# meringlab/FlashWeave.jl

Measured on AMD Instinct MI355X. Metric: ci_tests_per_sec, higher is better.
Workload: dtype f64

## Files before the change

flashweave.jl_amd/csrc/fw_devhiton.hip:

```cpp
#include <algorithm>
#include <cassert>
#include <cstring>
#include <condition_variable>
#include <mutex>
#include <thread>
#include <vector>

#include "fw_internal.h"
#define MI_MAX_K FW_MAX_K_FAST
#include "fw_mi_core.h"
#include "fw_fz_core.h"
#include "fw_unrank.h"

namespace {

struct DhTgt {
    int32_t T, phase, pos, nc;
    int32_t na, ntpc, npc, wl_n;
    long long co;
    long long cand_off;
    long long wl_off, nb_off;
    int32_t nb_n, cap;
    int32_t jactive, nsp;
    int32_t cur, pad0;
    unsigned long long jN, jnext, jwidth, jwin, jevaluated;
    unsigned long long c_eval_short;
    int na_max, wl_used;
    double jbest_p, jbest_stat;
    unsigned long long c_ref, c_calls, c_eval;
    double c_alg;
    unsigned int r_first0, r_more0, r_first1, r_more1;
    int32_t spmode, wl_unsorted;
    unsigned long long jwin2, jN2;
    long long tm_off;
};

struct DhGlobal {
    unsigned long long launched_ranks, next_ranks;
    unsigned int n_live_prev, n_live_next;
    unsigned int ns, seglen, done, rounds, rounds_nonempty, max_a;
    unsigned long long cond_tests_ref, subsets_calls, evaluated;
    double alg_bytes;
    unsigned int n_act, act_sel;
    unsigned int pad_b, max_ab;
    unsigned int ns_ring[64];
    unsigned int pad_l0[32];
    unsigned int step_ticket;
    unsigned int pad_l1[31];
    unsigned int any_big;
    unsigned int pad_l2[31];
};

#define DH_ACC_OFF(x, b, d1) (2ll * (x).co * (long long)(d1) + 2ll * (long long)(b) * (long long)(x).cap)

struct DhArrays {
    const int32_t *cand0;
    int32_t *tpc_key, *pc_key, *acc;
    double *tpc_stat, *tpc_p, *pc_stat, *pc_p;
    const int32_t *wl;
    const unsigned int *wl_cnt;
    const long long *nb_off;
    const int32_t *nb_idx;
    const double *nb_stat, *nb_p;
    const float *tmat;
    fw_rejection *rej;
};

struct DhParams {
    double alpha;
    int max_k;
    long long max_tests;
    unsigned long long small_launch, w0_big, w0_small;
    unsigned int seg_q, seg_min;
    double disc_bytes_per_col;
    int elim_full;
    unsigned long long growth_small, growth, growth_busy;
    unsigned int busy_jobs;
    int spec_depth;
    unsigned long long spec_below;
    unsigned int mi_seq, mi_win0, mi_chunk_div, mi_chunk_min, mi_chunk_max, mi_help_jobs;
    unsigned int mi_elim_min;
    unsigned int mi_heavy;
    unsigned int mi_seq_heavy;
    unsigned int mi_seq_tail;
    unsigned int mi_chunk_tail, mi_win0_tail;
    unsigned int mi_ahead;
    unsigned int mi_team;
    unsigned int mi_team_tail;
    unsigned int mi_team_steps;
    unsigned int mi_trace;
    int spec0_depth;
    unsigned long long spec0_below;
    unsigned int spec0_jobs;
    int spec0_depth_light;
    unsigned long long spec0_light_below;
    int spec1_depth;
    int elim_mode;
};

__device__ __forceinline__ bool dh_in_wl(const DhTgt &x, const DhArrays &A, int32_t v)
{
    const int lane = (int)(threadIdx.x & 63u);
    const int32_t *w = A.wl + x.wl_off;
    for (int base = 0; base < x.wl_n; base += 64) {
        const int32_t e = base + lane < x.wl_n ? w[base + lane] : -1;
        if (__ballot(e == v) != 0ull) return true;
        if (!x.wl_unsorted && __shfl(e, 63) > v) return false;
    }
    return false;
}

__device__ __forceinline__ double dh_alg_bytes(int a, unsigned long long evaluated, int max_k, double disc_bytes_per_col)
{
    double bytes = 0.0, left = (double)evaluated;
    for (int s = max_k; s >= 1 && left > 0.0; --s) {
        double b = 1.0;
        for (int i = 1; i <= s; ++i) b = b * (double)(a - s + i) / (double)i;
        if (a < s) b = 0.0;
        const double cnt = left < b ? left : b;
        bytes += cnt * (disc_bytes_per_col > 0.0 ? (double)(s + 2) * disc_bytes_per_col + 32.0
                                                 : 4.0 * (double)((s + 2) * (s + 1) / 2) + 32.0);
        left -= cnt;
    }
    return bytes;
}

__device__ __forceinline__ unsigned long long dh_enum_size(int a, int max_k, long long max_tests)
{
    unsigned long long N = 0ull;
    if (max_k <= 3 && a <= FW_UNRANK32_A) {
        for (int s = max_k; s >= 1; --s) N += (unsigned long long)fw_binom32(a, s);
    } else {
        for (int s = max_k; s >= 1; --s) {
            N += fw_binom_u64(a, s);
            if (N > (1ull << 62)) N = 1ull << 62;
        }
    }
    if (max_tests > 0 && (unsigned long long)max_tests < N) N = (unsigned long long)max_tests;
    return N;
}

__device__ __noinline__ void dh_rej_write(const DhTgt &x, const DhArrays &A, int max_k, int32_t cand, const int32_t *acc, int a,
                                          unsigned long long nt, double stat, double p, int df, int pow)
{
    const int32_t *b = A.nb_idx + x.nb_off;
    int lo = 0, hi = x.nb_n;
    while (lo < hi) {
        const int mid = (lo + hi) >> 1;
        if (b[mid] < cand)
            lo = mid + 1;
        else
            hi = mid;
    }
    if (lo >= x.nb_n || b[lo] != cand) return;
    fw_rejection r;
    r.target = x.T;
    r.candidate = cand;
    r.n_zs = 0;
#pragma unroll
    for (int q = 0; q < FW_MAX_K; ++q) r.zs[q] = 0;
    if (nt > 0ull) {
        unsigned long long rem = nt - 1ull;
        int s = max_k;
        while (s > 1) {
            const unsigned long long cnt = fw_binom_u64(a, s);
            if (rem < cnt) break;
            rem -= cnt;
            --s;
        }
        int pos[FW_MAX_K_FAST];
        fw_unrank_comb(rem, a, s, pos);
        r.n_zs = s;
#pragma unroll
        for (int q = 0; q < FW_MAX_K_FAST; ++q)
            if (q < s) r.zs[q] = acc[pos[q]];
    }
    r.df = nt > 0ull ? df : 0;
    r.suff_power = pow;
    r.phase = x.phase;
    r.n_acc = a;
    r.num_tests = (long long)nt;
    r.frac = 0.0;
    r.stat = stat;
    r.pval = p;
    A.rej[x.nb_off + lo] = r;
}

__device__ __forceinline__ double dh_alg_bytes_disc32(int a, unsigned long long evaluated, int max_k, double disc_bytes_per_col)
{
    double bytes = 0.0;
    unsigned long long left = evaluated;
    for (int s = max_k; s >= 1 && left > 0ull; --s) {
        const unsigned long long b = (unsigned long long)fw_binom32(a, s), cnt = left < b ? left : b;
        bytes += (double)cnt * ((double)(s + 2) * disc_bytes_per_col + 32.0);
        left -= cnt;
    }
    return bytes;
}

__device__ bool dh_advance(DhTgt &x, const DhArrays &A, int lane, int d1, bool keep_elim_stats = false)
{
    for (;;) {
        int32_t *acc = A.acc + DH_ACC_OFF(x, x.cur, d1);
        if (x.phase == 2) return false;
        const int32_t *cands = x.phase == 0 ? A.cand0 + x.cand_off : A.tpc_key + x.co;
        int32_t *dkey = (x.phase == 0 ? A.tpc_key : A.pc_key) + x.co;
        double *dstat = (x.phase == 0 ? A.tpc_stat : A.pc_stat) + x.co;
        double *dp = (x.phase == 0 ? A.tpc_p : A.pc_p) + x.co;
        int32_t &dn = x.phase == 0 ? x.ntpc : x.npc;
        while (x.pos < x.nc) {
            const int32_t cand = cands[x.pos];
            if (x.wl_n > 0 && dh_in_wl(x, A, cand)) {
                if (lane == 0) {
                    acc[x.na] = cand;
                    dkey[dn] = cand;
                    dstat[dn] = NAN;
                    dp[dn] = NAN;
                }
                ++x.na;
                x.wl_used += x.phase == 0 ? 1 : 0;
                ++dn;
                ++x.pos;
                continue;
            }
            if (x.phase == 1) {
                __builtin_amdgcn_fence(__ATOMIC_SEQ_CST, "workgroup");
                int w = 0;
                for (int base = 0; base < x.na; base += 64) {
                    const int q = base + lane;
                    const int32_t v = q < x.na ? acc[q] : cand;
                    const bool keep = q < x.na && v != cand;
                    const unsigned long long m = __ballot(keep);
                    if (keep) acc[w + __popcll(m & ((1ull << lane) - 1ull))] = v;
                    w += __popcll(m);
                }
                x.na = w;
                __builtin_amdgcn_fence(__ATOMIC_SEQ_CST, "workgroup");
            }
            if (x.na == 0) {
                double s = NAN, p = NAN;
                if (x.phase == 0) {
                    const int32_t *b = A.nb_idx + x.nb_off;
                    int lo = 0, hi = x.nb_n;
                    while (lo < hi) {
                        const int mid = (lo + hi) >> 1;
                        if (b[mid] < cand)
                            lo = mid + 1;
                        else
                            hi = mid;
                    }
                    s = A.nb_stat[x.nb_off + lo];
                    p = A.nb_p[x.nb_off + lo];
                } else {
                    for (int q = 0; q < x.ntpc; ++q)
                        if (A.tpc_key[x.co + q] == cand) {
                            s = A.tpc_stat[x.co + q];
                            p = A.tpc_p[x.co + q];
                            break;
                        }
                }
                if (lane == 0) {
                    acc[x.na] = cand;
                    dkey[dn] = cand;
                    dstat[dn] = s;
                    dp[dn] = p;
                }
                ++x.na;
                ++dn;
                ++x.pos;
                continue;
            }
            return true;
        }
        __builtin_amdgcn_fence(__ATOMIC_SEQ_CST, "workgroup");
        if (x.phase == 0) {
            x.phase = 1;
            x.nc = x.ntpc;
            for (int q = lane; q < x.ntpc; q += 64) acc[q] = A.tpc_key[x.co + q];
            x.na = x.ntpc;
            x.pos = 0;
        } else {
            for (int i = keep_elim_stats ? x.npc : lane; i < x.npc; i += 64) {
                const int32_t k = A.pc_key[x.co + i];
                for (int q = 0; q < x.ntpc; ++q)
                    if (A.tpc_key[x.co + q] == k) {
                        const double tp = A.tpc_p[x.co + q], pp = A.pc_p[x.co + i];
                        if (tp > pp || isnan(pp)) {
                            A.pc_stat[x.co + i] = A.tpc_stat[x.co + q];
                            A.pc_p[x.co + i] = tp;
                        }
                        break;
                    }
            }
            x.phase = 2;
        }
        __builtin_amdgcn_fence(__ATOMIC_SEQ_CST, "workgroup");
    }
}

__device__ __forceinline__ unsigned int dh_ceil_div(unsigned long long w, unsigned long long seglen, double inv)
{
    if (w == 0ull) return 0u;
    unsigned long long q = (unsigned long long)((double)w * inv);
    while (q * seglen < w) ++q;
    while (q > 0ull && (q - 1ull) * seglen >= w) --q;
    return (unsigned int)q;
}


#define DH_MAX_SPEC 8
#define DH_SPEC_EXACT 4

struct DhMerge {
    bool stop;
    double stat, p;
    int pow;
    unsigned long long nt;
    unsigned long long ev;
    double g;
    int df;
};

template <bool TR = false>
__device__ __forceinline__ DhMerge dh_merge(const FwSegOut *__restrict__ so, long long base, int nseg, int lane)
{
    unsigned long long ev = 0ull;
    int my_stop = 0x7fffffff;
    double st_stat = 0.0, st_p = 0.0;
    int st_pow = 0, st_df = 0;
    unsigned long long st_rank = 0ull;
    double bp = -2.0, bs = 0.0;
    int bi = -1;
    for (int sg = lane; sg < nseg; sg += 64) {
        const FwSegOut o = so[base + sg];
        ev += o.evaluated;
        if (o.stop_rank != FW_RANK_NONE) {
            if (my_stop == 0x7fffffff) {
                my_stop = sg;
                st_stat = o.stop_stat;
                st_p = o.stop_pval;
                st_pow = o.stop_power;
                st_rank = o.stop_rank;
                st_df = o.stop_df;
            }
        } else if (o.best_pval >= bp) {
            bp = o.best_pval;
            bs = o.best_stat;
            bi = sg;
        }
    }
    int first = my_stop;
#pragma unroll
    for (int o = 32; o > 0; o >>= 1) {
        ev += __shfl_xor(ev, o);
        const int f2 = __shfl_xor(first, o);
        first = f2 < first ? f2 : first;
        const double p2 = __shfl_xor(bp, o), s2 = __shfl_xor(bs, o);
        const int i2 = __shfl_xor(bi, o);
        if (p2 > bp || (p2 == bp && i2 > bi)) {
            bp = p2;
            bs = s2;
            bi = i2;
        }
    }
    DhMerge M;
    M.ev = ev;
    if (first != 0x7fffffff) {
        const int owner = first & 63;
        M.stop = true;
        M.stat = __shfl(st_stat, owner);
        M.p = __shfl(st_p, owner);
        M.pow = __shfl(st_pow, owner);
        M.nt = __shfl(st_rank, owner) + 1ull;
        if (__shfl(st_df, owner) == -2) M.nt = 0ull;
        if constexpr (TR) M.df = __shfl(st_df, owner);
    } else {
        M.stop = false;
        M.stat = bs;
        M.p = bi >= 0 ? bp : -2.0;
        M.pow = 1;
        M.nt = 0ull;
    }
    M.g = 0.0;
    if constexpr (!TR) M.df = 0;
    else if (!M.stop) M.df = 0;
    return M;
}

template <bool TR = false>
__device__ __forceinline__ bool dh_commit(DhTgt &x, const DhArrays &A, int lane, int d1, double r_stat, double r_p, int r_pow,
                                          double alpha, bool exact = false, int max_k_rej = 0, unsigned long long r_nt = 0ull, int r_df = 0)
{
    const int32_t *cands = x.phase == 0 ? A.cand0 + x.cand_off : A.tpc_key + x.co;
    const int32_t cand = cands[x.pos];
    ++x.pos;
    if (!(r_p < alpha && r_pow)) {
        if constexpr (TR) {
            if (lane == 0) dh_rej_write(x, A, max_k_rej, cand, A.acc + DH_ACC_OFF(x, x.cur, d1), x.na, r_nt, r_stat, r_p, r_df, r_pow);
        }
        if (!(exact && x.phase == 1)) return false;
        if (lane == 0) A.acc[DH_ACC_OFF(x, x.cur, d1) + x.na] = cand;
        ++x.na;
        return true;
    }
    if (lane == 0) {
        A.acc[DH_ACC_OFF(x, x.cur, d1) + x.na] = cand;
        if (x.phase == 0) {
            A.tpc_key[x.co + x.ntpc] = cand;
            A.tpc_stat[x.co + x.ntpc] = r_stat;
            A.tpc_p[x.co + x.ntpc] = r_p;
        } else {
            A.pc_key[x.co + x.npc] = cand;
            A.pc_stat[x.co + x.npc] = r_stat;
            A.pc_p[x.co + x.npc] = r_p;
        }
    }
    ++x.na;
    if (x.phase == 0)
        ++x.ntpc;
    else
        ++x.npc;
    return true;
}

#define MI_BOARD_CAP (1u << 18)
#define MI_REC_CAP (1u << 20)

__shared__ unsigned short dh_mi_tab[4][2 * MI_TAB16];

__shared__ int32_t dh_mi_acc[4][1024];
__shared__ DhTgt dh_mi_x[4];
__shared__ MiBest dh_mi_seed[4];
struct DhMiCtx {
    DhArrays A;
    MiDev M;
    DhParams P;
};
__shared__ DhMiCtx dh_mi_ctx;
__shared__ FwSegOut dh_mi_out[4];
#ifdef FW_MI_TICKS
__shared__ unsigned long long dh_mi_ticks[4][12];
#endif

struct MiBoard {
    unsigned long long tc;
    unsigned long long ac;
    unsigned long long acc_off;
    unsigned long long start, end;
    unsigned long long nr;
    unsigned long long stop_min;
    unsigned int next_chunk, done;
    unsigned int ready, seed_df;
    double seed_p, seed_g;
};

struct alignas(16) MiQueue {
    unsigned int next_target, targets_done, n_boards, hint, res_top, bacc_top, pad[1], next_team;
    unsigned long long t_body, t_ctl, t_sleep, n_seg;
    unsigned long long t_total;
    unsigned long long tick[12];
    unsigned long long tm_run, tm_wait, tm_steps, tm_tests;
};

#define MI_BACC_CAP (1u << 22)
#define MI_ACC_LDS 1024

__device__ __forceinline__ unsigned int mi_ld_u32(const unsigned int *p) { return __hip_atomic_load(p, __ATOMIC_RELAXED, __HIP_MEMORY_SCOPE_AGENT); }
__device__ __forceinline__ unsigned long long mi_ld_u64(const unsigned long long *p) { return __hip_atomic_load(p, __ATOMIC_RELAXED, __HIP_MEMORY_SCOPE_AGENT); }
__device__ __forceinline__ void mi_st_u64(unsigned long long *p, unsigned long long v) { __hip_atomic_store(p, v, __ATOMIC_RELAXED, __HIP_MEMORY_SCOPE_AGENT); }
__device__ __forceinline__ void mi_st_u32(unsigned int *p, unsigned int v) { __hip_atomic_store(p, v, __ATOMIC_RELAXED, __HIP_MEMORY_SCOPE_AGENT); }
__device__ __forceinline__ void mi_drain() { asm volatile("s_waitcnt vmcnt(0)" ::: "memory"); }
typedef unsigned int mi_u32x4 __attribute__((ext_vector_type(4)));
__device__ __forceinline__ mi_u32x4 mi_ld_u128(const void *p)
{
    mi_u32x4 v;
    asm volatile("global_load_dwordx4 %0, %1, off sc1\n\ts_waitcnt vmcnt(0)" : "=v"(v) : "v"(p) : "memory");
    return v;
}
#ifndef MI_NAP_WAIT
#define MI_NAP_WAIT 2
#endif
#ifndef MI_NAP_TAIL
#define MI_NAP_TAIL 32
#endif
__device__ __forceinline__ void mi_nap_wait()
{
#pragma unroll
    for (int i = 0; i < MI_NAP_WAIT; ++i) __builtin_amdgcn_s_sleep(2);
}
__device__ __forceinline__ void mi_nap_tail()
{
#pragma unroll
    for (int i = 0; i < MI_NAP_TAIL; ++i) __builtin_amdgcn_s_sleep(8);
}
#ifndef MI_WD_TICKS
#define MI_WD_TICKS 200000000ull
#endif
struct MiWatch {
    unsigned long long t0;
    unsigned int last, n;
};
__device__ __forceinline__ void mi_watch_begin(MiWatch &w, unsigned int word)
{
    w.t0 = 0ull;
    w.last = word;
    w.n = 0u;
}
__device__ __forceinline__ bool mi_watch_expired(MiWatch &w, unsigned int word)
{
    if (word != w.last) {
        w.last = word;
        w.t0 = 0ull;
        w.n = 0u;
        return false;
    }
    if ((++w.n & 255u) != 0u) return false;
    const unsigned long long now = wall_clock64();
    if (w.t0 == 0ull) {
        w.t0 = now;
        return false;
    }
    return now - w.t0 > MI_WD_TICKS;
}
__device__ __forceinline__ unsigned int mi_wave_add(unsigned int *p, unsigned int v, int lane)
{
    unsigned int r = 0u;
    if (lane == 0) r = atomicAdd(p, v);
    return (unsigned int)__builtin_amdgcn_readfirstlane((int)r);
}

__device__ __forceinline__ unsigned long long mi_rfl_lane64(unsigned long long v, int src)
{
    const unsigned lo = (unsigned)__builtin_amdgcn_readlane((int)(unsigned)v, src), hi = (unsigned)__builtin_amdgcn_readlane((int)(unsigned)(v >> 32), src);
    return ((unsigned long long)hi << 32) | lo;
}

template <int L, int NXY, int PRE, bool STOP_P = false>
__device__ __noinline__ void mi_run_ranks(int T, int cand, const int32_t *__restrict__ acc_in, int a, int max_k,
                                          long long max_tests, unsigned long long r0, unsigned long long r1,
                                          const unsigned long long *stop_min_in, int remote_acc, const MiBest *seed_in)
{
    unsigned short *tab = dh_mi_tab[threadIdx.x >> 6];
    const MiDev M = mi_uniform(dh_mi_ctx.M);
    T = __builtin_amdgcn_readfirstlane(T);
    cand = __builtin_amdgcn_readfirstlane(cand);
    a = __builtin_amdgcn_readfirstlane(a);
    max_k = __builtin_amdgcn_readfirstlane(max_k);
    max_tests = (long long)mi_rfl64((unsigned long long)max_tests);
    r0 = mi_rfl64(r0);
    r1 = mi_rfl64(r1);
    const int32_t *acc = (const int32_t *)mi_rfl64((unsigned long long)acc_in);
    const unsigned long long *stop_min = (const unsigned long long *)mi_rfl64((unsigned long long)stop_min_in);
    remote_acc = __builtin_amdgcn_readfirstlane(remote_acc);
    FwSegOut o;
    o.stop_rank = FW_RANK_NONE;
    o.stop_stat = o.stop_pval = 0.0;
    o.best_rank = 0ull;
    o.best_stat = 0.0;
    o.best_pval = -3.0;
// ... 1010 lines not shown
                        o.evaluated += computed;
                    }
                }
            }
            if (!first_known)
                o = mi_run_ranks_sel<L, NXY, PRE, R4>(x.T, cand, A.acc + acc_off, a, P.max_k, P.max_tests, 0ull, next, nullptr, 0, nullptr);
            unsigned long long ev = o.evaluated, nt = 0ull;
            bool stopped = o.stop_rank != FW_RANK_NONE;
            double r_stat = stopped ? o.stop_stat : 0.0, r_p = stopped ? o.stop_pval : 0.0;
            int r_pow = stopped ? o.stop_power : 1;
            double best_p = o.best_pval, best_stat = o.best_stat, best_g = stopped ? 0.0 : o.stop_stat;
            int best_df = o.best_df;
            if (stopped) nt = o.stop_rank + 1ull;
            unsigned long long width = elim_full ? N : (unsigned long long)(tail ? P.mi_win0_tail : P.mi_win0);
            const unsigned long long chunk_min = tail ? P.mi_chunk_tail : P.mi_chunk_min;
            unsigned int bacc_off = MI_BACC_CAP;
            const unsigned long long tk2 = MI_CLK();
            tk_seq += tk2 - tk1;
            if (lane == 0) x.r_first1 += (unsigned int)(tk2 - tk1);
            while (!stopped && next < N) {
                const unsigned long long W = (N - next) < width ? (N - next) : width;
                unsigned long long chunk = W / (unsigned long long)P.mi_chunk_div;
                chunk = chunk < chunk_min ? chunk_min : (chunk > P.mi_chunk_max ? P.mi_chunk_max : chunk);
                const unsigned int nch = (unsigned int)((W + chunk - 1ull) / chunk);
                unsigned int bi, ro;
                const unsigned long long tkp0 = MI_CLK();
                const bool published = mi_publish(Q, boards, bacc, bacc_off, A.acc + acc_off, a, x.T, cand, next, W, chunk, nch, lane, bi, ro,
                                                  best_p, best_g, best_df);
                MI_TICK(9, tkp0);
                DhMerge mg;
                if (!published) {
                    const FwSegOut q = mi_run_ranks_sel<L, NXY, PRE, R4>(x.T, cand, A.acc + acc_off, a, P.max_k, P.max_tests, next, next + W, nullptr, 0, nullptr);
                    mg.stop = q.stop_rank != FW_RANK_NONE;
                    mg.stat = mg.stop ? q.stop_stat : q.best_stat;
                    mg.p = mg.stop ? q.stop_pval : (q.best_pval < 0.0 ? -2.0 : q.best_pval);
                    mg.pow = q.stop_power;
                    mg.nt = q.stop_rank + 1ull;
                    mg.ev = q.evaluated;
                    mg.g = q.stop_stat;
                    mg.df = q.best_df;
                } else {
                    MiBoard *b = boards + bi;
                    while (mi_board_work<L, NXY, PRE, R4>(b, res, bacc, A.acc + acc_off, lane)) {
                    }
                    MiWatch wd;
                    unsigned int dn = mi_ld_u32(&b->done);
                    mi_watch_begin(wd, dn);
                    while (dn < nch) {
                        if (heavy || !mi_help<L, NXY, PRE, R4>(Q, boards, res, bacc, lane)) {
                            const unsigned long long tkw0 = MI_CLK();
                            mi_nap_wait();
                            MI_TICK(10, tkw0);
                            if (mi_watch_expired(wd, mi_ld_u32(&b->done))) {
                                if (lane == 0) atomicExch(&Q->pad[0], 1u);
                                break;
                            }
                        } else {
                            mi_watch_begin(wd, dn);
                        }
                        dn = mi_ld_u32(&b->done);
                    }
                    const unsigned long long tkm0 = MI_CLK();
                    mg = mi_merge(res, (long long)ro, (int)nch, lane);
                    MI_TICK(11, tkm0);
                }
                ev += mg.ev;
                if (mg.stop) {
                    stopped = true;
                    r_stat = mg.stat;
                    r_p = mg.p;
                    r_pow = mg.pow;
                    nt = mg.nt;
                } else if (mg.p != -2.0 && mg.p >= best_p) {
                    best_p = mg.p;
                    best_stat = mg.stat;
                    best_g = mg.g;
                    best_df = mg.df;
                }
                next += W;
                width *= 8ull;
            }
            {
                const unsigned long long tk3 = MI_CLK();
                tk_board += tk3 - tk2;
                if (lane == 0) {
                    x.r_more1 += (unsigned int)(tk3 - tk2);
                    if (next > (elim_full ? 0ull : (N < seq ? N : seq))) x.c_eval_short += 1ull;
                }
            }
            if (!stopped) {
                r_stat = best_stat;
                r_p = best_p < 0.0 ? 0.0 : best_p;
                r_pow = 1;
                nt = N;
            }
            const unsigned long long tkc0 = MI_CLK();
            x.c_ref += nt;
            x.c_calls += 1ull;
            x.c_eval += ev;
            x.c_alg += (P.max_k <= 3 && a <= FW_UNRANK32_A) ? dh_alg_bytes_disc32(a, ev, P.max_k, P.disc_bytes_per_col)
                                                            : dh_alg_bytes(a, ev, P.max_k, P.disc_bytes_per_col);
            if constexpr (TR) {
                if (stopped && !(r_p < P.alpha && r_pow)) mi_rej_record<L, NXY, PRE, R4>(Q, x, x.T, cand, A.acc + acc_off, a, nt, r_stat, r_p, r_pow, lane);
                dh_commit(x, A, lane, 1, r_stat, r_p, r_pow, P.alpha, P.elim_mode != 0);
            } else {
                dh_commit(x, A, lane, 1, r_stat, r_p, r_pow, P.alpha, EX);
            }
            MI_TICK(8, tkc0);
        }
        if (lane == 0) {
            x.r_more0 = (unsigned int)MI_CLK();
            tg[t] = x;
            atomicAdd(&Q->targets_done, 1u);
        }
    }
    const unsigned long long tk_t0 = MI_CLK();
    MiWatch wd;
    mi_watch_begin(wd, 0u);
    unsigned int wd_periods = 0u;
    while (mi_ld_u32(&Q->targets_done) < (unsigned int)ntg && mi_ld_u32(&Q->pad[0]) == 0u) {
        if (!mi_help<L, NXY, PRE, R4>(Q, boards, res, bacc, lane)) {
            mi_nap_tail();
            wd.n |= 255u;
            if (mi_watch_expired(wd, mi_ld_u32(&Q->targets_done) + mi_ld_u32(&Q->n_boards))) {
                wd.t0 = 0ull;
                if (++wd_periods >= 5u) {
                    if (lane == 0) atomicExch(&Q->pad[0], 2u);
                    break;
                }
            }
        } else {
            wd_periods = 0u;
            wd.t0 = 0ull;
        }
    }
    tk_tail = MI_CLK() - tk_t0;
    if (lane == 0) {
        atomicAdd(&Q->t_body, tk_seq);
        atomicAdd(&Q->t_ctl, tk_board);
        atomicAdd(&Q->t_sleep, tk_help);
        atomicAdd(&Q->n_seg, tk_tail);
        atomicAdd(&Q->t_total, tk_t0 - tk_begin);
#ifdef FW_MI_TICKS
        for (int q = 0; q < 12; ++q) atomicAdd(&Q->tick[q], dh_mi_ticks[threadIdx.x >> 6][q]);
#endif
    }
}

template <bool TR>
__device__ __forceinline__ void dh_step_dev(DhTgt *__restrict__ tg, int ntg, DhGlobal *__restrict__ g, const DhArrays &A,
                                            const FwSegOut *__restrict__ so, const long long *__restrict__ seg0,
                                            unsigned long long *__restrict__ win, unsigned int *__restrict__ sp,
                                            unsigned long long *__restrict__ win2, const int32_t *__restrict__ act, const DhParams &P,
                                            const int ci )
{
    const int lane = threadIdx.x & 63;
    const int d1 = P.spec_depth + 1;
    unsigned long long mywin = 0ull;
    if (ci < (int)g->n_act) {
        const int t = act[(size_t)g->act_sel * ntg + ci];
        DhTgt x = tg[t];
        const long long jseg0 = seg0[ci];
        const int nsp_done = x.nsp;
        const int spmode_done = x.spmode;
        const int nseg_all = (int)(seg0[ci + 1] - jseg0);
        int jnseg = nseg_all / (1 + nsp_done), jnseg2 = jnseg;
        if (nsp_done > 0 && spmode_done == 1) {
            const unsigned long long sl = g->seglen;
            jnseg = (int)dh_ceil_div(x.jwin, sl, 1.0 / (double)sl);
            jnseg2 = (nseg_all - jnseg) / nsp_done;
        }
        x.nsp = 0;
        x.spmode = 0;
        bool finished = false, kept = false;
        if (x.jactive) {
            if (x.phase == 0) (x.jnext == 0ull ? x.r_first0 : x.r_more0) += 1u;
            else (x.jnext == 0ull ? x.r_first1 : x.r_more1) += 1u;
            const DhMerge M = dh_merge<TR>(so, jseg0, jnseg, lane);
            double r_stat = 0.0, r_p = 1.0;
            int r_pow = 0;
            [[maybe_unused]] int r_df = 0;
            unsigned long long r_nt = 0ull;
            bool done = false;
            if (M.stop) {
                if constexpr (TR) r_df = M.df;
                r_stat = M.stat;
                r_p = M.p;
                r_pow = M.pow;
                r_nt = M.nt;
                done = true;
            } else if (M.p != -2.0 && M.p >= x.jbest_p) {
                x.jbest_p = M.p;
                x.jbest_stat = M.stat;
            }
            x.jevaluated += M.ev;
            if (!done) {
                x.jnext += x.jwin;
                const unsigned long long growth = g->launched_ranks < P.small_launch ? P.growth_small : (g->n_live_prev > P.busy_jobs ? P.growth_busy : P.growth);
                x.jwidth *= growth;
                if (x.jnext >= x.jN) {
                    r_stat = x.jbest_stat;
                    r_p = x.jbest_p < 0.0 ? 0.0 : x.jbest_p;
                    r_pow = 1;
                    r_nt = x.jN;
                    done = true;
                }
            }
            if (done) {
                x.jactive = 0;
                finished = true;
                x.c_ref += r_nt;
                x.c_calls += 1ull;
                x.c_eval += x.jevaluated;
                x.c_eval_short += x.na <= FW_HK_A ? x.jevaluated : 0ull;
                x.na_max = x.na > x.na_max ? x.na : x.na_max;
                x.c_alg += dh_alg_bytes(x.na, x.jevaluated, P.max_k, P.disc_bytes_per_col);
                if constexpr (TR) kept = dh_commit<true>(x, A, lane, d1, r_stat, r_p, r_pow, P.alpha, P.elim_mode != 0, P.max_k, r_nt, r_df);
                else kept = dh_commit(x, A, lane, d1, r_stat, r_p, r_pow, P.alpha, P.elim_mode != 0);
            }
        }
        if (nsp_done > 0) {
            const bool ph1 = x.phase == 1, acc_mode = spmode_done == 1;
            const int n = acc_mode ? x.na : x.na - (kept ? 1 : 0), cur0 = x.cur;
            const unsigned long long wsp = acc_mode ? x.jwin2 : x.jwin;
            if (acc_mode) x.jN = x.jN2;
            bool valid = finished && ((ph1 || acc_mode) ? kept : !kept);
            for (int j = 1; j <= nsp_done; ++j) {
                const DhMerge M = dh_merge<TR>(so, jseg0 + (long long)jnseg + (long long)(j - 1) * jnseg2, jnseg2, lane);
                if (!valid) {
                    x.c_eval += M.ev;
                    continue;
                }
                if (ph1) {
                    x.cur = (cur0 + j) % d1;
                    x.na = n;
                }
                if (!M.stop && wsp < x.jN) {
                    const unsigned long long growth = g->launched_ranks < P.small_launch ? P.growth_small : (g->n_live_prev > P.busy_jobs ? P.growth_busy : P.growth);
                    x.jactive = 1;
                    x.jnext = wsp;
                    x.jwidth = wsp * growth;
                    x.jbest_p = M.p != -2.0 ? M.p : -1.0;
                    x.jbest_stat = M.p != -2.0 ? M.stat : 0.0;
                    x.jevaluated = M.ev;
                    valid = false;
                    continue;
                }
                const double r_stat = M.stop ? M.stat : (M.p != -2.0 ? M.stat : 0.0);
                const double r_p = M.stop ? M.p : (M.p < 0.0 ? 0.0 : M.p);
                x.c_ref += M.stop ? M.nt : x.jN;
                x.c_calls += 1ull;
                x.c_eval += M.ev;
                x.c_eval_short += n <= FW_HK_A ? M.ev : 0ull;
                x.c_alg += dh_alg_bytes(n, M.ev, P.max_k, P.disc_bytes_per_col);
                bool k;
                if constexpr (TR) k = dh_commit<true>(x, A, lane, d1, r_stat, r_p, M.stop ? M.pow : 1, P.alpha, P.elim_mode != 0, P.max_k, M.nt, M.df);
                else k = dh_commit(x, A, lane, d1, r_stat, r_p, M.stop ? M.pow : 1, P.alpha, P.elim_mode != 0);
                valid = ph1 ? k : !k;
            }
        }
        if (!x.jactive && x.phase != 2 && dh_advance(x, A, lane, d1, P.elim_mode == 2)) {
            const unsigned long long N = dh_enum_size(x.na, P.max_k, P.max_tests);
            x.jN = N;
            x.jnext = 0ull;
            x.jwidth = (x.phase == 1 && P.elim_full) ? N : (x.na >= 64 ? P.w0_big : P.w0_small);
            x.jbest_p = -1.0;
            x.jbest_stat = 0.0;
            x.jevaluated = 0ull;
            x.jactive = 1;
            if (lane == 0 && (unsigned int)x.na > g->max_a) atomicMax(&g->max_a, (unsigned int)x.na);
            {
                const int abi = x.phase == 0 ? x.na + x.wl_n - x.wl_used : (x.na > x.ntpc ? x.na : x.ntpc);
                if (lane == 0 && (unsigned int)abi > g->max_ab) atomicMax(&g->max_ab, (unsigned int)abi);
            }
            if (x.phase == 0 && P.spec0_depth > 0 && g->launched_ranks < P.spec0_below && g->n_live_prev < P.spec0_jobs) {
                const int32_t *cands = A.cand0 + x.cand_off;
                int q = 0;
                const int depth = g->launched_ranks < P.spec0_light_below ? P.spec0_depth_light : P.spec0_depth;
                while (q < depth && x.pos + 1 + q < x.nc) {
                    if (x.wl_n > 0 && dh_in_wl(x, A, cands[x.pos + 1 + q])) break;
                    ++q;
                }
                x.nsp = q;
            }
            if (x.phase == 1 && P.elim_full && P.spec_depth > 0 && g->launched_ranks < P.spec_below) {
                const int32_t *cands = A.tpc_key + x.co;
                const int n = x.na;
                const int32_t c0 = cands[x.pos];
                int32_t cn[DH_MAX_SPEC];
                int Q = 0;
#pragma unroll
                for (int j = 0; j < DH_MAX_SPEC; ++j) {
                    cn[j] = -1;
                    if (j == Q && j < P.spec_depth && x.pos + 1 + j < x.nc) {
                        const int32_t c = cands[x.pos + 1 + j];
                        if (!(x.wl_n > 0 && dh_in_wl(x, A, c))) {
                            cn[j] = c;
                            Q = j + 1;
                        }
                    }
                }
                const int32_t *src = A.acc + DH_ACC_OFF(x, x.cur, d1);
                int w[DH_MAX_SPEC];
#pragma unroll
                for (int j = 0; j < DH_MAX_SPEC; ++j) w[j] = 0;
                __builtin_amdgcn_fence(__ATOMIC_SEQ_CST, "workgroup");
                for (int base = 0; base < n; base += 64) {
                    const int i = base + lane;
                    const int32_t v = i < n ? src[i] : -1;
                    bool alive = i < n;
#pragma unroll
                    for (int j = 0; j < DH_MAX_SPEC; ++j) {
                        if (j < Q) {
                            alive = alive && v != cn[j];
                            const unsigned long long m = __ballot(alive);
                            int32_t *dst = A.acc + DH_ACC_OFF(x, (x.cur + 1 + j) % d1, d1);
                            if (alive) dst[w[j] + __popcll(m & ((1ull << lane) - 1ull))] = v;
                            w[j] += __popcll(m);
                        }
                    }
                }
                int q = 0;
#pragma unroll
                for (int j = 0; j < DH_MAX_SPEC; ++j) {
                    if (j == q && j < Q && w[j] == n - (j + 1)) {
                        int32_t *dst = A.acc + DH_ACC_OFF(x, (x.cur + 1 + j) % d1, d1);
                        if (lane <= j) {
                            int32_t tail = c0;
#pragma unroll
                            for (int u = 0; u < DH_MAX_SPEC; ++u)
                                if (lane == u + 1) tail = cn[u];
                            dst[w[j] + lane] = tail;
                        }
                        q = j + 1;
                    }
                }
                __builtin_amdgcn_fence(__ATOMIC_SEQ_CST, "workgroup");
                x.nsp = q;
            }
        }
        if (x.jactive) {
            const unsigned long long left = x.jN - x.jnext;
            mywin = x.jwidth < left ? x.jwidth : left;
        }
        x.jwin = mywin;
        if (x.nsp > 0) x.jwin2 = mywin, x.jN2 = x.jN;
        if (x.jactive && x.phase == 0 && x.jnext > 0ull && mywin == x.jN - x.jnext && x.nsp == 0 && P.spec1_depth > 0 &&
            g->launched_ranks < P.spec0_below && g->n_live_prev < P.spec0_jobs) {
            const int32_t *cands = A.cand0 + x.cand_off;
            int q = 0;
            while (q < P.spec1_depth && x.pos + 1 + q < x.nc) {
                if (x.wl_n > 0 && dh_in_wl(x, A, cands[x.pos + 1 + q])) break;
                ++q;
            }
            if (q > 0) {
                if (lane == 0) A.acc[DH_ACC_OFF(x, x.cur, d1) + x.na] = cands[x.pos];
                const unsigned long long N2 = dh_enum_size(x.na + 1, P.max_k, P.max_tests);
                const unsigned long long w0 = x.na + 1 >= 64 ? P.w0_big : P.w0_small;
                x.nsp = q;
                x.spmode = 1;
                x.jN2 = N2;
                x.jwin2 = w0 < N2 ? w0 : N2;
                if (lane == 0 && (unsigned int)(x.na + 1) > g->max_a) atomicMax(&g->max_a, (unsigned int)(x.na + 1));
            }
        }
        if (lane == 0) {
            tg[t] = x;
            win[t] = mywin;
            sp[t] = (unsigned int)x.nsp;
            win2[t] = x.nsp > 0 ? x.jwin2 : 0ull;
        }
    }
}

template <bool TR>
__global__ __launch_bounds__(256) void dh_step_kernel(DhTgt *__restrict__ tg, int ntg, DhGlobal *__restrict__ g, DhArrays A,
                                                      const FwSegOut *__restrict__ so, const long long *__restrict__ seg0,
                                                      unsigned long long *__restrict__ win, unsigned int *__restrict__ sp,
                                                      unsigned long long *__restrict__ win2, const int32_t *__restrict__ act, DhParams P)
{
    dh_step_dev<TR>(tg, ntg, g, A, so, seg0, win, sp, win2, act, P, (int)(blockIdx.x * 4 + (threadIdx.x >> 6)));
}

#define DH_PER 16
struct DhPlanArgs {
    unsigned int seg_target, seg_q, seg_min, log_cap;
    ulonglong2 *log;
    unsigned long long seg_a, seg_b;
};
template <int NT>
__device__ __forceinline__ void dh_plan_dev(int ntg, DhGlobal *__restrict__ g, const unsigned long long *__restrict__ win,
                                            const unsigned int *__restrict__ sp, const unsigned long long *__restrict__ win2,
                                            const int32_t *__restrict__ act_all, long long *__restrict__ seg0, const DhPlanArgs PA)
{
    constexpr int NW = NT / 64;
    const unsigned int seg_target = PA.seg_target, seg_q = PA.seg_q, seg_min = PA.seg_min, log_cap = PA.log_cap;
    ulonglong2 *__restrict__ log = PA.log;
    const unsigned long long seg_a = PA.seg_a, seg_b = PA.seg_b;
    __shared__ unsigned long long s_tot[16];
    __shared__ unsigned int s_live[16], s_wsum[16];
    const int tid = threadIdx.x, lane = tid & 63, wave = tid >> 6;
    const int na = (int)g->n_act;
    const int32_t *act = act_all + (size_t)g->act_sel * ntg;
    const int per = (na + NT - 1) / NT;
    const int b = tid * per, e = (b + per) < na ? (b + per) : na;
    unsigned long long tot = 0ull;
    unsigned int live = 0u;
    unsigned long long wr[DH_PER];
    unsigned long long w2r[DH_PER];
    unsigned int mr[DH_PER];
#pragma unroll
    for (int q = 0; q < DH_PER; ++q) {
        const int tq = (b + q < e) ? act[b + q] : 0;
        wr[q] = (b + q < e) ? win[tq] : 0ull;
        mr[q] = (b + q < e) ? sp[tq] : 0u;
        w2r[q] = (b + q < e && mr[q] > 0u) ? win2[tq] : 0ull;
    }
#pragma unroll
    for (int q = 0; q < DH_PER; ++q) {
        tot += wr[q] + w2r[q] * mr[q];
        live += wr[q] != 0ull ? 1u + mr[q] : 0u;
    }
    for (int t = b + DH_PER; t < e; ++t) {
        const unsigned long long w = win[act[t]];
        const unsigned int m = sp[act[t]];
        tot += w + (m ? win2[act[t]] * m : 0ull);
        live += w != 0ull ? 1u + m : 0u;
    }
#pragma unroll
    for (int o = 32; o > 0; o >>= 1) {
        tot += __shfl_xor(tot, o);
        live += __shfl_xor(live, o);
    }
    if (lane == 0) {
        s_tot[wave] = tot;
        s_live[wave] = live;
    }
    __syncthreads();
    unsigned long long total = 0ull;
    unsigned int n_live = 0u;
#pragma unroll
    for (int w = 0; w < NW; ++w) {
        total += s_tot[w];
        n_live += s_live[w];
    }
    const unsigned int tgt = total < seg_a ? (seg_target + 2u) / 3u : (total < seg_b ? (2u * seg_target + 2u) / 3u : seg_target);
    unsigned long long seglen = (total / tgt + seg_q - 1ull) / seg_q * seg_q;
    seglen = seglen < seg_min ? seg_min : seglen;
    const double inv = 1.0 / (double)seglen;
    unsigned int local = 0u;
    unsigned int nr[DH_PER];
#pragma unroll
    for (int q = 0; q < DH_PER; ++q) {
        nr[q] = dh_ceil_div(wr[q], seglen, inv) + dh_ceil_div(w2r[q], seglen, inv) * mr[q];
        local += nr[q];
    }
    for (int t = b + DH_PER; t < e; ++t)
        local += dh_ceil_div(win[act[t]], seglen, inv) + (sp[act[t]] ? dh_ceil_div(win2[act[t]], seglen, inv) * sp[act[t]] : 0u);
    unsigned int incl = local;
#pragma unroll
    for (int o = 1; o < 64; o <<= 1) {
        const unsigned int v = __shfl_up(incl, o);
        if (lane >= o) incl += v;
    }
    if (lane == 63) s_wsum[wave] = incl;
    __syncthreads();
    unsigned int wbase = 0u, ns = 0u;
#pragma unroll
    for (int w = 0; w < NW; ++w) {
        if (w < wave) wbase += s_wsum[w];
        ns += s_wsum[w];
    }
    unsigned int run = wbase + incl - local;
#pragma unroll
    for (int q = 0; q < DH_PER; ++q)
        if (b + q < e) {
            seg0[b + q] = (long long)run;
            run += nr[q];
        }
    for (int t = b + DH_PER; t < e; ++t) {
        seg0[t] = (long long)run;
        run += dh_ceil_div(win[act[t]], seglen, inv) + (sp[act[t]] ? dh_ceil_div(win2[act[t]], seglen, inv) * sp[act[t]] : 0u);
    }
    if (tid == 0) {
        seg0[na] = (long long)ns;
        g->ns = ns;
        g->any_big = 0u;
        g->seglen = (unsigned int)seglen;
        g->launched_ranks = total;
        g->n_live_prev = n_live;
        if (n_live == 0u) g->done = 1u;
        const unsigned int r = g->rounds;
        g->ns_ring[r & 63u] = ns;
        g->rounds = r + 1u;
        if (log && r < log_cap) log[r] = make_ulonglong2(total, ((unsigned long long)n_live << 32) | ns);
    }
}

__global__ __launch_bounds__(1024) void dh_plan_kernel(int ntg, DhGlobal *__restrict__ g, const unsigned long long *__restrict__ win,
                                                       const unsigned int *__restrict__ sp, const unsigned long long *__restrict__ win2,
                                                       const int32_t *__restrict__ act_all, long long *__restrict__ seg0, DhPlanArgs PA)
{
    dh_plan_dev<1024>(ntg, g, win, sp, win2, act_all, seg0, PA);
}
__global__ __launch_bounds__(256) void dh_plan_small_kernel(int ntg, DhGlobal *__restrict__ g, const unsigned long long *__restrict__ win,
                                                            const unsigned int *__restrict__ sp, const unsigned long long *__restrict__ win2,
                                                            const int32_t *__restrict__ act_all, long long *__restrict__ seg0, DhPlanArgs PA)
{
    dh_plan_dev<256>(ntg, g, win, sp, win2, act_all, seg0, PA);
}

__global__ __launch_bounds__(256) void dh_tmat_build_kernel(const DhTgt *__restrict__ tg, int ntg, const int32_t *__restrict__ nb_idx,
                                                            const float *__restrict__ cor, int p, float *__restrict__ tmat)
{
    __shared__ int32_t s_id[4096];
    const DhTgt &x = tg[blockIdx.x];
    if (x.tm_off < 0) return;
    const int m = x.nb_n + 1;
    const int32_t *ids = nb_idx + x.nb_off;
    for (int b = threadIdx.x; b < m; b += 256) s_id[b] = b == 0 ? x.T : ids[b - 1];
    __syncthreads();
    float *M = tmat + x.tm_off;
    for (int a0 = (int)blockIdx.y * 4; a0 < m; a0 += (int)gridDim.y * 4)
        for (int b = threadIdx.x; b < m; b += 256) {
            const size_t col = (size_t)s_id[b];
            float v[4];
#pragma unroll
            for (int q = 0; q < 4; ++q) v[q] = a0 + q < m ? cor[(size_t)s_id[a0 + q] * (size_t)p + col] : 0.0f;
#pragma unroll
            for (int q = 0; q < 4; ++q)
                if (a0 + q < m) M[(size_t)(a0 + q) * m + b] = v[q];
        }
}

__device__ __forceinline__ void dh_fill_one(const unsigned int s, const DhTgt *__restrict__ tg, int ntg, DhGlobal *__restrict__ g,
                                            const long long *__restrict__ seg0, const DhArrays &A, FwSeg *__restrict__ segs, int d1,
                                            const int32_t *__restrict__ act)
{
    int lo = 0, hi = (int)g->n_act;
    while (lo < hi) {
        const int mid = (lo + hi) >> 1;
        if (seg0[mid] <= (long long)s)
            lo = mid + 1;
        else
            hi = mid;
    }
    const DhTgt &x = tg[act[(size_t)g->act_sel * ntg + lo - 1]];
    const unsigned long long seglen = g->seglen;
    unsigned long long k = (unsigned long long)((long long)s - seg0[lo - 1]);
    const int32_t *cands = x.phase == 0 ? A.cand0 + x.cand_off : A.tpc_key + x.co;
    unsigned int slot = 0;
    if (x.nsp > 0) {
        const unsigned int all = (unsigned int)(seg0[lo] - seg0[lo - 1]);
        const unsigned int n0 = x.spmode == 1 ? dh_ceil_div(x.jwin, seglen, 1.0 / (double)seglen) : all / (1u + (unsigned int)x.nsp);
        if ((unsigned int)k >= n0) {
            const unsigned int per = (all - n0) / (unsigned int)x.nsp;
            slot = 1u + ((unsigned int)k - n0) / per;
            k -= (unsigned long long)n0 + (unsigned long long)(slot - 1u) * per;
        }
    }
    const bool acc_mode = slot > 0u && x.spmode == 1;
    FwSeg sg;
    sg.X = x.T;
    sg.Y = cands[x.pos + (int)slot];
    sg.acc_off = DH_ACC_OFF(x, x.phase == 1 ? (x.cur + (int)slot) % d1 : x.cur, d1);
    sg.acc_len = x.na + (acc_mode ? 1 : 0);
    if (sg.acc_len > FW_TAB_A) g->any_big = 1u;
    sg.pad = act[(size_t)g->act_sel * ntg + lo - 1];
    const unsigned long long lo_r = acc_mode ? 0ull : x.jnext;
    sg.start = lo_r + k * seglen;
    const unsigned long long hi_r = lo_r + (slot > 0u ? x.jwin2 : x.jwin);
    sg.end = sg.start + seglen < hi_r ? sg.start + seglen : hi_r;
    const bool has_tm = A.tmat != nullptr && x.tm_off >= 0;
    sg.tm = has_tm ? (uint64_t)(A.tmat + x.tm_off) : 0ull;
    sg.tm_ids = has_tm ? (uint64_t)(A.nb_idx + x.nb_off) : 0ull;
    sg.tm_m = has_tm ? x.nb_n + 1 : 0;
    sg.pad1 = 0;
    segs[s] = sg;
}
__global__ __launch_bounds__(256) void dh_fill_kernel(const DhTgt *__restrict__ tg, int ntg, DhGlobal *__restrict__ g,
                                                      const long long *__restrict__ seg0, const DhArrays A,
                                                      FwSeg *__restrict__ segs, int d1, const int32_t *__restrict__ act)
{
    const unsigned int s = blockIdx.x * 256 + threadIdx.x;
    if (s >= g->ns) return;
    dh_fill_one(s, tg, ntg, g, seg0, A, segs, d1, act);
}


__global__ __launch_bounds__(1024) void dh_compact_kernel(const DhTgt *__restrict__ tg, int ntg, DhGlobal *__restrict__ g,
                                                          int32_t *__restrict__ act_all)
{
    __shared__ unsigned int s_wsum[16];
    const int tid = threadIdx.x, lane = tid & 63, wave = tid >> 6;
    const int na = (int)g->n_act;
    const unsigned int sel = g->act_sel;
    const int32_t *src = act_all + (size_t)sel * ntg;
    int32_t *dst = act_all + (size_t)(sel ^ 1u) * ntg;
    const int per = (na + 1023) / 1024;
    const int b = tid * per, e = (b + per) < na ? (b + per) : na;
    unsigned int local = 0u;
    for (int i = b; i < e; ++i) {
        const DhTgt &x = tg[src[i]];
        local += (x.phase != 2 || x.jactive) ? 1u : 0u;
    }
    unsigned int incl = local;
#pragma unroll
    for (int o = 1; o < 64; o <<= 1) {
        const unsigned int v = __shfl_up(incl, o);
        if (lane >= o) incl += v;
    }
    if (lane == 63) s_wsum[wave] = incl;
    __syncthreads();
    unsigned int wbase = 0u, total = 0u;
#pragma unroll
    for (int w = 0; w < 16; ++w) {
        if (w < wave) wbase += s_wsum[w];
        total += s_wsum[w];
    }
    unsigned int pos = wbase + incl - local;
    for (int i = b; i < e; ++i) {
        const int t = src[i];
        const DhTgt &x = tg[t];
        if (x.phase != 2 || x.jactive) dst[pos++] = t;
    }
    if (tid == 0) {
        g->n_act = total;
        g->act_sel = sel ^ 1u;
    }
}

__global__ __launch_bounds__(256) void dh_nz_recs_kernel(const DhTgt *__restrict__ tg, int ntg, const DhGlobal *__restrict__ g,
                                                         const int32_t *__restrict__ act, const DhArrays A, FwNzJob *__restrict__ recs,
                                                         const long long *__restrict__ arena_off)
{
    const int ci = (int)(blockIdx.x * 256u + threadIdx.x);
    if (ci >= (int)g->n_act) return;
    const int t = act[(size_t)g->act_sel * ntg + ci];
    const DhTgt &x = tg[t];
    FwNzJob *r = recs + t;
    if (x.jactive && x.jwin > 0ull && x.jnext == 0ull) {
        r->X = x.T;
        r->Y = (x.phase == 0 ? A.cand0 + x.cand_off : A.tpc_key + x.co)[x.pos];
        r->acc_off = DH_ACC_OFF(x, x.cur, 1);
        r->acc_len = x.na;
        r->m = x.na + 2;
        r->cor_off = arena_off[t];
        r->pad = 0;
    } else {
        r->pad = 1;
    }
}

__global__ __launch_bounds__(256) void dh_sched_init_kernel(DhTgt *__restrict__ tg, int nt, const int32_t *__restrict__ tgt_T,
                                                            const long long *__restrict__ nb_off, const int32_t *__restrict__ levels,
                                                            const long long *__restrict__ slot_tm, int wl_unsorted)
{
    const int i = (int)(blockIdx.x * 256u + threadIdx.x);
    if (i >= nt) return;
    DhTgt x;
    __builtin_memset(&x, 0, sizeof(x));
    const int T = tgt_T[i];
    const long long o = nb_off[T];
    const int deg = (int)(nb_off[T + 1] - o);
    x.T = T;
    x.nc = x.cap = deg;
    x.phase = (deg == 0 || (levels && levels[T] < 2)) ? 2 : 0;
    x.co = x.cand_off = x.wl_off = x.nb_off = o;
    x.nb_n = deg;
    x.wl_unsorted = wl_unsorted;
    if (slot_tm) x.tm_off = slot_tm[i];
    tg[i] = x;
}

__global__ __launch_bounds__(256) void dh_wl_append_kernel(const DhTgt *__restrict__ tg, int ntg, const int32_t *__restrict__ pc_key,
                                                           const int32_t *__restrict__ round_of, int round, int32_t *__restrict__ wl,
                                                           const long long *__restrict__ nb_off, unsigned int *__restrict__ wl_cnt)
{
    const int t = (int)(blockIdx.x * 4u + (threadIdx.x >> 6)), lane = threadIdx.x & 63;
    if (t >= ntg) return;
    const int T = tg[t].T, npc = tg[t].npc;
    const long long co = tg[t].co;
    for (int i = lane; i < npc; i += 64) {
        const int32_t u = pc_key[co + i];
        if (round_of[u] > round) wl[nb_off[u] + (long long)atomicAdd(&wl_cnt[u], 1u)] = T;
    }
}

__global__ __launch_bounds__(256) void dh_iota_kernel(int32_t *__restrict__ act, int n)
{
    const int i = (int)(blockIdx.x * 256u + threadIdx.x);
    if (i < n) act[i] = i;
}

__global__ __launch_bounds__(256) void dh_fz_round_begin_kernel(DhTgt *__restrict__ tg, int ntg, const unsigned int *__restrict__ wl_cnt,
                                                                int32_t *__restrict__ wl, DhGlobal *__restrict__ g, long long *__restrict__ seg0,
                                                                int32_t *__restrict__ act, unsigned int *__restrict__ wl_max)
{
    __shared__ int32_t s_w[4096];
    const int t = (int)blockIdx.x, tid = (int)threadIdx.x;
    if (t >= ntg) return;
    DhTgt &x = tg[t];
    const int n = (int)wl_cnt[x.T];
    if (n > 1 && n <= 4096) {
        int32_t *w = wl + x.wl_off;
        for (int i = tid; i < n; i += 256) s_w[i] = w[i];
        __syncthreads();
        for (int i = tid; i < n; i += 256) {
            const int32_t e = s_w[i];
            int r = 0;
            for (int j = 0; j < n; ++j) r += s_w[j] < e;
            w[r] = e;
        }
    }
    if (tid == 0) {
        x.wl_n = n;
        x.wl_unsorted = n > 4096;
        act[t] = t;
        seg0[t] = 0;
        if (n > 0) atomicMax(wl_max, (unsigned int)n);
    }
    if (t == 0) {
        unsigned int *gw = (unsigned int *)g;
        for (int i = tid; i < (int)(sizeof(DhGlobal) / 4); i += 256) gw[i] = 0u;
        __syncthreads();
        if (tid == 0) {
            g->n_act = (unsigned int)ntg;
            seg0[ntg] = 0;
        }
    }
}

__global__ __launch_bounds__(256) void dh_sched_pack_kernel(const DhTgt *__restrict__ tg, int nt, const int32_t *__restrict__ pc_key,
                                                         const double *__restrict__ pc_stat, const double *__restrict__ pc_p,
                                                         int32_t *__restrict__ o_t, int32_t *__restrict__ o_u, double *__restrict__ o_s,
                                                         double *__restrict__ o_p, unsigned long long *__restrict__ tot, double *__restrict__ alg)
{
    const int t = (int)(blockIdx.x * 4u + (threadIdx.x >> 6)), lane = threadIdx.x & 63;
    if (t >= nt) return;
// ... 102 lines not shown
    P.w0_big = fz ? fw_knob_u64(knob::FW_W0_BIG, c->P.max_k <= 3 ? 32768ull : 16384ull) : 16ull;
    P.seg_q = fz ? 256u : 4u;
    P.seg_min = fz ? 256u : 8u;
    P.disc_bytes_per_col = fz ? 0.0 : (double)c->P.n * (c->P.kind == FW_MI ? 1.0 : 2.0) / 8.0;
    P.elim_mode = c->elim_mode;
    return P;
}

struct DhPolicy {
    bool nzk;
    bool fz;
    bool per_target;
    bool use_hp, plan_small;
    unsigned seg_target, grid_seg;
    unsigned long long seg_a, seg_b;
    int spec_depth, spec0_depth;
    int nb;
    int time_every;
    int tm_min;
    const char *log_path;
};
constexpr int DH_BATCH = 16;
constexpr unsigned DH_LOG_CAP = 1u << 16;

static DhPolicy dh_policy(const fw_ctx *c, int ntg)
{
    DhPolicy y{};
    const bool fz_kind = c->P.kind == FW_FZ || c->P.kind == FW_FZ_NZ;
    static const int tm_env = fw_knob_int(knob::FW_FZ_TMAT, -1);
    y.tm_min = tm_env >= 0 ? tm_env : (c->P.max_k > 3 ? 1 : 16);
    static const unsigned seg_target_env = (unsigned)fw_seg_target();
    y.seg_target = seg_target_env ? seg_target_env : (fz_kind ? (c->P.max_k > 3 ? 8192u : 3072u) : 4096u);
    static const int spec_env = fw_knob_int(knob::FW_DH_SPEC, -1);
    const int spec_dflt = c->elim_mode != 0 ? DH_SPEC_EXACT : 4;
    y.spec_depth = c->P.kind == FW_FZ ? std::min(std::max(spec_env >= 0 ? spec_env : spec_dflt, 0), DH_MAX_SPEC) : 0;
    static const bool mi_rounds = fw_mi_rounds();
    y.nzk = c->P.kind == FW_FZ_NZ;
    y.fz = fz_kind;
    y.per_target = !fz_kind && !mi_rounds;
    static const int spec0_env = fw_knob_int(knob::FW_DH_SPEC0, 2);
    y.spec0_depth = c->P.kind == FW_FZ ? std::min(std::max(spec0_env, 0), DH_MAX_SPEC) : 0;
    static const unsigned long long seg_a_env = fw_knob_u64(knob::FW_SEG_A, 8000000ull);
    static const unsigned long long seg_b_env = fw_knob_u64(knob::FW_SEG_B, 12000000ull);
    y.seg_a = fz_kind ? seg_a_env : 0ull;
    y.seg_b = fz_kind ? seg_b_env : 0ull;
    static const unsigned seg_grid_env = (unsigned)fw_knob_pos(knob::FW_SEG_GRID, 0ull);
    const unsigned grid_dflt = (c->P.kind == FW_FZ && c->P.max_k <= 3) ? std::min(y.seg_target + 512u, 2048u) : y.seg_target + 512u;
    y.grid_seg = seg_grid_env ? std::min(y.seg_target + 512u, seg_grid_env) : grid_dflt;
    static const char *log_path = fw_knob_str(knob::FW_DH_LOG);
    y.log_path = log_path;
    static const int nb_env = std::min((int)fw_knob_pos(knob::FW_DH_BATCH, 0ull), DH_BATCH);
    y.nb = nb_env ? nb_env : (ntg <= 1024 ? 4 : DH_BATCH);
    static const int time_every = (int)fw_knob_pos(knob::FW_DH_TIME_EVERY, 4ull);
    y.time_every = time_every;
    static const int hp_env = fw_knob_int(knob::FW_DH_HP, -1);
    y.use_hp = !y.per_target && hp_env > 0;
    static const bool plan_small = fw_knob_on(knob::FW_DH_PLAN_SMALL);
    y.plan_small = plan_small;
    return y;
}

static unsigned dh_team_min() { static const unsigned v = (unsigned)fw_knob_int(knob::FW_MI_TEAM_MIN, 96); return v; }
static unsigned dh_team_max() { static const unsigned v = (unsigned)fw_knob_int(knob::FW_MI_TEAM_MAX, 192); return v; }
template <class Deg>
static unsigned dh_heaviest_first(int32_t *order, int n, Deg deg)
{
    for (int t = 0; t < n; ++t) order[t] = t;
    std::stable_sort(order, order + n, [&](int32_t u, int32_t v) { return deg(u) > deg(v); });
    const unsigned team_min = dh_team_min(), team_max = dh_team_max();
    unsigned team = 0u;
    while (team_min > 0u && team < team_max && (int)team < n && (unsigned)deg(order[team]) >= team_min) ++team;
    return team;
}

static unsigned dh_mi_launch(fw_ctx *c, hipStream_t st, DhTgt *d_tg, int ntg, const int32_t *d_order, const DhArrays &A, DhParams P, unsigned team,
                             bool trace_host, MiQueue *d_mq, MiBoard *d_boards, FwSegOut *d_mres, int32_t *d_bacc)
{
    MiDev M = fwi_mi_dev(c);
    M.view = M.dense && M.nzmode && c->mi_view;
    static const unsigned wg_per_cu = (unsigned)fw_knob_pos(knob::FW_MI_WG_PER_CU, 1ull);
    int n_cu = 256;
    (void)hipDeviceGetAttribute(&n_cu, hipDeviceAttributeMultiprocessorCount, c->P.device);
    const unsigned grid = std::min((unsigned)((ntg + 3) / 4), wg_per_cu * (unsigned)n_cu);
    static const unsigned team_steps = (unsigned)fw_knob_int(knob::FW_MI_TEAM_STEPS, 2);
    static const unsigned team_tail = (unsigned)fw_knob_int(knob::FW_MI_TEAM_TAIL, 0);
    P.mi_team = team;
    P.mi_team_steps = team_steps;
    P.mi_team_tail = team_tail;
#ifdef FW_MI_TICKS
    P.mi_trace = 1u;
#else
    P.mi_trace = trace_host ? 1u : 0u;
#endif
#define DH_MI_LAUNCH(LL, NN, PP, RR)                                                                                                  \
    do {                                                                                                                              \
        if (A.rej)                                                                                                                    \
            hipLaunchKernelGGL((dh_mi_target_kernel<LL, NN, PP, RR, false, true>), dim3(grid), dim3(256), 0, st, d_tg, ntg, d_order, \
                               A, M, P, d_mq, d_boards, d_mres, d_bacc);                                                              \
        else if (P.elim_mode != 0)                                                                                                    \
            hipLaunchKernelGGL((dh_mi_target_kernel<LL, NN, PP, RR, true, false>), dim3(grid), dim3(256), 0, st, d_tg, ntg, d_order, \
                               A, M, P, d_mq, d_boards, d_mres, d_bacc);                                                              \
        else                                                                                                                          \
            hipLaunchKernelGGL((dh_mi_target_kernel<LL, NN, PP, RR, false, false>), dim3(grid), dim3(256), 0, st, d_tg, ntg, d_order,\
                               A, M, P, d_mq, d_boards, d_mres, d_bacc);                                                              \
    } while (0)
    const bool pre = c->P.n <= MI_PRE_N && c->P.max_k <= MI_PRE_K;
    static const bool row4_env = fw_knob_on(knob::FW_MI_ROW4);
    static const bool row4_force = fw_knob_int(knob::FW_MI_ROW4, 1) == 2;
    const bool r4 = row4_env && pre && c->P.n <= (row4_force ? MI4_N : 2048) && (c->L == 2 || c->mi_nxy == 2);
    const bool wide = c->P.n > 65535;
    if (c->L == 2) {
        if (wide) DH_MI_LAUNCH(2, 2, 2, false); else if (r4) DH_MI_LAUNCH(2, 2, 1, true); else if (pre) DH_MI_LAUNCH(2, 2, 1, false); else DH_MI_LAUNCH(2, 2, 0, false);
    } else if (c->mi_nxy == 2) {
        if (wide) DH_MI_LAUNCH(3, 2, 2, false); else if (r4) DH_MI_LAUNCH(3, 2, 1, true); else if (pre) DH_MI_LAUNCH(3, 2, 1, false); else DH_MI_LAUNCH(3, 2, 0, false);
    } else {
        if (wide) DH_MI_LAUNCH(3, 3, 2, false); else if (pre) DH_MI_LAUNCH(3, 3, 1, false); else DH_MI_LAUNCH(3, 3, 0, false);
    }
#undef DH_MI_LAUNCH
    return grid;
}

static void dh_mi_trace(const MiQueue &hq, unsigned grid)
{
    const double nw = 4.0 * (double)grid, ms = 1e-5;
    if (hq.tick[1])
        fprintf(stderr, "[fw] test routine: %llu calls, %llu tests (mean set size %.2f); per test %.2f us before the core (unranking, list), %.2f us in the core, %.2f us in the accounting (Q)\n",
                hq.tick[0], hq.tick[1], (double)hq.tick[5] / (double)hq.tick[1], 1e-2 * hq.tick[2] / (double)hq.tick[1],
                1e-2 * hq.tick[3] / (double)hq.tick[1], 1e-2 * hq.tick[4] / (double)hq.tick[1]);
    if (hq.tick[1])
        fprintf(stderr, "[fw] state machine, ms per wavefront: dh_advance %.3f, job set-up %.3f, commit + counters %.3f, publish %.3f, idle wait for own board %.3f, merge %.3f; "
                        "test routine: before the core %.3f, core %.3f, accounting %.3f\n",
                ms * hq.tick[6] / nw, ms * hq.tick[7] / nw, ms * hq.tick[8] / nw, ms * hq.tick[9] / nw, ms * hq.tick[10] / nw, ms * hq.tick[11] / nw,
                ms * hq.tick[2] / nw, ms * hq.tick[3] / nw, ms * hq.tick[4] / nw);
    if (hq.tm_steps)
        fprintf(stderr, "[fw] team rounds: %llu wavefront-rounds, %llu tests in them; per wavefront-round %.2f us in the test routine, %.2f us at the barrier\n",
                hq.tm_steps, hq.tm_tests, 1e-2 * hq.tm_run / (double)hq.tm_steps, 1e-2 * hq.tm_wait / (double)hq.tm_steps);
    fprintf(stderr, "[fw] boards %u records %u; per wavefront (%u wavefronts): until out of targets %.2f ms = own first tests %.2f + board phases %.2f + helping before jobs %.2f + state machine %.2f; tail %.2f ms\n",
            hq.n_boards, hq.res_top, 4u * grid, ms * hq.t_total / nw, ms * hq.t_body / nw, ms * hq.t_ctl / nw, ms * hq.t_sleep / nw,
            ms * ((double)hq.t_total - (double)hq.t_body - (double)hq.t_ctl - (double)hq.t_sleep) / nw, ms * hq.n_seg / nw);
}

static int dh_mi_check(fw_ctx *c, const MiQueue &hq, unsigned grid, int round, int ntg, bool trace_host)
{
    if (hq.pad[0])
        return fw_fail(c, FW_ERR_DEVICE, "discrete HITON kernel, round %d: watchdog %u (boards %u, targets done %u of %d)", round, hq.pad[0], hq.n_boards, hq.targets_done, ntg);
    if (trace_host) dh_mi_trace(hq, grid);
    return FW_OK;
}


struct DhLists {
    int32_t *tpc_key, *pc_key, *acc, *wl;
    double *tpc_stat, *tpc_p, *pc_stat, *pc_p;
};
static DhLists dh_lists_layout(DhArena &a, size_t n, size_t acc_d1, size_t n_wl)
{
    DhLists b{};
    b.tpc_key = a.take<int32_t>(n, 4);
    b.pc_key = a.take<int32_t>(n, 4);
    b.acc = a.take<int32_t>(2 * n * acc_d1, 4);
    b.tpc_stat = a.take<double>(n, 8);
    b.tpc_p = a.take<double>(n, 8);
    b.pc_stat = a.take<double>(n, 8);
    b.pc_p = a.take<double>(n, 8);
    b.wl = a.take<int32_t>(n_wl, 4);
    return b;
}

struct DhRoundScratch {
    DhGlobal *g;
    long long *seg0;
    unsigned long long *win, *win2;
    unsigned int *sp;
    int32_t *act;
    FwSeg *segs;
    FwSegOut *so;
    float *tmat;
};
static DhRoundScratch dh_scratch_layout(DhArena &a, size_t ntg, size_t max_ns, size_t tm_floats)
{
    DhRoundScratch b{};
    b.g = a.take<DhGlobal>(1);
    b.seg0 = a.take<long long>(ntg + 1);
    b.win = a.take<unsigned long long>(ntg + 1);
    b.sp = a.take<unsigned int>(ntg + 1);
    b.win2 = a.take<unsigned long long>(ntg + 1);
    b.act = a.take<int32_t>(2 * ntg);
    b.segs = a.take<FwSeg>(max_ns);
    b.so = a.take<FwSegOut>(max_ns);
    if (tm_floats) b.tmat = a.take<float>(tm_floats, 4);
    return b;
}

struct DhLevel0 {
    long long *off;
    int32_t *idx;
    double *stat, *p;
};

static DhArrays dh_arrays(const fw_ctx *c, const int32_t *cand0, const DhLists &s, const DhLevel0 &own)
{
    const bool nb_on_dev = c->d_nb_idx != nullptr;
    DhArrays A{};
    A.cand0 = cand0;
    A.tpc_key = s.tpc_key;
    A.pc_key = s.pc_key;
    A.acc = s.acc;
    A.tpc_stat = s.tpc_stat;
    A.tpc_p = s.tpc_p;
    A.pc_stat = s.pc_stat;
    A.pc_p = s.pc_p;
    A.wl = s.wl;
    A.nb_off = nb_on_dev ? c->d_nb_off : own.off;
    A.nb_idx = nb_on_dev ? c->d_nb_idx : own.idx;
    A.nb_stat = nb_on_dev ? c->d_nb_stat : own.stat;
    A.nb_p = nb_on_dev ? c->d_nb_p : own.p;
    A.rej = c->d_rej_run;
    return A;
}


struct DhRunSizes {
    size_t ntg, tot, d1, n_wl, max_ns, tm_floats, nz_arena, p, nnz;
    bool log, per_target, nzk, own_nb;
};
struct DhRunBufs {
    DhTgt *tg;
    DhRoundScratch s;
    int32_t *cand0;
    DhLists lists;
    ulonglong2 *log;
    MiQueue *mq;
    MiBoard *boards;
    FwSegOut *mres;
    int32_t *bacc;
    FwNzJob *nzrecs;
    long long *nzaoff;
    float *nzarena;
    DhLevel0 nb;
};
static DhRunBufs dh_run_layout(DhArena &a, const DhRunSizes &z)
{
    DhRunBufs b{};
    b.tg = a.take<DhTgt>(z.ntg);
    b.s = dh_scratch_layout(a, z.ntg, z.max_ns, z.tm_floats);
    b.cand0 = a.take<int32_t>(z.tot, 4);
    b.lists = dh_lists_layout(a, z.tot, z.d1, z.n_wl);
    if (z.log) b.log = a.take<ulonglong2>(DH_LOG_CAP);
    if (z.per_target) {
        b.mq = a.take<MiQueue>(1);
        b.boards = a.take<MiBoard>(MI_BOARD_CAP);
        b.mres = a.take<FwSegOut>(MI_REC_CAP);
        b.bacc = a.take<int32_t>(MI_BACC_CAP);
    }
    if (z.nzk) {
        b.nzrecs = a.take<FwNzJob>(z.ntg);
        b.nzaoff = a.take<long long>(z.ntg);
        b.nzarena = a.take<float>(z.nz_arena, 4);
    }
    if (z.own_nb) {
        b.nb.off = a.take<long long>(z.p + 1);
        b.nb.idx = a.take<int32_t>(z.nnz, 4);
        b.nb.stat = a.take<double>(z.nnz, 8);
        b.nb.p = a.take<double>(z.nnz, 8);
    }
    return b;
}

struct DhRun {
    fw_ctx *c;
    int chain, ntg;
    hipStream_t st;
    bool trace_host;
    DhPolicy y;
    bool use_devc;
    std::vector<DhTgt> tg;
    std::vector<int32_t> cand0, wl;
    std::vector<long long> nz_aoff;
    size_t tot = 0, tm_floats = 0, nz_arena = 0;
    int max_cap = 0, max_wl = 0;
    unsigned max_ns = 0;
    DhRunBufs D{};
    DhGlobal *hg = nullptr;
    DhArrays A{};
    DhParams P{};
    double timed_s = 0.0;
    long timed_n = 0, launches_n = 0;
    std::vector<float> log_ms;
    unsigned max_a_seen = 0;
    unsigned max_ab_seen = 0;
    bool dev_wl = false;
};

static long long dh_tm_off(const fw_ctx *c, const DhPolicy &y, int deg, size_t &tm_floats)
{
    const bool tm_on = c->P.kind == FW_FZ && c->P.max_k <= 5 && c->d_cor != nullptr && y.tm_min > 0;
    const size_t m = (size_t)deg + 1;
    if (!tm_on || deg < y.tm_min || m > 4096 || tm_floats + m * m > (size_t)1 << 32) return -1;
    const long long off = (long long)tm_floats;
    tm_floats += m * m;
    return off;
}
static unsigned dh_max_ns(const DhPolicy &y, int ntg) { return y.seg_target + (unsigned)ntg * (unsigned)(1 + DH_MAX_SPEC) + 256u; }

static void dh_build_targets(DhRun &R, const std::vector<FwDhTarget> &in)
{
    const fw_ctx *c = R.c;
    const int ntg = R.ntg;
    R.use_devc = in[0].nc_dev >= 0 && c->d_cand != nullptr;
    R.tg.resize((size_t)ntg);
    long long co = 0, wo = 0;
    for (int t = 0; t < ntg; ++t) {
        DhTgt x{};
        x.T = in[t].T;
        x.nc = R.use_devc ? in[t].nc_dev : (int32_t)in[t].cands.size();
        x.cap = x.nc;
        x.cand_off = R.use_devc ? c->nb_off[in[t].T] : co;
        x.phase = x.nc == 0 ? 2 : 0;
        x.co = co;
        x.wl_off = wo;
        x.wl_n = in[t].wl_n;
        x.nb_off = c->nb_off[x.T];
        x.nb_n = (int32_t)(c->nb_off[x.T + 1] - c->nb_off[x.T]);
        if (!R.use_devc) R.cand0.insert(R.cand0.end(), in[t].cands.begin(), in[t].cands.end());
        if (in[t].wl_n) R.wl.insert(R.wl.end(), in[t].wl, in[t].wl + in[t].wl_n);
        co += x.nc;
        wo += in[t].wl_n;
        R.max_cap = std::max(R.max_cap, x.nc);
        R.max_wl = std::max(R.max_wl, (int)in[t].wl_n);
        R.tg[t] = x;
    }
    R.tot = (size_t)co;
    for (int t = 0; t < ntg; ++t) R.tg[t].tm_off = dh_tm_off(c, R.y, R.tg[t].nb_n, R.tm_floats);
    if (R.y.nzk) {
        R.nz_aoff.resize((size_t)ntg);
        for (int t = 0; t < ntg; ++t) {
            R.nz_aoff[t] = (long long)R.nz_arena;
            const size_t mt = (size_t)(R.wl.empty() ? 1 : 2) * (size_t)R.tg[t].nc + 2;
            R.nz_arena += mt * mt;
        }
    }
    R.max_ns = dh_max_ns(R.y, ntg);
}

static int dh_upload(DhRun &R)
{
    fw_ctx *c = R.c;
    hipStream_t st = R.st;
    const int ntg = R.ntg, p = c->P.p;
    const size_t tot = R.tot, nnz = (size_t)c->nb_off[p];
    const bool nb_on_dev = c->d_nb_idx != nullptr;
    const DhRunSizes z{(size_t)ntg, tot, (size_t)R.y.spec_depth + 1, R.wl.size(), R.max_ns, R.tm_floats, R.nz_arena, (size_t)p, nnz,
                       R.y.log_path != nullptr, R.y.per_target, R.y.nzk, !nb_on_dev};
    int rc;
    if ((rc = dh_arena_reserve(c, c->d_dh[R.chain], dh_run_layout, z, &R.D))) return rc;
    if ((rc = fw_pin_reserve(c, c->h_dh[R.chain], 4096))) return rc;
    const DhRunBufs &D = R.D;
    DhGlobal *hg = R.hg = (DhGlobal *)c->h_dh[R.chain].ptr;
    memset(hg, 0, 2 * sizeof(DhGlobal));
    if (R.y.nzk) {
        FW_HIP(c, hipMemcpyAsync(D.nzaoff, R.nz_aoff.data(), sizeof(long long) * (size_t)ntg, hipMemcpyHostToDevice, st));
        FW_HIP(c, hipMemsetAsync(D.nzrecs, 0xff, sizeof(FwNzJob) * (size_t)ntg, st));
    }
    FW_HIP(c, hipMemcpyAsync(D.tg, R.tg.data(), sizeof(DhTgt) * ntg, hipMemcpyHostToDevice, st));
    hg[0].n_act = (unsigned int)ntg;
    FW_HIP(c, hipMemcpyAsync(D.s.g, hg, sizeof(DhGlobal), hipMemcpyHostToDevice, st));
    hipLaunchKernelGGL(dh_iota_kernel, dim3((unsigned)((ntg + 255) / 256)), dim3(256), 0, st, D.s.act, ntg);
    FW_HIP(c, hipMemsetAsync(D.s.seg0, 0, sizeof(long long) * ((size_t)ntg + 1), st));
    if (tot && !R.use_devc) FW_HIP(c, hipMemcpyAsync(D.cand0, R.cand0.data(), 4 * tot, hipMemcpyHostToDevice, st));
    if (!R.wl.empty()) FW_HIP(c, hipMemcpyAsync(D.lists.wl, R.wl.data(), 4 * R.wl.size(), hipMemcpyHostToDevice, st));
    if (!nb_on_dev) {
        FW_HIP(c, hipMemcpyAsync(D.nb.off, c->nb_off.data(), 8 * ((size_t)p + 1), hipMemcpyHostToDevice, st));
        if (nnz) {
            FW_HIP(c, hipMemcpyAsync(D.nb.idx, c->nb_idx.data(), 4 * nnz, hipMemcpyHostToDevice, st));
            FW_HIP(c, hipMemcpyAsync(D.nb.stat, c->nb_stat.data(), 8 * nnz, hipMemcpyHostToDevice, st));
            FW_HIP(c, hipMemcpyAsync(D.nb.p, c->nb_p.data(), 8 * nnz, hipMemcpyHostToDevice, st));
        }
    }
    DhArrays &A = R.A = dh_arrays(c, R.use_devc ? c->d_cand : D.cand0, D.lists, D.nb);
    A.tmat = D.s.tmat;
    if (D.s.tmat) {
        hipLaunchKernelGGL(dh_tmat_build_kernel, dim3((unsigned)ntg, 8u), dim3(256), 0, st, (const DhTgt *)D.tg, ntg, A.nb_idx, (const float *)c->d_cor, p, D.s.tmat);
        FW_HIP(c, hipGetLastError());
        if (R.trace_host) fprintf(stderr, "[fw] chain %d: local correlation matrices: %.1f MB\n", R.chain, 4e-6 * (double)R.tm_floats);
    }
    R.P = dh_make_params(c, ntg, R.y.spec_depth, R.y.spec0_depth);
    return FW_OK;
}

static int dh_run_persistent(DhRun &R, DhEvents &E)
{
    fw_ctx *c = R.c;
    hipStream_t st = R.st;
    const int ntg = R.ntg;
    const DhRunBufs &D = R.D;
    const std::vector<DhTgt> &tg = R.tg;
    std::vector<int32_t> order((size_t)ntg);
    const unsigned team = dh_heaviest_first(order.data(), ntg, [&](int32_t t) { return tg[t].nc; });
    FW_HIP(c, hipMemcpyAsync(D.s.act, order.data(), sizeof(int32_t) * (size_t)ntg, hipMemcpyHostToDevice, st));
    if (R.trace_host) {
        int c32 = 0, c64 = 0, c128 = 0, c192 = 0;
        for (int t = 0; t < ntg; ++t) c32 += tg[t].nc >= 32, c64 += tg[t].nc >= 64, c128 += tg[t].nc >= 128, c192 += tg[t].nc >= 192;
        fprintf(stderr, "[fw] chain %d: %u targets run by a workgroup each (>= %u candidates); targets with >= 32 / 64 / 128 / 192 candidates: %d / %d / %d / %d; "
                        "candidates of the 1st / 64th / 256th heaviest: %d / %d / %d\n", R.chain, team, dh_team_min(), c32, c64, c128, c192,
                tg[order[0]].nc, ntg > 63 ? tg[order[63]].nc : -1, ntg > 255 ? tg[order[255]].nc : -1);
    }
    FW_HIP(c, hipMemsetAsync(D.mq, 0, sizeof(MiQueue), st));
    FW_HIP(c, hipMemsetAsync(D.boards, 0, sizeof(MiBoard) * MI_BOARD_CAP, st));
    FW_HIP(c, hipEventRecord(E.ev[0], st));
    const unsigned grid = dh_mi_launch(c, st, D.tg, ntg, (const int32_t *)D.s.act, R.A, R.P, team, R.trace_host, D.mq, D.boards, D.mres, D.bacc);
    FW_HIP(c, hipGetLastError());
    FW_HIP(c, hipEventRecord(E.ev[1], st));
    FW_HIP(c, hipStreamSynchronize(st));
    MiQueue hq{};
    FW_HIP(c, hipMemcpy(&hq, D.mq, sizeof(hq), hipMemcpyDeviceToHost));
    if (int rc = dh_mi_check(c, hq, grid, 0, ntg, R.trace_host)) return rc;
    float ms = 0.0f;
    FW_HIP(c, hipEventElapsedTime(&ms, E.ev[0], E.ev[1]));
    R.timed_s = 1e-3 * (double)ms;
    R.timed_n = R.launches_n = 1;
    return FW_OK;
}

struct DhRounds {
    DhRun &R;
    DhEvents &E;
    fw_ctx *c = R.c;
    const DhRunBufs &D = R.D;
    const DhRoundScratch &S = R.D.s;
    const DhPolicy &y = R.y;
    const int ntg = R.ntg;
    hipStream_t st = R.st, hs = R.st;
    DhPlanArgs PA{};
    const bool any_wl = !R.wl.empty() || (R.dev_wl && R.max_wl > 0);
    const bool any_big_static = (any_wl ? 2 * R.max_cap : R.max_cap) > FW_TAB_A;
    const unsigned g_fill = (R.max_ns + 255) / 256;
    unsigned n_act_bound = (unsigned)R.ntg;
    bool big_skipped[2] = {false, false};

    DhRounds(DhRun &r, DhEvents &e) : R(r), E(e)
    {
        PA.seg_target = y.seg_target;
        PA.seg_q = R.P.seg_q;
        PA.seg_min = R.P.seg_min;
        PA.log_cap = DH_LOG_CAP;
        PA.log = D.log;
        PA.seg_a = y.seg_a;
        PA.seg_b = y.seg_b;
    }
    hipEvent_t &ev(int q, int i) { return E.ev[(size_t)(q * 2 * DH_BATCH + i)]; }
    bool timed(unsigned b, int r) const { return ((r + (int)(b % (unsigned)y.time_every)) % y.time_every) == 0; }

    int hp_stream()
    {
        const int chain = R.chain;
        if (!c->dh_hp_stream[chain]) {
            int lo = 0, hi = 0;
            FW_HIP(c, hipDeviceGetStreamPriorityRange(&lo, &hi));
            FW_HIP(c, hipStreamCreateWithPriority(&c->dh_hp_stream[chain], hipStreamNonBlocking, hi));
            for (int e = 0; e < 2; ++e) FW_HIP(c, hipEventCreateWithFlags(&c->dh_hp_ev[chain][e], hipEventDisableTiming));
        }
        hs = c->dh_hp_stream[chain];
        return FW_OK;
    }
    int planfill(bool compact)
    {
        const DhArrays &A = R.A;
        if (y.use_hp) {
            FW_HIP(c, hipEventRecord(c->dh_hp_ev[R.chain][0], st));
            FW_HIP(c, hipStreamWaitEvent(hs, c->dh_hp_ev[R.chain][0], 0));
        }
        if (A.rej)
            hipLaunchKernelGGL(dh_step_kernel<true>, dim3((n_act_bound + 3u) / 4u), dim3(256), 0, hs, D.tg, ntg, S.g, A,
                               (const FwSegOut *)S.so, (const long long *)S.seg0, S.win, S.sp, S.win2, (const int32_t *)S.act, R.P);
        else
            hipLaunchKernelGGL(dh_step_kernel<false>, dim3((n_act_bound + 3u) / 4u), dim3(256), 0, hs, D.tg, ntg, S.g, A,
                               (const FwSegOut *)S.so, (const long long *)S.seg0, S.win, S.sp, S.win2, (const int32_t *)S.act, R.P);
        if (compact)
            hipLaunchKernelGGL(dh_compact_kernel, dim3(1), dim3(1024), 0, hs, (const DhTgt *)D.tg, ntg, S.g, S.act);
        if (y.plan_small)
            hipLaunchKernelGGL(dh_plan_small_kernel, dim3(1), dim3(256), 0, hs, ntg, S.g, (const unsigned long long *)S.win,
                               (const unsigned int *)S.sp, (const unsigned long long *)S.win2, (const int32_t *)S.act, S.seg0, PA);
        else
            hipLaunchKernelGGL(dh_plan_kernel, dim3(1), dim3(1024), 0, hs, ntg, S.g, (const unsigned long long *)S.win,
                               (const unsigned int *)S.sp, (const unsigned long long *)S.win2, (const int32_t *)S.act, S.seg0, PA);
        hipLaunchKernelGGL(dh_fill_kernel, dim3(g_fill), dim3(256), 0, hs, (const DhTgt *)D.tg, ntg, S.g,
                           (const long long *)S.seg0, A, S.segs, y.spec_depth + 1, (const int32_t *)S.act);
        if (y.use_hp) {
            FW_HIP(c, hipEventRecord(c->dh_hp_ev[R.chain][1], hs));
            FW_HIP(c, hipStreamWaitEvent(st, c->dh_hp_ev[R.chain][1], 0));
        }
        return FW_OK;
    }
    int enqueue_batch(unsigned b)
    {
        const DhArrays &A = R.A;
        const int q = (int)(b & 1u);
        const unsigned *d_ns = &S.g->ns;
        for (int r = 0; r < y.nb; ++r) {
            const bool any_big = any_big_static && R.max_ab_seen + 3u * (unsigned)DH_BATCH + 1u > (unsigned)FW_TAB_A;
            if (r == 0) big_skipped[q] = false;
            if (!any_big) big_skipped[q] = true;
            if (timed(b, r)) (void)hipEventRecord(ev(q, 2 * r), st);
            const unsigned grid_mi = std::min(R.max_ns, y.seg_target + n_act_bound * (unsigned)(1 + std::max(y.spec_depth, y.spec0_depth)) + 256u);
            int rc;
            if (y.nzk) {
                hipLaunchKernelGGL(dh_nz_recs_kernel, dim3((n_act_bound + 255u) / 256u), dim3(256), 0, st, (const DhTgt *)D.tg, ntg, (const DhGlobal *)S.g,
                                   (const int32_t *)S.act, A, D.nzrecs, (const long long *)D.nzaoff);
                rc = fwi_fznz_submatrices_dev(c, ntg, D.nzrecs, A.acc, D.nzarena, (any_wl ? 2 * R.max_cap : R.max_cap) + 2, true, st);
                if (!rc) rc = fwi_fznz_segments_dev(c, y.grid_seg, S.segs, A.acc, S.so, d_ns, any_big, &S.g->any_big, D.nzrecs, D.nzarena, st);
            } else {
                rc = y.fz ? fwi_fz_segments_dev(c, y.grid_seg, S.segs, A.acc, S.so, d_ns, any_big, &S.g->any_big, st)
                          : fwi_mi_segments_dev(c, grid_mi, S.segs, A.acc, S.so, d_ns, st);
            }
            if (rc) return rc;
            if (timed(b, r)) (void)hipEventRecord(ev(q, 2 * r + 1), st);
            if ((rc = planfill((b * (unsigned)y.nb + (unsigned)r) % 16u == 0u))) return rc;
        }
        FW_HIP(c, hipGetLastError());
        FW_HIP(c, hipMemcpyAsync(R.hg + q, S.g, sizeof(DhGlobal), hipMemcpyDeviceToHost, st));
        FW_HIP(c, hipEventRecord(E.ev_end[q], st));
        return FW_OK;
    }
    int retire_batch(unsigned b, int *done)
    {
        const int q = (int)(b & 1u);
        FW_HIP(c, hipEventSynchronize(E.ev_end[q]));
        const DhGlobal &rec = R.hg[q];
        for (int r = 0; r < y.nb; ++r) {
            if (rec.ns_ring[(b * (unsigned)y.nb + (unsigned)r) & 63u] == 0) continue;
            ++R.launches_n;
            if (!timed(b, r)) continue;
            float ms = 0.0f;
            FW_HIP(c, hipEventElapsedTime(&ms, ev(q, 2 * r), ev(q, 2 * r + 1)));
            R.timed_s += 1e-3 * (double)ms;
            ++R.timed_n;
            if (y.log_path) {
                const size_t idx = (size_t)b * (size_t)y.nb + (size_t)r;
                if (R.log_ms.size() <= idx) R.log_ms.resize(idx + 1, 0.0f);
                R.log_ms[idx] = ms;
            }
        }
        if (y.fz && c->P.max_k <= 3 && big_skipped[q] && rec.max_a > (unsigned)FW_TAB_A)
            return fw_fail(c, FW_ERR_DEVICE, "device rounds: an accepted list of %u entries met a batch without the in-lane kernel", rec.max_a);
        R.max_a_seen = std::max(R.max_a_seen, rec.max_a);
        R.max_ab_seen = std::max(R.max_ab_seen, rec.max_ab);
        n_act_bound = std::min(n_act_bound, rec.n_act);
        *done = rec.done != 0u;
        return FW_OK;
    }
    int run()
    {
        int rc = y.use_hp ? hp_stream() : FW_OK;
        if (rc) return rc;
        R.max_ab_seen = (unsigned)R.max_wl;
        unsigned b = 0;
        int done = 0;
        if (!(rc = planfill(true)))
            rc = enqueue_batch(0);
        while (!rc) {
            if ((rc = enqueue_batch(b + 1))) break;
            if ((rc = retire_batch(b, &done))) break;
            ++b;
            if (done) {
                int d2 = 0;
                rc = retire_batch(b, &d2);
                break;
            }
            if (b > 250000u) {
                rc = fw_fail(c, FW_ERR_DEVICE, "device HITON: no convergence after %u rounds", b * (unsigned)y.nb);
                break;
            }
        }
        if (rc) (void)hipStreamSynchronize(st);
        return rc;
    }
};

static int dh_write_log(const DhRun &R)
{
    fw_ctx *c = R.c;
    std::vector<ulonglong2> lg(DH_LOG_CAP);
    DhGlobal fin{};
    FW_HIP(c, hipMemcpy(&fin, R.D.s.g, sizeof(DhGlobal), hipMemcpyDeviceToHost));
    FW_HIP(c, hipMemcpy(lg.data(), R.D.log, sizeof(ulonglong2) * DH_LOG_CAP, hipMemcpyDeviceToHost));
    long long n_tpc = 0, n_pc = 0;
    for (const DhTgt &x : R.tg) {
        n_tpc += x.ntpc;
        n_pc += x.npc;
    }
    if (FILE *f = fopen(R.y.log_path, "a")) {
        fprintf(f, "# targets %d rounds %u tpc %lld pc %lld\n", R.ntg, fin.rounds, n_tpc, n_pc);
        for (unsigned r = 0; r < fin.rounds && r < DH_LOG_CAP; ++r)
            fprintf(f, "%u %llu %llu %llu %.1f\n", r, lg[r].x, lg[r].y >> 32, lg[r].y & 0xffffffffull,
                    r < R.log_ms.size() ? 1e3 * (double)R.log_ms[r] : 0.0);
        fclose(f);
    }
    return FW_OK;
}

static int dh_download(DhRun &R, std::vector<FwDhResult> &out, FwDhFlat &flat)
{
    fw_ctx *c = R.c;
    const size_t tot = R.tot;
    flat.key.resize(tot);
    flat.stat.resize(tot);
    flat.pval.resize(tot);
    FW_HIP(c, hipMemcpyAsync(R.tg.data(), R.D.tg, sizeof(DhTgt) * R.ntg, hipMemcpyDeviceToHost, R.st));
    if (tot) {
        FW_HIP(c, hipMemcpyAsync(flat.key.data(), R.A.pc_key, 4 * tot, hipMemcpyDeviceToHost, R.st));
        FW_HIP(c, hipMemcpyAsync(flat.stat.data(), R.A.pc_stat, 8 * tot, hipMemcpyDeviceToHost, R.st));
        FW_HIP(c, hipMemcpyAsync(flat.pval.data(), R.A.pc_p, 8 * tot, hipMemcpyDeviceToHost, R.st));
    }
    FW_HIP(c, hipStreamSynchronize(R.st));
    if (R.D.log)
        if (int rc = dh_write_log(R)) return rc;
    for (int t = 0; t < R.ntg; ++t) {
        const DhTgt &x = R.tg[t];
        if (x.phase != 2) return fw_fail(c, FW_ERR_DEVICE, "device HITON: target %d did not finish (phase %d)", x.T, x.phase);
        out[t].off = x.co;
        out[t].n = x.npc;
    }
    return FW_OK;
}

static void dh_trace_run(const DhRun &R, double t_setup, double t_rounds, double t_results)
{
    const std::vector<DhTgt> &tg = R.tg;
    const int chain = R.chain;
    unsigned long long mx_ref = 0, mx_calls = 0, tot_ref = 0, tot_calls = 0;
    int t_ref = -1, t_calls = -1;
    for (const DhTgt &x : tg) {
        tot_ref += x.c_ref;
        tot_calls += x.c_calls;
        if (x.c_ref > mx_ref) mx_ref = x.c_ref, t_ref = x.T;
        if (x.c_calls > mx_calls) mx_calls = x.c_calls, t_calls = x.T;
    }
    fprintf(stderr, "[fw] chain %d: tests %llu jobs %llu; most tests in one target %llu (T=%d), most jobs in one target %llu (T=%d)\n",
            chain, tot_ref, tot_calls, mx_ref, t_ref, mx_calls, t_calls);
    unsigned long long ev_all = 0, ev_short = 0;
    int na_max = 0;
    for (const DhTgt &x : tg) {
        ev_all += x.c_eval;
        ev_short += x.c_eval_short;
        na_max = std::max(na_max, x.na_max);
    }
    fprintf(stderr, "[fw] chain %d: executed tests %llu, of them in jobs with at most %d accepted variables %llu; longest accepted list %d\n",
            chain, ev_all, (int)FW_HK_A, ev_short, na_max);
    if (R.y.per_target) {
        unsigned int t0 = ~0u;
        for (const DhTgt &x : tg) t0 = std::min(t0, x.r_first0);
        std::vector<const DhTgt *> by_end;
        for (const DhTgt &x : tg) by_end.push_back(&x);
        std::sort(by_end.begin(), by_end.end(), [&](const DhTgt *a, const DhTgt *b) { return a->r_more0 - t0 > b->r_more0 - t0; });
        for (size_t i = 0; i < by_end.size() && i < 6; ++i) {
            const DhTgt *w = by_end[i];
            fprintf(stderr, "[fw]   finished at %.2f ms (taken at %.2f): T=%d, %d candidates, %d in PC, %llu jobs, %llu tests (%llu executed); "
                            "sequential prefixes %.2f ms, board phases %.2f ms (%llu jobs went to a board; %llu team rounds)\n",
                    1e-5 * (w->r_more0 - t0), 1e-5 * (w->r_first0 - t0), w->T, w->cap, w->npc, w->c_calls, w->c_ref, w->c_eval,
                    1e-5 * w->r_first1, 1e-5 * w->r_more1, w->c_eval_short & 0xffffffffull, w->c_eval_short >> 32);
        }
    } else {
        const DhTgt *w = &tg[0];
        for (const DhTgt &x : tg)
            if (x.r_first0 + x.r_more0 + x.r_first1 + x.r_more1 > w->r_first0 + w->r_more0 + w->r_first1 + w->r_more1) w = &x;
        fprintf(stderr, "[fw] chain %d: longest-busy target T=%d: %d candidates, %d in TPC, %d in PC, %llu jobs; rounds: interleaving first windows %u, later windows %u; elimination first %u, later %u\n",
                chain, w->T, w->cap, w->ntpc, w->npc, w->c_calls, w->r_first0, w->r_more0, w->r_first1, w->r_more1);
    }
    fprintf(stderr, "[fw] chain %d: longest accepted list %u, accepted + whitelisted to come %u (most whitelisted neighbours of one target %d)\n",
            chain, R.max_a_seen, R.max_ab_seen, R.max_wl);
    fprintf(stderr, "[fw] device rounds chain %d: %d targets, set-up %.2f ms, rounds %.2f ms, results %.2f ms\n", chain, R.ntg,
            1e3 * t_setup, 1e3 * t_rounds, 1e3 * t_results);
}

static void dh_count_run(const DhRun &R, long extra_kernels)
{
    fw_ctx *c = R.c;
    std::lock_guard<std::mutex> lk(dh_cnt_mu);
    if (R.timed_n > 0) c->cnt.t_dev_subsets_s += R.timed_s * (double)R.launches_n / (double)R.timed_n;
    c->cnt.subsets_launches += R.launches_n;
    c->cnt.kernel_launches += (R.y.per_target ? R.launches_n : (R.y.nzk ? 7 : 4) * R.launches_n) + extra_kernels;
}

int fwi_devhiton_run(fw_ctx *c, const std::vector<FwDhTarget> &in, std::vector<FwDhResult> &out, FwDhFlat &flat, int chain)
{
    const int ntg = (int)in.size();
    out.assign((size_t)ntg, FwDhResult{});
    if (ntg == 0) return FW_OK;
    static const bool trace_host = fw_trace_host();
    const double th0 = fwi_now_s();
    if (chain > 0 && !c->dh_stream[chain]) FW_HIP(c, hipStreamCreateWithFlags(&c->dh_stream[chain], hipStreamNonBlocking));
    DhRun R{c, chain, ntg, chain == 0 ? c->pb[0].stream : c->dh_stream[chain], trace_host, dh_policy(c, ntg)};
    dh_build_targets(R, in);
    int rc;
    if ((rc = dh_upload(R))) return rc;
    DhEvents E(R.st, 2 * 2 * DH_BATCH, 2);
    if (!E.ok) return fw_fail(c, FW_ERR_DEVICE, "device HITON: hipEventCreate failed");
    const double th1 = fwi_now_s();
    rc = R.y.per_target ? dh_run_persistent(R, E) : DhRounds(R, E).run();
    dh_count_run(R, 0);
    if (rc) return rc;
    const double th2 = fwi_now_s();
    if ((rc = dh_download(R, out, flat))) return rc;
    if (trace_host) dh_trace_run(R, th1 - th0, th2 - th1, fwi_now_s() - th2);
    std::lock_guard<std::mutex> lk(dh_cnt_mu);
    for (const DhTgt &x : R.tg) {
        c->cnt.cond_tests_ref += (int64_t)x.c_ref;
        c->cnt.subsets_calls += (int64_t)x.c_calls;
        c->cnt.cond_tests_evaluated += (int64_t)x.c_eval;
        c->cnt.alg_bytes_subsets += x.c_alg;
    }
    return FW_OK;
}


struct DhSchedPlan {
    int nt, R, nrounds;
    std::vector<int32_t> round_of;
    DhSchedPlan(const int32_t *sched, int nt_, int R_, int p) : nt(nt_), R(R_ <= 0 || R_ > nt_ ? nt_ : R_), nrounds((nt + R - 1) / R), round_of((size_t)p, 0x7fffffff)
    {
        for (int i = 0; i < nt; ++i) round_of[sched[i]] = i / R;
    }
    int first(int r) const { return r * R; }
    int count(int r) const { return std::min(nt, r * R + R) - r * R; }
};

struct DhSchedState {
    DhTgt *tg;
    int32_t *round_of;
    unsigned int *wl_cnt;
    DhLists lists;
    int32_t *ot, *ou;
    double *os, *op;
    unsigned long long *tot;
};
static DhSchedState dh_sched_state_layout(DhArena &a, size_t nt, size_t p, size_t nnz, size_t acc_d1)
{
    DhSchedState b{};
    b.tg = a.take<DhTgt>(nt);
    b.round_of = a.take<int32_t>(p);
    b.wl_cnt = a.take<unsigned int>(p);
    b.lists = dh_lists_layout(a, nnz, acc_d1, nnz);
    b.ot = a.take<int32_t>(nnz, 4);
    b.ou = a.take<int32_t>(nnz, 4);
    b.os = a.take<double>(nnz, 8);
    b.op = a.take<double>(nnz, 8);
    b.tot = a.take<unsigned long long>(8);
    return b;
}

static int dh_sched_begin(fw_ctx *c, hipStream_t st, const DhSchedState &S, const DhSchedPlan &pl, const int32_t *d_T, const int32_t *levels,
                          const long long *slot_tm, int wl_unsorted)
{
    const size_t p = pl.round_of.size();
    FW_HIP(c, hipMemsetAsync(S.tot, 0, 64, st));
    FW_HIP(c, hipMemsetAsync(S.wl_cnt, 0, 4 * p, st));
    FW_HIP(c, hipMemcpyAsync(S.round_of, pl.round_of.data(), 4 * p, hipMemcpyHostToDevice, st));
    hipLaunchKernelGGL(dh_sched_init_kernel, dim3((unsigned)((pl.nt + 255) / 256)), dim3(256), 0, st, S.tg, pl.nt, d_T, (const long long *)c->d_nb_off, levels,
                       slot_tm, wl_unsorted);
    FW_HIP(c, hipGetLastError());
    return FW_OK;
}

static void dh_sched_append(fw_ctx *c, hipStream_t st, const DhSchedState &S, const DhTgt *tg, int ntg, int round)
{
    hipLaunchKernelGGL(dh_wl_append_kernel, dim3((unsigned)((ntg + 3) / 4)), dim3(256), 0, st, tg, ntg, (const int32_t *)S.lists.pc_key,
                       (const int32_t *)S.round_of, round, S.lists.wl, (const long long *)c->d_nb_off, S.wl_cnt);
}

static int dh_sched_pack(fw_ctx *c, hipStream_t st, const DhSchedState &S, int nt)
{
    hipLaunchKernelGGL(dh_sched_pack_kernel, dim3((unsigned)((nt + 3) / 4)), dim3(256), 0, st, (const DhTgt *)S.tg, nt, (const int32_t *)S.lists.pc_key,
                       (const double *)S.lists.pc_stat, (const double *)S.lists.pc_p, S.ot, S.ou, S.os, S.op, S.tot, (double *)(S.tot + 5));
    FW_HIP(c, hipGetLastError());
    return FW_OK;
}
static int dh_sched_totals(fw_ctx *c, hipStream_t st, const DhSchedState &S, unsigned long long (&htot)[8])
{
    FW_HIP(c, hipMemcpyAsync(htot, S.tot, 64, hipMemcpyDeviceToHost, st));
    FW_HIP(c, hipStreamSynchronize(st));
    return FW_OK;
}
static int dh_sched_finish(fw_ctx *c, hipStream_t st, const DhSchedState &S, const unsigned long long (&htot)[8], size_t nnz, FwDirected &all)
{
    if (htot[4]) return fw_fail(c, FW_ERR_DEVICE, "device schedule: %llu targets did not finish", htot[4]);
    const size_t nres = (size_t)htot[0], at0 = all.size();
    if (nres > nnz) return fw_fail(c, FW_ERR_DEVICE, "device schedule: %zu result entries for %zu level-0 entries", nres, nnz);
    all.resize(at0 + nres);
    if (nres) {
        FW_HIP(c, hipMemcpyAsync(all.t.data() + at0, S.ot, 4 * nres, hipMemcpyDeviceToHost, st));
        FW_HIP(c, hipMemcpyAsync(all.u.data() + at0, S.ou, 4 * nres, hipMemcpyDeviceToHost, st));
        FW_HIP(c, hipMemcpyAsync(all.s.data() + at0, S.os, 8 * nres, hipMemcpyDeviceToHost, st));
        FW_HIP(c, hipMemcpyAsync(all.p.data() + at0, S.op, 8 * nres, hipMemcpyDeviceToHost, st));
        FW_HIP(c, hipStreamSynchronize(st));
    }
    c->cnt.cond_tests_ref += (int64_t)htot[1];
    c->cnt.subsets_calls += (int64_t)htot[2];
    c->cnt.cond_tests_evaluated += (int64_t)htot[3];
    double alg;
    memcpy(&alg, &htot[5], sizeof(double));
    c->cnt.alg_bytes_subsets += alg;
    return FW_OK;
}


struct DhSchedSizes {
    size_t nt, p, nnz, nrounds;
};
struct DhSchedBufs {
    DhSchedState S;
    int32_t *sched, *order;
    MiQueue *mq;
    MiBoard *boards;
    FwSegOut *mres;
    int32_t *bacc;
};
static DhSchedBufs dh_sched_layout(DhArena &a, const DhSchedSizes &z)
{
    DhSchedBufs b{};
    b.S = dh_sched_state_layout(a, z.nt, z.p, z.nnz, 1);
    b.sched = a.take<int32_t>(z.nt);
    b.order = a.take<int32_t>(z.nt);
    b.mq = a.take<MiQueue>(z.nrounds);
    b.boards = a.take<MiBoard>(MI_BOARD_CAP);
    b.mres = a.take<FwSegOut>(MI_REC_CAP);
    b.bacc = a.take<int32_t>(MI_BACC_CAP);
    return b;
}

int fwi_devhiton_mi_schedule(fw_ctx *c, const int32_t *sched, int nt, int R, bool feed_forward, FwDirected &all)
{
    if (nt == 0) return FW_OK;
    if (!c->d_cand || !c->d_nb_idx) return fw_fail(c, FW_ERR_STATE, "device schedule: the level-0 lists are not on the device");
    static const bool trace_host = fw_trace_host();
    const double th0 = fwi_now_s();
    hipStream_t st = c->pb[0].stream;
    const int p = c->P.p;
    const size_t nnz = (size_t)c->nb_off[p];
    const DhSchedPlan pl(sched, nt, R, p);
    const int nrounds = pl.nrounds;
    std::vector<int32_t> order((size_t)nt), deg((size_t)nt);
    std::vector<unsigned> team((size_t)nrounds, 0u);
    for (int i = 0; i < nt; ++i) deg[i] = (int32_t)(c->nb_off[sched[i] + 1] - c->nb_off[sched[i]]);
    for (int r = 0; r < nrounds; ++r) {
        const int32_t *d = deg.data() + pl.first(r);
        team[r] = dh_heaviest_first(order.data() + pl.first(r), pl.count(r), [&](int32_t i) { return d[i]; });
    }
    DhSchedBufs D;
    if (int rc = dh_arena_reserve(c, c->d_dh[0], dh_sched_layout, DhSchedSizes{(size_t)nt, (size_t)p, nnz, (size_t)nrounds}, &D)) return rc;
    DhArrays A = dh_arrays(c, c->d_cand, D.S.lists, DhLevel0{});
    A.wl_cnt = feed_forward ? D.S.wl_cnt : nullptr;
    FW_HIP(c, hipMemcpyAsync(D.sched, sched, 4 * (size_t)nt, hipMemcpyHostToDevice, st));
    FW_HIP(c, hipMemcpyAsync(D.order, order.data(), 4 * (size_t)nt, hipMemcpyHostToDevice, st));
    FW_HIP(c, hipMemsetAsync(D.mq, 0, sizeof(MiQueue) * (size_t)nrounds, st));
    if (int rc = dh_sched_begin(c, st, D.S, pl, D.sched, (const int32_t *)c->d_levels, nullptr, 1)) return rc;
    const DhParams P = dh_make_params(c, pl.R, 0, 0);
    DhEvents E(st, 2, 0);
    if (!E.ok) return fw_fail(c, FW_ERR_DEVICE, "device schedule: hipEventCreate failed");
    const double th1 = fwi_now_s();
    FW_HIP(c, hipEventRecord(E.ev[0], st));
    std::vector<unsigned> grids((size_t)nrounds, 0u);
    for (int r = 0; r < nrounds; ++r) {
        const int r0 = pl.first(r), ntg = pl.count(r);
        FW_HIP(c, hipMemsetAsync(D.boards, 0, sizeof(MiBoard) * MI_BOARD_CAP, st));
        grids[r] = dh_mi_launch(c, st, D.S.tg + r0, ntg, (const int32_t *)(D.order + r0), A, P, team[r], trace_host, D.mq + r, D.boards, D.mres, D.bacc);
        if (feed_forward && r + 1 < nrounds) dh_sched_append(c, st, D.S, D.S.tg + r0, ntg, r);
    }
    FW_HIP(c, hipGetLastError());
    FW_HIP(c, hipEventRecord(E.ev[1], st));
    if (int rc = dh_sched_pack(c, st, D.S, nt)) return rc;
    std::vector<MiQueue> hq((size_t)nrounds);
    FW_HIP(c, hipMemcpyAsync(hq.data(), D.mq, sizeof(MiQueue) * (size_t)nrounds, hipMemcpyDeviceToHost, st));
    unsigned long long htot[8] = {0, 0, 0, 0, 0, 0, 0, 0};
    if (int rc = dh_sched_totals(c, st, D.S, htot)) return rc;
    const double th2 = fwi_now_s();
    for (int r = 0; r < nrounds; ++r)
        if (int rc = dh_mi_check(c, hq[r], grids[r], r, pl.count(r), trace_host)) return rc;
    float ms = 0.0f;
    FW_HIP(c, hipEventElapsedTime(&ms, E.ev[0], E.ev[1]));
    if (int rc = dh_sched_finish(c, st, D.S, htot, nnz, all)) return rc;
    c->cnt.t_dev_subsets_s += 1e-3 * (double)ms;
    c->cnt.subsets_launches += nrounds;
    c->cnt.kernel_launches += 2 * nrounds + 1;
    if (trace_host)
        fprintf(stderr, "[fw] device schedule: %d targets in %d rounds, set-up %.2f ms, launches + download %.2f ms (kernels %.2f ms), results %.2f ms\n", nt, nrounds,
                1e3 * (th1 - th0), 1e3 * (th2 - th1), (double)ms, 1e3 * (fwi_now_s() - th2));
    return FW_OK;
}


struct DhFzChainSizes {
    size_t ntg, max_ns, tm_floats;
};
struct DhFzSizes {
    size_t nt, p, nnz, d1, nslots;
    int K;
    DhFzChainSizes ch[FW_DH_MAX_CHAINS];
};
struct DhFzBufs {
    DhSchedState S;
    int32_t *slot_T;
    long long *slot_tm;
    unsigned int *wl_max;
    DhRoundScratch ch[FW_DH_MAX_CHAINS];
};
static DhFzBufs dh_fz_layout(DhArena &a, const DhFzSizes &z)
{
    DhFzBufs b{};
    b.S = dh_sched_state_layout(a, z.nt, z.p, z.nnz, z.d1);
    b.slot_T = a.take<int32_t>(z.nt);
    b.slot_tm = a.take<long long>(z.nt);
    b.wl_max = a.take<unsigned int>(z.nslots);
    for (int q = 0; q < z.K; ++q) b.ch[q] = dh_scratch_layout(a, z.ch[q].ntg, z.ch[q].max_ns, z.ch[q].tm_floats);
    return b;
}

struct DhFzBarrier {
    std::mutex m;
    std::condition_variable cv;
    int n, waiting = 0, rc = FW_OK;
    unsigned gen = 0;
    explicit DhFzBarrier(int k) : n(k) {}
    int arrive(int my_rc)
    {
        std::unique_lock<std::mutex> lk(m);
        if (my_rc && !rc) rc = my_rc;
        const unsigned g = gen;
        if (++waiting == n) {
            waiting = 0;
            ++gen;
            cv.notify_all();
        } else {
            cv.wait(lk, [&] { return gen != g; });
        }
        return rc;
    }
};

struct DhFzSlot {
    int base = 0, ntg = 0, max_cap = 0;
    unsigned max_ns = 0;
    size_t tm_floats = 0;
};

int fwi_devhiton_fz_schedule(fw_ctx *c, const int32_t *sched, int nt, int R, bool feed_forward, FwDirected &all)
{
    if (nt == 0) return FW_OK;
    if (!c->d_cand || !c->d_nb_idx || !c->d_nb_off) return fw_fail(c, FW_ERR_STATE, "device schedule: the level-0 lists are not on the device");
    static const bool trace_host = fw_trace_host();
    const double th0 = fwi_now_s();
    const int p = c->P.p;
    const size_t nnz = (size_t)c->nb_off[p];
    const DhSchedPlan pl(sched, nt, R, p);
    const int nrounds = pl.nrounds;
    int K = 1;
    for (int r = 0; r < nrounds; ++r) K = std::max(K, fwi_chain_count(c, (size_t)pl.count(r)));
    std::vector<DhFzSlot> slots((size_t)nrounds * (size_t)K);
    std::vector<int32_t> slot_T((size_t)nt);
    std::vector<long long> slot_tm((size_t)nt);
    DhFzSizes z{(size_t)nt, (size_t)p, nnz, 0, (size_t)nrounds * (size_t)K, K, {}};
    {
        std::vector<int> chain_of;
        std::vector<size_t> chain_idx;
        for (int r = 0; r < nrounds; ++r) {
            const int r0 = pl.first(r), n = pl.count(r);
            const int Kr = fwi_chain_count(c, (size_t)n);
            fwi_deal_chains((size_t)n, Kr, chain_of, chain_idx);
            DhFzSlot *s = &slots[(size_t)r * (size_t)K];
            for (int i = 0; i < n; ++i) ++s[chain_of[i]].ntg;
            for (int q = 0, base = r0; q < K; ++q) {
                s[q].base = base;
                base += s[q].ntg;
            }
            for (int i = 0; i < n; ++i) slot_T[(size_t)s[chain_of[i]].base + chain_idx[i]] = sched[r0 + i];
            for (int q = 0; q < K; ++q) {
                if (s[q].ntg == 0) continue;
                const DhPolicy y = dh_policy(c, s[q].ntg);
                z.d1 = (size_t)y.spec_depth + 1;
                for (int t = 0; t < s[q].ntg; ++t) {
                    const int T = slot_T[(size_t)(s[q].base + t)];
                    const int deg = (int)(c->nb_off[T + 1] - c->nb_off[T]);
                    s[q].max_cap = std::max(s[q].max_cap, deg);
                    slot_tm[(size_t)(s[q].base + t)] = dh_tm_off(c, y, deg, s[q].tm_floats);
                }
                s[q].max_ns = dh_max_ns(y, s[q].ntg);
                z.ch[q].ntg = std::max(z.ch[q].ntg, (size_t)s[q].ntg);
                z.ch[q].max_ns = std::max(z.ch[q].max_ns, (size_t)s[q].max_ns);
                z.ch[q].tm_floats = std::max(z.ch[q].tm_floats, s[q].tm_floats);
            }
        }
    }
    DhFzBufs D;
    if (int rc = dh_arena_reserve(c, c->d_dh[0], dh_fz_layout, z, &D)) return rc;
    hipStream_t sts[FW_DH_MAX_CHAINS];
    for (int q = 0; q < K; ++q) {
        if (q > 0 && !c->dh_stream[q]) FW_HIP(c, hipStreamCreateWithFlags(&c->dh_stream[q], hipStreamNonBlocking));
        sts[q] = q == 0 ? c->pb[0].stream : c->dh_stream[q];
        if (int rc = fw_pin_reserve(c, c->h_dh[q], 4096)) return rc;
    }
    static_assert(2 * sizeof(DhGlobal) <= 3072, "the pinned page holds two batch records and, at byte 3072, the whitelist word");
    hipStream_t st = sts[0];
    DhEvents X(st, 0, 3 * K);
    if (!X.ok) return fw_fail(c, FW_ERR_DEVICE, "device schedule: hipEventCreate failed");
    const DhArrays A = dh_arrays(c, c->d_cand, D.S.lists, DhLevel0{});
    FW_HIP(c, hipMemsetAsync(D.wl_max, 0, 4 * z.nslots, st));
    FW_HIP(c, hipMemcpyAsync(D.slot_T, slot_T.data(), 4 * (size_t)nt, hipMemcpyHostToDevice, st));
    FW_HIP(c, hipMemcpyAsync(D.slot_tm, slot_tm.data(), 8 * (size_t)nt, hipMemcpyHostToDevice, st));
    if (int rc = dh_sched_begin(c, st, D.S, pl, D.slot_T, nullptr, D.slot_tm, 0)) return rc;
    for (int q = 1; q < K; ++q) {
        FW_HIP(c, hipEventRecord(X.ev_end[(size_t)q * 3], st));
        FW_HIP(c, hipStreamWaitEvent(sts[q], X.ev_end[(size_t)q * 3], 0));
    }
    const double th1 = fwi_now_s();
    DhFzBarrier bar(K);
    std::vector<double> t_start((size_t)nrounds, 0.0);
    auto chain_round = [&](int q, int r, DhEvents &E) -> int {
        const DhFzSlot &s = slots[(size_t)r * (size_t)K + (size_t)q];
        hipStream_t sq = sts[q];
        if (r > 0)
            for (int o = 0; o < K; ++o)
                if (o != q) FW_HIP(c, hipStreamWaitEvent(sq, X.ev_end[(size_t)o * 3 + (size_t)((r - 1) & 1)], 0));
        if (q == 0) t_start[(size_t)r] = fwi_now_s() - th0;
        DhRun Rn{c, q, s.ntg, sq, trace_host, dh_policy(c, s.ntg)};
        Rn.use_devc = true;
        Rn.dev_wl = true;
        Rn.max_cap = s.max_cap;
        Rn.max_ns = s.max_ns;
        Rn.tm_floats = s.tm_floats;
        Rn.D.tg = D.S.tg + s.base;
        Rn.D.s = D.ch[q];
        if (!s.tm_floats) Rn.D.s.tmat = nullptr;
        const DhRoundScratch &cb = Rn.D.s;
        Rn.A = A;
        Rn.A.tmat = cb.tmat;
        Rn.hg = (DhGlobal *)c->h_dh[q].ptr;
        memset(Rn.hg, 0, 2 * sizeof(DhGlobal));
        unsigned int *h_wl_max = (unsigned int *)((char *)c->h_dh[q].ptr + 3072);
        unsigned int *d_wl_max = D.wl_max + (size_t)r * (size_t)K + (size_t)q;
        hipLaunchKernelGGL(dh_fz_round_begin_kernel, dim3((unsigned)s.ntg), dim3(256), 0, sq, Rn.D.tg, s.ntg, (const unsigned int *)D.S.wl_cnt, D.S.lists.wl,
                           cb.g, cb.seg0, cb.act, d_wl_max);
        FW_HIP(c, hipGetLastError());
        if (feed_forward && r > 0) {
            FW_HIP(c, hipMemcpyAsync(h_wl_max, d_wl_max, sizeof(unsigned int), hipMemcpyDeviceToHost, sq));
            FW_HIP(c, hipEventRecord(X.ev_end[(size_t)q * 3 + 2], sq));
        }
        if (cb.tmat) {
            hipLaunchKernelGGL(dh_tmat_build_kernel, dim3((unsigned)s.ntg, 8u), dim3(256), 0, sq, (const DhTgt *)Rn.D.tg, s.ntg, A.nb_idx,
                               (const float *)c->d_cor, p, cb.tmat);
            FW_HIP(c, hipGetLastError());
        }
        Rn.P = dh_make_params(c, s.ntg, Rn.y.spec_depth, Rn.y.spec0_depth);
        if (feed_forward && r > 0) {
            FW_HIP(c, hipEventSynchronize(X.ev_end[(size_t)q * 3 + 2]));
            Rn.max_wl = (int)*h_wl_max;
        }
        int rc = DhRounds(Rn, E).run();
        const bool append = !rc && feed_forward && r + 1 < nrounds;
        dh_count_run(Rn, 1 + (cb.tmat ? 1 : 0) + (append ? 1 : 0));
        if (rc) return rc;
        if (append) {
            dh_sched_append(c, sq, D.S, Rn.D.tg, s.ntg, r);
            FW_HIP(c, hipGetLastError());
        }
        return FW_OK;
    };
    auto chain_body = [&](int q) {
        DhEvents E(sts[q], 2 * 2 * DH_BATCH, 2);
        int rc = E.ok ? FW_OK : fw_fail(c, FW_ERR_DEVICE, "device schedule: hipEventCreate failed");
        for (int r = 0; r < nrounds; ++r) {
            if (!rc && slots[(size_t)r * (size_t)K + (size_t)q].ntg > 0) rc = chain_round(q, r, E);
            if (!rc && hipEventRecord(X.ev_end[(size_t)q * 3 + (size_t)(r & 1)], sts[q]) != hipSuccess)
                rc = fw_fail(c, FW_ERR_DEVICE, "device schedule: hipEventRecord failed");
            if ((rc = bar.arrive(rc))) break;
        }
    };
    {
        std::vector<std::thread> th;
        for (int q = 1; q < K; ++q)
            th.emplace_back([&, q] {
                (void)hipSetDevice(c->P.device);
                chain_body(q);
            });
        chain_body(0);
        for (std::thread &t : th) t.join();
    }
    if (bar.rc) return bar.rc;
    const double th2 = fwi_now_s();
    if (int rc = dh_sched_pack(c, st, D.S, nt)) return rc;
    unsigned long long htot[8] = {0, 0, 0, 0, 0, 0, 0, 0};
    if (int rc = dh_sched_totals(c, st, D.S, htot)) return rc;
    if (int rc = dh_sched_finish(c, st, D.S, htot, nnz, all)) return rc;
    c->cnt.kernel_launches += 2;
    if (trace_host) {
        fprintf(stderr, "[fw] fz device schedule: %d targets in %d rounds on %d chains, set-up %.2f ms, rounds %.2f ms, results %.2f ms; rounds start at", nt,
                nrounds, K, 1e3 * (th1 - th0), 1e3 * (th2 - th1), 1e3 * (fwi_now_s() - th2));
        for (int r = 0; r < nrounds; ++r) fprintf(stderr, " %.2f", 1e3 * t_start[(size_t)r]);
        fprintf(stderr, " ms\n");
    }
    return FW_OK;
}
```

flashweave.jl_amd/csrc/fw_fz.hip:

```cpp
#include "fw_csc.h"
#include "fw_cscres.h"
#include "fw_internal.h"
#include "fw_unrank.h"

#include <algorithm>
#include <rocprim/device/device_scan.hpp>
#include <cmath>

__global__ __launch_bounds__(256) void fz_center_kernel(const float *__restrict__ data, float *__restrict__ xc,
                                                        float *__restrict__ sd, int n, int p, int n_pad)
{
    const int v = blockIdx.x;
    float *dst = xc + (size_t)v * n_pad;
    __shared__ double s_red[4];
    if (v >= p) {
        for (int i = threadIdx.x; i < n_pad; i += 256) dst[i] = 0.0f;
        if (threadIdx.x == 0) sd[v] = 0.0f;
        return;
    }
    const float *src = data + (size_t)v * n;
    double s = 0.0;
    for (int i = threadIdx.x; i < n; i += 256) s += (double)src[i];
    for (int o = 32; o > 0; o >>= 1) s += __shfl_xor(s, o);
    if ((threadIdx.x & 63) == 0) s_red[threadIdx.x >> 6] = s;
// ... 620 lines not shown
    ctx->cor_rows_world = world;
    ctx->cor_rows_per_rank = *rows_per_rank;
    return FW_OK;
}

int fwi_fz_level0(fw_ctx *ctx, std::vector<int32_t> &pi, std::vector<int32_t> &pj, std::vector<double> &stat,
                  std::vector<double> &pval, int64_t *m_reliable, FwL0Dev *dev)
{
    if (dev) *dev = FwL0Dev{};
    const int p = ctx->P.p;
    const long long npairs = (long long)p * (p - 1) / 2;
    if (ctx->P.n < ctx->n_obs_min_eff) {
        pi.clear();
        pj.clear();
        stat.clear();
        pval.clear();
        *m_reliable = 0;
        return FW_OK;
    }
    {
        int rc0 = fz_ensure_thresholds(ctx, ctx->stream);
        if (rc0) return rc0;
    }
    unsigned long long cap = (unsigned long long)std::min<long long>(npairs, 4ll << 20);
    if (cap < ctx->l0_cap_hint) cap = ctx->l0_cap_hint;
    if (cap == 0) cap = 1;
    FzL0Counters h{};
    for (int attempt = 0; attempt < 2; ++attempt) {
        int rc;
        if ((rc = fw_dev_reserve(ctx, ctx->d_tmp0, 2 * sizeof(FzL0Counters)))) return rc;
        if ((rc = fw_dev_reserve(ctx, ctx->d_tmp1, cap * (2 * sizeof(int32_t) + sizeof(float))))) return rc;
        if ((rc = fw_dev_reserve(ctx, ctx->d_tmp2, cap * sizeof(double)))) return rc;
        if ((rc = fw_dev_reserve(ctx, ctx->d_jobs, cap * (2 * sizeof(int32_t) + sizeof(float))))) return rc;
        FW_HIP(ctx, hipMemsetAsync(ctx->d_tmp0.ptr, 0, 2 * sizeof(FzL0Counters), ctx->stream));
        FzL0Counters *d_c1 = (FzL0Counters *)ctx->d_tmp0.ptr, *d_c2 = d_c1 + 1;
        int32_t *oi = (int32_t *)ctx->d_tmp1.ptr;
        int32_t *oj = oi + cap;
        float *orr = (float *)(oj + cap);
        double *op = (double *)ctx->d_tmp2.ptr;
        int32_t *ci = (int32_t *)ctx->d_jobs.ptr;
        int32_t *cj = ci + cap;
        float *cr = (float *)(cj + cap);
        if (ctx->P.no_cor_mat) {
            const int n = ctx->P.n;
            ctx->n_pad = (n + GEMM_BK - 1) / GEMM_BK * GEMM_BK;
            ctx->p_pad = (p + GEMM_BM - 1) / GEMM_BM * GEMM_BM;
            if (!ctx->d_xc) FW_HIP(ctx, hipMalloc(&ctx->d_xc, sizeof(float) * (size_t)ctx->n_pad * ctx->p_pad));
            if (!ctx->d_sd) FW_HIP(ctx, hipMalloc(&ctx->d_sd, sizeof(float) * (size_t)ctx->p_pad));
            if (attempt == 0)
                hipLaunchKernelGGL(fz_center_kernel, dim3(ctx->p_pad), dim3(256), 0, ctx->stream, ctx->d_data, ctx->d_xc, ctx->d_sd, n, p,
                                   ctx->n_pad);
            const int T = ctx->p_pad / GEMM_BM;
            hipLaunchKernelGGL(fz_cor_gemm_kernel<true>, dim3((unsigned)(T * (T + 1) / 2)), dim3(256), 0, ctx->stream, ctx->d_xc, ctx->d_sd,
                               (float *)nullptr, p, ctx->n_pad, T, 0, 0, (const double *)ctx->d_thr, d_c1, cap, ci, cj, cr);
        } else {
            dim3 grid((p + FZ_L0_COLS - 1) / FZ_L0_COLS, (p + FZ_L0_ROWS - 1) / FZ_L0_ROWS);
            hipLaunchKernelGGL(fz_level0_kernel, grid, dim3(256), 0, ctx->stream, ctx->d_cor, p, (const double *)ctx->d_thr, d_c1, cap, ci,
                               cj, cr);
        }
        FW_HIP(ctx, hipGetLastError());
        FzL0Counters h1{};
        FW_HIP(ctx, hipMemcpyAsync(&h1, d_c1, sizeof(h1), hipMemcpyDeviceToHost, ctx->stream));
        FW_HIP(ctx, hipStreamSynchronize(ctx->stream));
        if (h1.n_sig > ctx->l0_cap_hint) ctx->l0_cap_hint = h1.n_sig;
        if (h1.n_sig > cap) {
            cap = h1.n_sig;
            continue;
        }
        if (h1.n_sig)
            hipLaunchKernelGGL(fz_level0_exact_kernel, dim3((unsigned)((h1.n_sig + 255) / 256)), dim3(256), 0, ctx->stream,
                               (const int32_t *)ci, (const int32_t *)cj, (const float *)cr, h1.n_sig, ctx->P.alpha, fz_zscale(ctx),
                               d_c2, cap, oi, oj, orr, op);
        FW_HIP(ctx, hipGetLastError());
        FW_HIP(ctx, hipMemcpyAsync(&h, d_c2, sizeof(h), hipMemcpyDeviceToHost, ctx->stream));
        FW_HIP(ctx, hipStreamSynchronize(ctx->stream));
        h.n_nan = h1.n_nan;
        ctx->cnt.kernel_launches += 2;
        if (h.n_sig <= cap) {
            const size_t k = (size_t)h.n_sig;
            if (dev) {
                dev->i = oi;
                dev->j = oj;
                dev->stat32 = orr;
                dev->pval = op;
                dev->k = k;
                *m_reliable = npairs - (long long)h.n_nan;
                return FW_OK;
            }
            pi.resize(k);
            pj.resize(k);
            stat.resize(k);
            pval.resize(k);
            std::vector<float> rr(k);
            if (k) {
                FW_HIP(ctx, hipMemcpy(pi.data(), oi, k * sizeof(int32_t), hipMemcpyDeviceToHost));
                FW_HIP(ctx, hipMemcpy(pj.data(), oj, k * sizeof(int32_t), hipMemcpyDeviceToHost));
                FW_HIP(ctx, hipMemcpy(rr.data(), orr, k * sizeof(float), hipMemcpyDeviceToHost));
                FW_HIP(ctx, hipMemcpy(pval.data(), op, k * sizeof(double), hipMemcpyDeviceToHost));
            }
            for (size_t t = 0; t < k; ++t) stat[t] = (double)rr[t];
            *m_reliable = npairs - (long long)h.n_nan;
            return FW_OK;
        }
        cap = h.n_sig;
    }
    return fw_fail(ctx, FW_ERR_DEVICE, "fz level-0: compaction buffer overflow twice");
}

int fwi_fz_test_batch(fw_ctx *ctx, int64_t m, const int32_t *X, const int32_t *Y, const int64_t *zoff,
                      const int32_t *zflat, fw_test_result *out)
{
    if (m == 0) return FW_OK;
    const int64_t nz = zoff[m];
    int rc;
    if ((rc = fw_dev_reserve(ctx, ctx->d_jobs, (size_t)m * 2 * sizeof(int32_t) + (size_t)(m + 1) * sizeof(int64_t)))) return rc;
    if ((rc = fw_dev_reserve(ctx, ctx->d_acc, (size_t)(nz > 0 ? nz : 1) * sizeof(int32_t)))) return rc;
    if ((rc = fw_dev_reserve(ctx, ctx->d_out, (size_t)m * sizeof(fw_test_result)))) return rc;
    long long *dz = (long long *)ctx->d_jobs.ptr;
    int32_t *dX = (int32_t *)(dz + m + 1);
    int32_t *dY = dX + m;
    FW_HIP(ctx, hipMemcpyAsync(dz, zoff, (size_t)(m + 1) * sizeof(int64_t), hipMemcpyHostToDevice, ctx->stream));
    FW_HIP(ctx, hipMemcpyAsync(dX, X, (size_t)m * sizeof(int32_t), hipMemcpyHostToDevice, ctx->stream));
    FW_HIP(ctx, hipMemcpyAsync(dY, Y, (size_t)m * sizeof(int32_t), hipMemcpyHostToDevice, ctx->stream));
    if (nz > 0)
        FW_HIP(ctx, hipMemcpyAsync(ctx->d_acc.ptr, zflat, (size_t)nz * sizeof(int32_t), hipMemcpyHostToDevice, ctx->stream));
    int kmax = 0;
    for (int64_t t = 0; t < m; ++t) kmax = std::max<int>(kmax, (int)(zoff[t + 1] - zoff[t]));
    if (kmax > FW_MAX_K_FAST)
        hipLaunchKernelGGL(fz_test_batch_kernel<true>, dim3((unsigned)((m + 255) / 256)), dim3(256), 0, ctx->stream, ctx->d_cor,
                           ctx->P.p, (long long)m, dX, dY, dz, (const int32_t *)ctx->d_acc.ptr, fz_zscale(ctx),
                           (fw_test_result *)ctx->d_out.ptr);
    else
        hipLaunchKernelGGL(fz_test_batch_kernel<false>, dim3((unsigned)((m + 255) / 256)), dim3(256), 0, ctx->stream, ctx->d_cor,
                           ctx->P.p, (long long)m, dX, dY, dz, (const int32_t *)ctx->d_acc.ptr, fz_zscale(ctx),
                           (fw_test_result *)ctx->d_out.ptr);
    FW_HIP(ctx, hipGetLastError());
    FW_HIP(ctx, hipMemcpyAsync(out, ctx->d_out.ptr, (size_t)m * sizeof(fw_test_result), hipMemcpyDeviceToHost, ctx->stream));
    FW_HIP(ctx, hipStreamSynchronize(ctx->stream));
    ctx->cnt.kernel_launches += 1;
    const bool power = ctx->P.n >= ctx->n_obs_min_eff;
    if (!power)
        for (int64_t t = 0; t < m; ++t) {
            out[t].stat = 0.0;
            out[t].pval = 1.0;
            out[t].df = 0;
            out[t].suff_power = 0;
        }
    return FW_OK;
}

#ifdef FW_FZ_FASTDBG
extern "C" void fwi_fz_fastdbg_print()
{
    unsigned long long c[24] = {0};
    if (hipMemcpyFromSymbol(c, HIP_SYMBOL(fz_fast_cnt), sizeof(c)) == hipSuccess && c[19])
        fprintf(stderr, "[fw] cheap-screen potential: of %llu fast-loop wave-iterations, every lane clearly (relative margin on |stat|^2: 2e-4 / 2e-3 / 2e-2) above the wavefront's minimum so far and inside the sure range in %llu / %llu / %llu\n",
                c[19], c[16], c[17], c[18]);
    if (c[23])
        fprintf(stderr, "[fw] cheap screen (validation build: decides nothing): lanes it would skip %llu, of them VIOLATIONS (exact value not above the bound, or not sure) %llu; wave-iterations it would skip whole %llu of %llu\n",
                c[20], c[21], c[22], c[23]);
    if (hipMemcpyFromSymbol(c, HIP_SYMBOL(fz_fast_cnt), sizeof(c)) == hipSuccess)
        fprintf(stderr, "[fw] fast loop: wave-iterations %llu, lane-tests %llu; waves with a lane not clean %llu, not significant-for-sure %llu, beyond the normal range of p %llu, behind a stop %llu, tie %llu; lanes beyond the normal range %llu\n",
                c[0], c[1], c[2], c[3], c[4], c[5], c[6], c[7]);
    if (c[8])
        fprintf(stderr, "[fw] segments (table variant) %llu, evaluated %llu; 100 MHz ticks per segment (first wavefront): prologue %.1f, table build %.1f, lane loop %.1f, reductions %.1f, whole body %.1f\n",
                c[8], c[14], (double)c[9] / c[8], (double)c[10] / c[8], (double)c[11] / c[8], (double)c[12] / c[8], (double)c[13] / c[8]);
}
#endif
static int fz_ensure_thresholds(fw_ctx *ctx, hipStream_t stream)
{
    if (!ctx->d_thr) {
        const int flags = fw_knob_int(knob::FW_FZ_DBG, 0);
        FW_HIP(ctx, hipMemcpyToSymbol(HIP_SYMBOL(fz_dbg_flags), &flags, sizeof(int)));
        FW_HIP(ctx, hipMalloc((void **)&ctx->d_thr, 12 * sizeof(double)));
        hipLaunchKernelGGL(fz_thresholds_kernel, dim3(1), dim3(64), 0, stream, ctx->P.alpha, fz_zscale(ctx), ctx->d_thr);
        FW_HIP(ctx, hipGetLastError());
        FW_HIP(ctx, hipStreamSynchronize(stream));
    }
    return FW_OK;
}

int fwi_fz_thresholds(fw_ctx *ctx, hipStream_t stream, double *zscale)
{
    *zscale = fz_zscale(ctx);
    return fz_ensure_thresholds(ctx, stream);
}

int fwi_fz_segments_dev(fw_ctx *ctx, unsigned grid, const FwSeg *d_segs, const int32_t *d_acc, FwSegOut *d_out, const unsigned *d_ns,
                        bool any_big, const unsigned *d_big, hipStream_t stream)
{
    int rc = fz_ensure_thresholds(ctx, stream);
    if (rc) return rc;
    const unsigned grid_big = grid < 512u ? grid : 512u;
    if (ctx->P.max_k > 3) {
        const bool no_hk = fw_no_hk();
        if (!no_hk)
            hipLaunchKernelGGL((fz_subsets_seg_kernel<true, false, true>), dim3(grid), dim3(256), 0, stream, ctx->d_cor, ctx->P.p, d_segs,
                               d_acc, d_out, ctx->P.max_k, ctx->P.alpha, fz_zscale(ctx), (long long)ctx->P.max_tests, ctx->d_thr,
                               (const FwNzJob *)nullptr, 0ll, d_ns, d_big);
        hipLaunchKernelGGL((fz_subsets_seg_kernel<true, false, false>), dim3(grid), dim3(256), 0, stream, ctx->d_cor,
                           ctx->P.p, d_segs, d_acc, d_out, ctx->P.max_k, ctx->P.alpha, fz_zscale(ctx), (long long)ctx->P.max_tests,
                           ctx->d_thr, (const FwNzJob *)nullptr, 0ll, d_ns, no_hk ? (const unsigned *)nullptr : d_big);
    } else {
        hipLaunchKernelGGL((fz_subsets_seg_kernel<false, false, true>), dim3(grid), dim3(256), 0, stream, ctx->d_cor, ctx->P.p, d_segs,
                           d_acc, d_out, ctx->P.max_k, ctx->P.alpha, fz_zscale(ctx), (long long)ctx->P.max_tests, ctx->d_thr,
                           (const FwNzJob *)nullptr, 0ll, d_ns, d_big);
        if (any_big)
            hipLaunchKernelGGL((fz_subsets_seg_kernel<false, false, false>), dim3(grid_big), dim3(256), 0, stream, ctx->d_cor, ctx->P.p,
                               d_segs, d_acc, d_out, ctx->P.max_k, ctx->P.alpha, fz_zscale(ctx), (long long)ctx->P.max_tests,
                               ctx->d_thr, (const FwNzJob *)nullptr, 0ll, d_ns, d_big);
    }
    FW_HIP(ctx, hipGetLastError());
    return FW_OK;
}

int fwi_fz_segments(fw_ctx *ctx, int64_t nseg, int64_t nseg_tab, const FwSeg *d_segs, const int32_t *d_acc, FwSegOut *d_out,
                    FwPoolBuf &pb)
{
    if (nseg == 0) return FW_OK;
    FW_HIP(ctx, hipEventRecord(pb.ev0, pb.launch_stream));
    {
        int rc = fz_ensure_thresholds(ctx, pb.launch_stream);
        if (rc) return rc;
    }
    if (ctx->P.max_k > FW_MAX_K_FAST) {
        hipLaunchKernelGGL(fz_subsets_slow_kernel<false>, dim3((unsigned)nseg), dim3(256), 0, pb.launch_stream, ctx->d_cor, ctx->P.p, d_segs, d_acc,
                           d_out, ctx->P.max_k, ctx->P.alpha, fz_zscale(ctx), (long long)ctx->P.max_tests, (const FwNzJob *)nullptr, 0ll);
    } else if (ctx->P.max_k > 3) {
        if (nseg_tab > 0)
            hipLaunchKernelGGL((fz_subsets_seg_kernel<true, false, true>), dim3((unsigned)nseg_tab), dim3(256), 0, pb.launch_stream,
                               ctx->d_cor, ctx->P.p, d_segs, d_acc, d_out, ctx->P.max_k, ctx->P.alpha, fz_zscale(ctx),
                               (long long)ctx->P.max_tests, ctx->d_thr, (const FwNzJob *)nullptr, 0ll, (const unsigned *)nullptr, (const unsigned *)nullptr);
        if (nseg > nseg_tab)
            hipLaunchKernelGGL((fz_subsets_seg_kernel<true, false, false>), dim3((unsigned)(nseg - nseg_tab)), dim3(256), 0,
                               pb.launch_stream, ctx->d_cor, ctx->P.p, d_segs + nseg_tab, d_acc, d_out + nseg_tab, ctx->P.max_k,
                               ctx->P.alpha, fz_zscale(ctx), (long long)ctx->P.max_tests, ctx->d_thr, (const FwNzJob *)nullptr,
                               0ll, (const unsigned *)nullptr, (const unsigned *)nullptr);
    } else {
        if (nseg_tab > 0)
            hipLaunchKernelGGL((fz_subsets_seg_kernel<false, false, true>), dim3((unsigned)nseg_tab), dim3(256), 0, pb.launch_stream,
                               ctx->d_cor, ctx->P.p, d_segs, d_acc, d_out, ctx->P.max_k, ctx->P.alpha, fz_zscale(ctx),
                               (long long)ctx->P.max_tests, ctx->d_thr, (const FwNzJob *)nullptr, 0ll, (const unsigned *)nullptr, (const unsigned *)nullptr);
        if (nseg > nseg_tab)
            hipLaunchKernelGGL((fz_subsets_seg_kernel<false, false, false>), dim3((unsigned)(nseg - nseg_tab)), dim3(256), 0,
                               pb.launch_stream, ctx->d_cor, ctx->P.p, d_segs + nseg_tab, d_acc, d_out + nseg_tab, ctx->P.max_k,
                               ctx->P.alpha, fz_zscale(ctx), (long long)ctx->P.max_tests, ctx->d_thr, (const FwNzJob *)nullptr,
                               0ll, (const unsigned *)nullptr, (const unsigned *)nullptr);
    }
    FW_HIP(ctx, hipGetLastError());
    FW_HIP(ctx, hipEventRecord(pb.ev1, pb.launch_stream));
    return FW_OK;
}



template <bool CSC>
struct FznzCol;
template <>
struct FznzCol<false> {
    const float *c;
    struct Word {};
    __device__ __forceinline__ FznzCol(const float *data, const unsigned long long *, const uint32_t *, int n, int, int v) : c(data + (size_t)v * n) {}
    __device__ __forceinline__ Word word(int) const { return Word{}; }
    __device__ __forceinline__ float at(Word, int row) const { return c[row]; }
    __device__ __forceinline__ float at_set(Word, int row) const { return c[row]; }
    __device__ __forceinline__ float at(int row) const { return c[row]; }
};
template <>
struct FznzCol<true> {
    const unsigned long long *m;
    const uint32_t *b;
    const float *vals;
    struct Word {
        unsigned long long m;
        uint32_t b;
    };
    __device__ __forceinline__ FznzCol(const float *vals_, const unsigned long long *nz, const uint32_t *cbase, int, int W, int v)
        : m(nz + (size_t)v * W), b(cbase + (size_t)v * W), vals(vals_)
    {
    }
    __device__ __forceinline__ Word word(int w) const { return Word{m[w], b[w]}; }
    __device__ __forceinline__ float at(Word wd, int row) const { return fw_cscres_word_value(wd.m, wd.b, vals, row & 63); }
    __device__ __forceinline__ float at_set(Word wd, int row) const { return vals[fw_cscres_pos(wd.m, wd.b, row & 63)]; }
    __device__ __forceinline__ float at(int row) const { return fw_cscres_value(m, b, vals, row); }
};

template <bool CSC>
__global__ __launch_bounds__(256) void fznz_level0_kernel(const float *__restrict__ data, const unsigned long long *__restrict__ nz,
                                                          const uint32_t *__restrict__ cbase, int n, int p, int W, double alpha, long long n_obs_min,
                                                          FzL0Counters *cnt, unsigned long long cap, int32_t *out_i,
                                                          int32_t *out_j, double *out_s, double *out_p)
{
    const int X = blockIdx.y * 16 + (threadIdx.x >> 4), Y = blockIdx.x * 16 + (threadIdx.x & 15);
    if (blockIdx.x * 16 + 15 <= blockIdx.y * 16) return;
    const bool valid = X < Y && Y < p;
    const FznzCol<CSC> cx(data, nz, cbase, n, W, valid ? X : 0), cy(data, nz, cbase, n, W, valid ? Y : 0);
    const unsigned long long *mx = nz + (size_t)(valid ? X : 0) * W, *my = nz + (size_t)(valid ? Y : 0) * W;
    double sum_x = 0.0, sum_y = 0.0;
    long long nn = 0;
    for (int w = 0; w < W; ++w) {
        unsigned long long m = valid ? (mx[w] & my[w]) : 0ull;
        nn += __popcll(m);
        const typename FznzCol<CSC>::Word wx = cx.word(w), wy = cy.word(w);
        while (m) {
            const int row = w * 64 + __builtin_ctzll(m);
            m &= m - 1;
            sum_x += (double)cx.at_set(wx, row);
// ... 918 lines not shown
```

flashweave.jl_amd/csrc/fw_fz_core.h:

```cpp
#pragma once
#include "fw_internal.h"
#include "fw_unrank.h"

static __device__ __noinline__ double fz_pval_slow(double r, double zscale)
{
    double z = (zscale > 0.0) ? zscale * log((1.0 + r) / (1.0 - r)) : 0.0;
    double cc = erfc(fabs(z) * 0.7071067811865476) / 2.0;
    const double p = cc * 2.0;
    return p < 2.2250738585072014e-308 ? 0.0 : p;
}
static __device__ __noinline__ double fz_xkey_slow(double r, double zscale)
{
    return fabs(zscale * log((1.0 + r) / (1.0 - r))) * 0.7071067811865476;
}

__device__ __forceinline__ double fz_pval_dev(double r, double zscale )
{
    double z = (zscale > 0.0) ? zscale * log((1.0 + r) / (1.0 - r)) : 0.0;
    double cc = erfc(fabs(z) * 0.7071067811865476) / 2.0;
    const double p = cc * 2.0;
    return p < 2.2250738585072014e-308 ? 0.0 : p;
}

__device__ __forceinline__ float round5_f32(float x)
// ... 329 lines not shown
    const double denom = d1 * d2c;
    const double v = (denom == 0.0) ? 0.0 : fz_div_nn(ev, denom);
    return fz_clamp_unit_nn(v);
}

__device__ __forceinline__ double pc_l3_nn(double a, double b, double c)
{
    const double ev = round5_f64_nn(a - b * c);
    const double xb = 1.0 - b * b, xc = 1.0 - c * c;
    const double denom = fz_sqrt_unit_raw(xb) * fz_sqrt_unit_raw(xc);
    const double v = (xb == 0.0 || xc == 0.0) ? 0.0 : fz_div_nn(ev, denom);
    return fz_clamp_unit_nn(v);
}

static __device__ __noinline__ double fz_l3_finish(double ev, double xb, double xc)
{
    const double denom = fz_sqrt_unit_raw(xb) * fz_sqrt_unit_raw(xc);
    const double v = (xb == 0.0 || xc == 0.0) ? 0.0 : fz_div_nn(ev, denom);
    return fz_clamp_unit_nn(v);
}

__device__ __forceinline__ double pc_l3(double a, double b, double c)
{
    const double ev = round5_f64(a - b * c);
    const double denom = fz_sqrt_unit(1.0 - b * b) * fz_sqrt_unit(1.0 - c * c);
    double v = (denom == 0.0) ? 0.0 : ev / denom;
    v = v < -1.0 ? -1.0 : v;
    v = v >= 1.0 ? 1.0 : v;
    return v;
}

#ifndef FW_FZ_FASTLOOP
#define FW_FZ_FASTLOOP 1
#endif
#ifndef FW_L3_ENTRY_NN
#define FW_L3_ENTRY_NN 1
#endif
#ifndef FW_FZ_INTERLEAVE
#define FW_FZ_INTERLEAVE 1
#endif
#ifndef FW_RUN_MAX
#define FW_RUN_MAX 32
#endif
#ifndef FW_FZ_SCREEN
#define FW_FZ_SCREEN 1
#endif
#ifndef FW_FZ_CHEAPRED
#define FW_FZ_CHEAPRED 1
#endif
#ifndef FW_RUN_MAX3
#define FW_RUN_MAX3 64
#endif
#define FZ_TAB_A FW_TAB_A
#define FZ_TAB_CAP 1024
#define FZ_TAB_ZMASK 0x0FFFFFFF
__device__ __forceinline__ int fz_tab_off(int i, int i0, int a)
{
    return (i - i0) * (a - 1) - (i * (i - 1) - i0 * (i0 - 1)) / 2;
}
#define FZ_X_NONE 1.0e308
#define FZ_X_SUB 26.0
#define FZ_X_SUBKEY 1.0e300
#define FZ_X_LAZY (-1.0)

__device__ __forceinline__ bool fz_key_better(double xa, double pa, unsigned long long ra, double xb, double pb,
                                              unsigned long long rb)
{
    if (xa != xb) return xa < xb;
    if (xa == FZ_X_NONE) return false;
    if (pa != pb) return pa > pb;
    return ra > rb;
}

static __device__ void fz_thresholds_dev(double alpha, double zscale, double *thr)
{
    for (int sgn = 0; sgn < 2; ++sgn) {
        double lo = 0.0, hi = 1.0;
        const double sg = sgn ? -1.0 : 1.0;
        if (!(fz_pval_dev(sg * 1.0, zscale) < alpha)) {
            thr[2 * sgn] = 2.0;
            thr[2 * sgn + 1] = 2.0;
            continue;
        }
        for (int it = 0; it < 200; ++it) {
            const double mid = 0.5 * (lo + hi);
            if (fz_pval_dev(sg * mid, zscale) < alpha)
                hi = mid;
            else
                lo = mid;
        }
        thr[2 * sgn] = lo * (1.0 - 1e-9);
        thr[2 * sgn + 1] = hi * (1.0 + 1e-9);
    }
}


#define FZ_HK_A FW_HK_A
#define FZ_HK_CAP 4096
#define FZ_HK_DIR 96
__device__ __forceinline__ double pc_l3s(double a, double b, double c, double sb, double sc)
{
    const double ev = round5_f64(a - b * c);
    const double denom = sb * sc;
    double v = (denom == 0.0) ? 0.0 : ev / denom;
    v = v < -1.0 ? -1.0 : v;
    v = v >= 1.0 ? 1.0 : v;
    return v;
}
__device__ __forceinline__ double pc_l3s_nn(double a, double b, double c, double sb, double sc)
{
    const double ev = round5_f64_nn(a - b * c);
    const double denom = sb * sc;
    const double v = (denom == 0.0) ? 0.0 : fz_div_nn(ev, denom);
    return fz_clamp_unit_nn(v);
}
__device__ __forceinline__ double fz_sq1(double v) { return fz_sqrt_unit(1.0 - v * v); }
__device__ __forceinline__ int fz_hk_entries(int n) { return 1 + 2 * n + n * (n - 1) / 2; }
__device__ __forceinline__ unsigned int fz_hk_tests(int n, int t)
{
    const unsigned int u = (unsigned int)n;
    if (n < t) return 0u;
    const unsigned int h = u * (u - 1u) / 2u;
    return t == 2 ? h : h * (u - 2u) / 3u;
}

template <bool NN>
__device__ __forceinline__ double fz_hk_stat(const double *__restrict__ tb, int n, int s, int l3, int l4, int l5)
{
#define HK_L3(a, b, c, sb, sc) (NN ? pc_l3s_nn(a, b, c, sb, sc) : pc_l3s(a, b, c, sb, sc))
    const double *tx = tb + 1, *ty = tb + 1 + n, *tp = tb + 1 + 2 * n;
    const double XY = tb[0], X3 = tx[l3], Y3 = ty[l3], X4 = tx[l4], Y4 = ty[l4];
    const double P43 = tp[l4 * (l4 - 1) / 2 + l3];
    const double sX3 = fz_sq1(X3), sY3 = fz_sq1(Y3), s43 = fz_sq1(P43);
    const double T_XY = HK_L3(XY, X3, Y3, sX3, sY3);
    const double T_X4 = HK_L3(X4, X3, P43, sX3, s43);
    const double T_Y4 = HK_L3(Y4, Y3, P43, sY3, s43);
    const double sX4 = fz_sq1(T_X4), sY4 = fz_sq1(T_Y4);
    if (s == 4) return HK_L3(T_XY, T_X4, T_Y4, sX4, sY4);
    const int o5 = l5 * (l5 - 1) / 2;
    const double X5 = tx[l5], Y5 = ty[l5], P54 = tp[o5 + l4], P53 = tp[o5 + l3];
    const double s53 = fz_sq1(P53);
    const double T_X5 = HK_L3(X5, X3, P53, sX3, s53);
    const double T_Y5 = HK_L3(Y5, Y3, P53, sY3, s53);
    const double T_54 = HK_L3(P54, P53, P43, s53, s43);
    const double s54 = fz_sq1(T_54);
    const double Q_XY = HK_L3(T_XY, T_X4, T_Y4, sX4, sY4);
    const double Q_X5 = HK_L3(T_X5, T_X4, T_54, sX4, s54);
    const double Q_Y5 = HK_L3(T_Y5, T_Y4, T_54, sY4, s54);
    return HK_L3(Q_XY, Q_X5, Q_Y5, fz_sq1(Q_X5), fz_sq1(Q_Y5));
#undef HK_L3
}

#define FZ_L1_A 512
#ifdef FW_FZ_FASTDBG
static __device__ unsigned long long fz_fast_cnt[24];
#endif
static __device__ int fz_dbg_flags;
template <int K>
__device__ __forceinline__ double fz_l1t_stat(const float *__restrict__ cor, int p, const float4 *__restrict__ tab,
                                              const unsigned char *__restrict__ tabf, const int *__restrict__ acc, const int *pos,
                                              double a1v, bool a1f, bool clean )
{
    constexpr int M = K + 2;
    double R[M][M];
    bool is32[M][M];
    float c[K - 1], r[K - 1];
    int zid[K - 1];
    R[0][1] = a1v;
    is32[0][1] = a1f;
#pragma unroll
    for (int t = 0; t < K - 1; ++t) {
        const int pp = pos[K - 1 - t];
        const float4 e = tab[pp];
        const int f = tabf[pp];
        R[0][2 + t] = (double)e.x;
        is32[0][2 + t] = (f & 1) != 0;
        R[1][2 + t] = (double)e.y;
        is32[1][2 + t] = (f & 2) != 0;
        c[t] = e.z;
        r[t] = e.w;
        zid[t] = acc[pp];
    }
#pragma unroll
    for (int t = 0; t < K - 1; ++t)
#pragma unroll
        for (int u = t + 1; u < K - 1; ++u) {
#ifdef FW_CORT_TRANSPOSED
            const TV v = pc_l1_r(cor[(size_t)zid[u] * p + zid[t]], c[t], c[u], r[t], r[u]);
#else
            const TV v = pc_l1_r(cor[(size_t)zid[t] * p + zid[u]], c[t], c[u], r[t], r[u]);
#endif
            R[2 + t][2 + u] = v.v;
            is32[2 + t][2 + u] = v.f32;
            clean = clean && v.v == v.v;
        }
#ifndef FW_L1T_NO_NN
    if (__all(clean)) return fz_pcor_levels<K, true>(R, is32);
#endif
    return fz_pcor_levels<K, false>(R, is32);
}

#ifndef FZ_L3_CAP
#define FZ_L3_CAP 448
#endif
#define FZ_L3_DIR 64

template <bool HIGHK, bool LOCAL, bool TAB>
__device__ __forceinline__ void fz_seg_body(const float *__restrict__ cor_g, int p_g, const FwSeg seg ,
                                            const int32_t *__restrict__ gacc ,
                                            const bool remote_acc ,
                                            FwSegOut *out_rec, int max_k,
                                            double alpha, double zscale_g, long long max_tests,
                                            const double *__restrict__ thr_g, const FwNzJob *__restrict__ recs,
                                            long long n_obs_min)
{
    constexpr bool TAB3 = TAB && !HIGHK;
    constexpr bool HK = TAB && HIGHK && !LOCAL;
    static_assert(!(TAB && HIGHK && LOCAL), "no level-2 table variant for per-job matrices");
    constexpr bool L1T = HIGHK && !TAB && !LOCAL;
#ifndef FW_FZ_L1T_ROW32
#define FW_FZ_L1T_ROW32 1
#endif
#ifndef FW_FZ_TMAT_HIGHK
#define FW_FZ_TMAT_HIGHK 1
#endif
#ifndef FW_L3_SCREEN
#define FW_L3_SCREEN 0
#endif
    constexpr bool SCR = TAB3 || (L1T && FW_L3_SCREEN != 0);
    constexpr int ACC_LDS = TAB3 ? FZ_TAB_A : (HK ? FZ_HK_A + 8 : (L1T ? FZ_L1_A : FW_ACC_LDS));
    __shared__ int s_acc[ACC_LDS];
    __shared__ float4 s_l1[L1T ? FZ_L1_A : 1];
    __shared__ unsigned char s_l1f[L1T ? FZ_L1_A : 1];
    __shared__ double s_l1a;
    __shared__ int s_l1af, s_l1nan;
    __shared__ float s3_p2[L1T ? FZ_L3_CAP : 1], s3_r2[L1T ? FZ_L3_CAP : 1];
    __shared__ unsigned char s3_fl[L1T ? FZ_L3_CAP : 1];
    __shared__ double s3_blk[L1T ? 8 * FZ_L3_CAP : 1];
    double *const s3_d2c = s3_blk, *const s3_q3 = s3_blk + (L1T ? FZ_L3_CAP : 0), *const s3_sq3 = s3_blk + (L1T ? 2 * FZ_L3_CAP : 0),
                  *const s3_x3 = s3_blk + (L1T ? 3 * FZ_L3_CAP : 0), *const s3_sx3 = s3_blk + (L1T ? 4 * FZ_L3_CAP : 0), *const s3_y3 = s3_blk + (L1T ? 5 * FZ_L3_CAP : 0),
                  *const s3_sy3 = s3_blk + (L1T ? 6 * FZ_L3_CAP : 0), *const s3_a4 = s3_blk + (L1T ? 7 * FZ_L3_CAP : 0);
    __shared__ int s3_off[L1T ? FZ_L3_DIR + 1 : 2], s3_low[L1T ? FZ_L3_DIR : 1], s3_jk[L1T ? FZ_L3_DIR : 1];
    __shared__ float s3_bp2[L1T ? FZ_L3_DIR : 1];
    __shared__ unsigned char s3_bfl[L1T ? FZ_L3_DIR : 1];
    __shared__ double s3_bd2c[L1T ? FZ_L3_DIR : 1], s3_bx2[L1T ? FZ_L3_DIR : 1], s3_bsx2[L1T ? FZ_L3_DIR : 1], s3_by2[L1T ? FZ_L3_DIR : 1],
        s3_bsy2[L1T ? FZ_L3_DIR : 1], s3_ba3[L1T ? FZ_L3_DIR : 1];
    __shared__ int s3_n, s3_lin0, s3_okf, s3_dirty;
    __shared__ unsigned long long s3_end;
    __shared__ double s_hk[HK ? FZ_HK_CAP : 1];
    __shared__ int s_hk_off[HK ? FZ_HK_DIR + 1 : 2];
    __shared__ unsigned short s_hk_ij[HK ? FZ_HK_DIR : 1];
    __shared__ unsigned long long s_hk_end;
    __shared__ int s_hk_n, s_hk_lin0, s_hk_nan, s_hk_skip0, s_hk_prev;
    __shared__ unsigned int s_cstop;
    __shared__ unsigned int s_scrq;
    __shared__ unsigned long long s_stop[4];
    __shared__ double s_bx[4], s_bps[4];
    __shared__ unsigned long long s_br[4];
    __shared__ unsigned int s_evc[4];
    __shared__ double s_best_x, s_best_ps, s_best_stat;
    __shared__ unsigned long long s_best_rank;
    __shared__ float4 s_tab[TAB3 ? FZ_TAB_CAP : 1];
    __shared__ float s_tab_r1[TAB3 ? FZ_TAB_CAP : 1];
    __shared__ float2 s_tab_r2[TAB3 ? FZ_TAB_CAP : 1];
    __shared__ double s_tab_a2[TAB3 ? FZ_TAB_CAP : 1];
    __shared__ int s_blk[2];

#ifdef FW_FZ_FASTDBG
    const unsigned long long dbg_t0 = __builtin_amdgcn_s_memtime();
    unsigned long long dbg_t1 = 0, dbg_tab = 0, dbg_loop = 0, dbg_red = 0;
#endif
    const int a = seg.acc_len;
    const int tid = threadIdx.x, lane = tid & 63, wave = tid >> 6;
    const bool in_lds = a <= (TAB3 ? FZ_TAB_A : (HK ? FZ_HK_A : (L1T ? FZ_L1_A : FW_ACC_LDS)));
    const float *cor = cor_g;
    int p = p_g;
    double zscale = zscale_g;
    const double *thr = thr_g;
    if (LOCAL) {
        const FwNzJob *rec = recs + seg.pad;
        cor = cor_g + rec->cor_off;
        p = rec->m;
        zscale = rec->zscale;
        thr = rec->thr;
        if ((long long)rec->nR < n_obs_min) {
            if (tid == 0) {
                FwSegOut o;
                o.stop_rank = 0;
                o.stop_stat = 0.0;
                o.stop_pval = 1.0;
                o.best_rank = 0;
                o.best_stat = 0.0;
                o.best_pval = -1.0;
                o.stop_df = -2;
                o.stop_power = 0;
                o.best_df = 0;
                o.pad = 0;
                o.evaluated = 0;
                *out_rec = o;
            }
            return;
        }
    } else if (in_lds) {
        if (remote_acc)
            for (int i = tid; i < a; i += 256) s_acc[i] = __hip_atomic_load(gacc + i, __ATOMIC_RELAXED, __HIP_MEMORY_SCOPE_AGENT);
        else
            for (int i = tid; i < a; i += 256) s_acc[i] = gacc[i];
    }
    int Xl = -1, Yl = -1;
    bool tloc = false;
    if (!LOCAL && seg.tm != 0ull && (TAB3 || (FW_FZ_TMAT_HIGHK && ((HK && FW_FZ_TMAT_HIGHK != 2) || L1T) && in_lds))) {
        int32_t *s_ids = TAB3 ? (int32_t *)s_tab : (HK ? (int32_t *)s_hk : (int32_t *)s3_blk);
        if (!TAB3) tloc = true;
        const int32_t *ids = (const int32_t *)seg.tm_ids;
        const int nid = seg.tm_m - 1;
        for (int i = tid; i < nid; i += 256) s_ids[i] = ids[i];
        __syncthreads();
        auto local_of = [&](int v) -> int {
            if (v == seg.X) return 0;
            int lo = 0, hi = nid - 1;
            while (lo < hi) {
                const int mid = (lo + hi) >> 1;
                if (s_ids[mid] < v)
                    lo = mid + 1;
                else
                    hi = mid;
            }
            if (nid <= 0 || s_ids[lo] != v) __builtin_trap();
            return lo + 1;
        };
        for (int i = tid; i < a; i += 256) s_acc[i] = local_of(s_acc[i]);
        Xl = 0;
        Yl = local_of(seg.Y);
        cor = cor_g + (((long long)seg.tm - (long long)(unsigned long long)cor_g) >> 2);
        p = seg.tm_m;
        __syncthreads();
    }
    if (tid == 0) {
        s_best_x = FZ_X_NONE;
        s_best_ps = 0.0;
        s_best_stat = 0.0;
        s_best_rank = 0;
        s_cstop = 0xffffffffu;
        s_scrq = 0x7f7fffffu;
        if (HK) s_hk_prev = -1;
    }
    unsigned long long cnt[FW_MAX_K_FAST + 1];
#pragma unroll
    for (int s = FW_MAX_K_FAST; s >= 1; --s)
        cnt[s] = (s <= max_k) ? (TAB3 ? (unsigned long long)fw_binom32(a, s) : binom_u64(a, s)) : 0ull;
    const double rlo_pos = thr[0], rhi_pos = thr[1], rlo_neg = thr[2], rhi_neg = thr[3];
    const double rsub_lo = !LOCAL ? thr[4] : (zscale > 0.0 ? tanh(FZ_X_SUB * 0.7071067811865476 / zscale) * (1.0 - 1e-9) : 2.0);
    const double h2_pos = !LOCAL ? thr[5] : rhi_pos * rhi_pos * (1.0 + 1e-12), h2_neg = !LOCAL ? thr[6] : rhi_neg * rhi_neg * (1.0 + 1e-12);
    const double s2 = !LOCAL ? thr[7] : (rsub_lo < 1.0 ? rsub_lo * rsub_lo : 1.0) * (1.0 - 1e-12);
    const float scr_h2 = __int_as_float(__builtin_amdgcn_readfirstlane(__float_as_int((float)(h2_pos > h2_neg ? h2_pos : h2_neg) * 1.00001f)));
    __syncthreads();
#define ACCV(i) (LOCAL ? ((i) + 2) : (in_lds ? s_acc[(i)] : gacc[(i)]))
#define CORV(u, v) cor[(size_t)(u) * p + (v)]
#ifndef FW_CORT_TAB3
#define FW_CORT_TAB3 1
#endif
#ifdef FW_CORT_TRANSPOSED
#define CORT(u, v) (LOCAL ? CORV(u, v) : CORV(v, u))
#else
#define CORT(u, v) ((FW_CORT_TAB3 && TAB3 && !LOCAL) ? CORV(v, u) : ((FW_FZ_TMAT_HIGHK && HIGHK && !LOCAL) ? cor[(size_t)(tloc ? (v) : (u)) * p + (tloc ? (u) : (v))] : CORV(u, v)))
#endif

    const int X = LOCAL ? 0 : (Xl >= 0 ? Xl : seg.X), Y = LOCAL ? 1 : (Yl >= 0 ? Yl : seg.Y);
    const float cXY = CORV(X, Y);
    const unsigned long long NONE = FW_RANK_NONE;
    const unsigned long long len = seg.end - seg.start;
    constexpr int RMAX = (TAB && !HIGHK) ? FW_RUN_MAX3 : FW_RUN_MAX;
    const int R = (int)((len + 255) / 256 < RMAX ? (len + 255) / 256 : RMAX);
    unsigned long long evaluated = 0;

    unsigned long long cnext = seg.start;
    for (unsigned long long cbase = seg.start; cbase < seg.end; cbase = cnext) {
#ifdef FW_FZ_FASTDBG
        const unsigned long long dbg_c0 = __builtin_amdgcn_s_memtime();
        if (!dbg_t1) dbg_t1 = dbg_c0;
#endif
        unsigned long long cend = cbase + 256ull * R;
        cend = cend < seg.end ? cend : seg.end;
        int Rc = R;
        bool hk_ok = false, hk_nn = false;
        int hk_s = 0, hk_lin0 = 0;
        if (HK) {
            unsigned long long rem0 = cbase;
            int s0 = max_k;
            while (s0 > 1 && rem0 >= cnt[s0]) {
                rem0 -= cnt[s0];
                --s0;
            }
            if (s0 >= 4) {
                if (tid == 0) {
                    int q[FW_MAX_K_FAST];
                    fw_unrank_comb32((uint32_t)rem0, a, s0, q);
                    int i = q[0], j = q[1];
                    unsigned long long cur_end = (unsigned long long)(fw_binom32(a, s0) - fw_binom32(a - i, s0)) +
                                                 (unsigned long long)(fw_binom32(a - 1 - i, s0 - 1) - fw_binom32(a - j, s0 - 1)) +
                                                 (unsigned long long)fz_hk_tests(a - 1 - j, s0 - 2);
                    unsigned long long lim = rem0 + 256ull * FW_RUN_MAX;
                    if (lim > rem0 + (seg.end - cbase)) lim = rem0 + (seg.end - cbase);
                    if (lim > cnt[s0]) lim = cnt[s0];
                    const int ij0 = (s0 << 16) | (i << 8) | j;
                    s_hk_skip0 = (ij0 == s_hk_prev) ? 1 : 0;
                    s_hk_prev = ij0;
                    s_hk_lin0 = i * (a - s0 + 1) - i * (i - 1) / 2 + (j - i - 1);
                    int nd = 0, eoff = 0;
                    for (;;) {
                        const int e = fz_hk_entries(a - 1 - j);
                        if (nd > 0 && eoff + e > FZ_HK_CAP) {
                            lim = cur_end - (unsigned long long)fz_hk_tests(a - 1 - j, s0 - 2);
                            break;
                        }
                        s_hk_ij[nd] = (unsigned short)((i << 8) | j);
                        s_hk_off[nd] = eoff;
                        eoff += e;
                        ++nd;
                        if (cur_end >= lim) break;
                        if (nd == FZ_HK_DIR) {
                            lim = cur_end;
                            break;
                        }
                        if (++j > a - s0 + 1) {
                            ++i;
                            j = i + 1;
                        }
                        cur_end += (unsigned long long)fz_hk_tests(a - 1 - j, s0 - 2);
                    }
                    s_hk_off[nd] = eoff;
                    s_hk_n = nd;
                    s_hk_end = cbase + (lim - rem0);
                    if (!s_hk_skip0) s_hk_nan = 0;
                }
                __syncthreads();
                const int nd = s_hk_n, etot = s_hk_off[nd];
                cend = s_hk_end;
                hk_ok = true;
                hk_s = s0;
                hk_lin0 = s_hk_lin0;
                for (int e = (s_hk_skip0 ? s_hk_off[1] : 0) + tid; e < etot; e += 256) {
                    int d = 0;
                    for (int w = 64; w > 0; w >>= 1)
                        if (d + w < nd && s_hk_off[d + w] <= e) d += w;
                    const int ij = s_hk_ij[d], i = ij >> 8, j = ij & 255, n = a - 1 - j;
                    int l = e - s_hk_off[d];
                    int A, B;
                    if (l == 0) {
                        A = X;
                        B = Y;
                    } else if (l <= 2 * n) {
                        A = l <= n ? X : Y;
                        B = ACCV(j + 1 + (l <= n ? l - 1 : l - 1 - n));
                    } else {
                        l -= 1 + 2 * n;
                        int pl = (int)((1.0f + sqrtf(1.0f + 8.0f * (float)l)) * 0.5f);
                        while (pl * (pl - 1) / 2 > l) --pl;
                        while ((pl + 1) * pl / 2 <= l) ++pl;
                        A = ACCV(j + 1 + pl);
                        B = ACCV(j + 1 + (l - pl * (pl - 1) / 2));
                    }
                    const int z1 = ACCV(i), z2 = ACCV(j);
                    const float cAz1 = CORV(A, z1), cBz1 = CORV(B, z1), cz2z1 = CORV(z2, z1);
                    const TV RAB = pc_l1(CORV(A, B), cAz1, cBz1);
                    const TV RA2 = pc_l1(CORV(A, z2), cAz1, cz2z1);
                    const TV RB2 = pc_l1(CORV(B, z2), cBz1, cz2z1);
                    const double v = pc_l2(RAB, RA2, RB2);
                    s_hk[e] = v;
                    if (!(v == v)) s_hk_nan = 1;
                }
                __syncthreads();
                hk_nn = s_hk_nan == 0;
                const unsigned long long clen = cend - cbase;
                Rc = (int)((clen + 255ull) / 256ull);
            }
        }
        bool l1_ok = false, l1_clean = false, l3_ok = false, l3_nn = false;
        int l1_s = 0, l3_lin0 = 0, l3_i = 0;
        if (L1T && in_lds && a <= FZ_L1_A && !(fz_dbg_flags & 1)) {
            unsigned long long rem0 = cbase;
            int s0 = max_k;
            while (s0 > 1 && rem0 >= cnt[s0]) {
                rem0 -= cnt[s0];
                --s0;
            }
            if (s0 >= 4 && rem0 + (cend - cbase) <= cnt[s0]) {
                if (tid == 0) s_l1nan = 0;
                if (tid == 0 || tid == 64) {
// ... 925 lines not shown
```

flashweave.jl_amd/csrc/fw_internal.h:

```cpp
#pragma once
#if defined(__HIP_DEVICE_COMPILE__) && !defined(__gfx950__)
#error "libflashweave_amd targets gfx950 only (make ARCH=gfx950)"
#endif
#include <hip/hip_runtime.h>

#include <cstdint>
#include <cstdlib>
#include <cstdio>
#include <cstring>
#include <string>
#include <vector>

#include "../../include/flashweave_amd.h"
#include "fw_graph.h"

struct FwDevBuf {
    void *ptr = nullptr;
    size_t cap = 0;
};

struct FwPinned {
    void *ptr = nullptr;
    size_t cap = 0;
};

template <typename T> class FwDevArray {
    T *p_ = nullptr;

public:
    FwDevArray() = default;
    FwDevArray(FwDevArray &&o) noexcept : p_(o.release()) {}
    FwDevArray &operator=(FwDevArray &&o) noexcept
    {
        if (this != &o) {
            if (p_) (void)hipFree(p_);
            p_ = o.release();
        }
        return *this;
    }
    FwDevArray(const FwDevArray &) = delete;
    FwDevArray &operator=(const FwDevArray &) = delete;
    ~FwDevArray()
    {
        if (p_) (void)hipFree(p_);
    }
    hipError_t alloc(size_t count)
    {
        *this = FwDevArray();
        return hipMalloc((void **)&p_, sizeof(T) * count);
    }
    hipError_t upload(const T *src, size_t count)
    {
        const hipError_t e = alloc(count);
        return e != hipSuccess ? e : hipMemcpy(p_, src, sizeof(T) * count, hipMemcpyHostToDevice);
    }
    hipError_t upload(const std::vector<T> &v) { return upload(v.data(), v.size()); }
    hipError_t download(T *dst, size_t count) const { return hipMemcpy(dst, p_, sizeof(T) * count, hipMemcpyDeviceToHost); }
    hipError_t download(std::vector<T> &v) const { return download(v.data(), v.size()); }
    T *get() const { return p_; }
    T *release()
    {
        T *p = p_;
        p_ = nullptr;
        return p;
    }
};

inline bool fw_is_dev_ptr(const void *q, int device)
{
    if (!q) return false;
    hipPointerAttribute_t a;
    if (hipPointerGetAttributes(&a, q) != hipSuccess) {
        (void)hipGetLastError();
        return false;
    }
    return a.type == hipMemoryTypeDevice && a.device == device;
}

struct FwJob {
    int32_t X;
    int32_t Y;
    int64_t acc_off;
    int32_t acc_len;
    int32_t pad;
};

#define FW_MAX_K_FAST 5

struct FwJobOut {
    double stat;
    double pval;
    int64_t num_tests;
    int64_t evaluated;
    int32_t df;
    int32_t suff_power;
    int32_t status;
    int32_t n_zs;
    int32_t zs[FW_MAX_K];
    int32_t pad[3];
};

struct FwSeg {
    int32_t X;
    int32_t Y;
    int64_t acc_off;
    int32_t acc_len;
    int32_t pad;
    uint64_t start;
    uint64_t end;
    uint64_t tm, tm_ids;
    int32_t tm_m, pad1;
};

#define FW_RANK_NONE (~0ull)
#define FW_TAB_A 512
#ifndef FW_HK_A
#define FW_HK_A 88
#endif

struct FwNzJob {
    int32_t X, Y;
    long long acc_off;
    int32_t acc_len;
    int32_t m;
    long long cor_off;
    int32_t nR;
    int32_t pad;
    double zscale;
    double rxy;
    double thr[4];
};

struct FwSegOut {
    uint64_t stop_rank;
    double stop_stat;
    double stop_pval;
    uint64_t best_rank;
    double best_stat;
    double best_pval;
    int32_t stop_df;
    int32_t stop_power;
    int32_t best_df;
    int32_t pad;
    uint64_t evaluated;
};

struct FwL0Dev {
    const int32_t *i = nullptr, *j = nullptr;
    const double *stat64 = nullptr;
    const float *stat32 = nullptr;
    const double *pval = nullptr;
    size_t k = 0;
};

struct FwPoolBuf {
    hipStream_t stream = nullptr;
    hipEvent_t ev0 = nullptr, ev1 = nullptr;
    hipEvent_t evd = nullptr;
    hipStream_t launch_stream = nullptr;
    FwPinned h_in, h_out;
    FwDevBuf d_in, d_out;
    FwDevBuf d_acc;
};

struct FwComm;

struct fw_ctx {
    fw_params P{};
    FwComm *comm = nullptr;
    int64_t n_obs_min_eff = 0;
    mutable std::string err;
    hipStream_t stream = nullptr;
    hipEvent_t ev0 = nullptr, ev1 = nullptr;

    float *d_data = nullptr;
    float *d_xc = nullptr;
    float *d_sd = nullptr;
    float *d_cor = nullptr;
    bool cor_external = false;
    int64_t cor_capacity = 0;
    int cor_rows_rank = -1, cor_rows_world = 0;
    int64_t cor_rows_per_rank = 0;
    double *d_thr = nullptr;
    double *d_fzs_stat = nullptr;
    uint64_t gram_epoch = 0;
    bool have_fzs_stat = false;
    int n_pad = 0, p_pad = 0;
    bool have_data = false, have_cor = false;
    bool f64 = false;
    bool f32_input = false;
    double *d_data64 = nullptr, *d_xc64 = nullptr, *d_sd64 = nullptr, *d_cor64 = nullptr;

    std::vector<int32_t> levels, max_vals;
    int L = 0;
    int elim_mode = 0;
    int mi_view = 0;
    int l0_rank = 0, l0_world = 1;
    double *d_gthr = nullptr;
    int gthr_n = 0;
    int mi_nxy = 2;
    int W = 0;
    uint64_t *d_nzbits = nullptr;
    uint64_t *d_hibits = nullptr;
    int32_t *d_levels = nullptr, *d_maxvals = nullptr;
    unsigned char *d_vals = nullptr;
    bool mi_generic = false;
    long long mig_gtab_words = 0;
    FwDevBuf d_mig_tab[3];
    bool csc_resident = false;
    uint32_t *d_cbase = nullptr;
    float *d_cvals = nullptr;
    int64_t cvals_n = 0;
    bool fznz_lds_raised_csc = false;
    bool fznz_lds_raised = false;
    float *d_xlnx = nullptr;
    int32_t *d_firstnz = nullptr;

    bool have_level0 = false;
    std::vector<int64_t> nb_off;
    std::vector<int32_t> nb_idx;
    std::vector<double> nb_stat, nb_p;

    bool have_network = false;
    FwHostWorkers *host_workers = nullptr;
    FwNetwork net;

    int track_rej = 0;
    bool have_rej = false;
    std::vector<fw_rejection> rej, rej_slots;
    FwDevBuf d_rej;
    fw_rejection *d_rej_run = nullptr;
    size_t rej_n_last = 0;
    int rej_rank = 0, rej_world = 1;
    bool rej_gathered = false;
    std::vector<int64_t> rej_slot;
    std::vector<uint8_t> rej_host;
    FwDevBuf d_rej_x;
    int64_t rej_packed_host = 0, rej_packed_dev = 0, rej_received = 0;

    fw_counters cnt{};

    FwDevBuf d_jobs, d_acc, d_out, d_tmp0, d_tmp1, d_tmp2, d_segs, d_segout, d_nzrecs, d_arena;
    FwDevBuf d_l0m_i, d_l0m_d;
    FwDevBuf d_bh;
    const long long *d_nb_off = nullptr;
    const int32_t *d_nb_idx = nullptr;
    const double *d_nb_stat = nullptr, *d_nb_p = nullptr;
    const int32_t *d_cand = nullptr;
    unsigned long long l0_cap_hint = 0;
    bool nb_host_valid = true;
#define FW_DH_MAX_CHAINS 4
    FwDevBuf d_dh[FW_DH_MAX_CHAINS];
    FwPinned h_dh[FW_DH_MAX_CHAINS];
    hipStream_t dh_stream[FW_DH_MAX_CHAINS] = {nullptr, nullptr, nullptr, nullptr};
    hipStream_t dh_hp_stream[FW_DH_MAX_CHAINS] = {nullptr, nullptr, nullptr, nullptr};
    hipEvent_t dh_hp_ev[FW_DH_MAX_CHAINS][2] = {{nullptr, nullptr}, {nullptr, nullptr}, {nullptr, nullptr}, {nullptr, nullptr}};
    FwPinned h_jobs, h_acc, h_out;
    FwPoolBuf pb[2];
};

#include "fw_knobs.h"

int fw_fail(const fw_ctx *ctx, int code, const char *fmt, ...);
int fw_dev_reserve(fw_ctx *ctx, FwDevBuf &b, size_t bytes);
int fw_pin_reserve(fw_ctx *ctx, FwPinned &b, size_t bytes);

#define FW_HIP(ctx, call)                                                                        \
    do {                                                                                         \
        hipError_t e__ = (call);                                                                 \
        if (e__ != hipSuccess)                                                                   \
            return fw_fail(ctx, FW_ERR_DEVICE, "%s failed: %s (%s:%d)", #call, hipGetErrorString(e__), \
// ... 144 lines not shown
```

Before: 83.80 billion.

## Maintain local matrix indices alongside accepted lists to skip per-segment binary search

Keeps a parallel array of local (sub-matrix) indices next to the global candidate and accepted lists. The indices are computed once in the tmat build kernel and carried through advance, commit and speculative copies. The fz kernel then reads precomputed local ids through a shifted acc offset and a new tm_y field, so each segment no longer loads ids into LDS, binary-searches every accepted entry, and adds two syncthreads. In exchange, every list write becomes a double write and extra buffers are allocated; the step kernel also gains a launch-bounds occupancy hint.

```diff
diff --git a/flashweave.jl_amd/csrc/fw_devhiton.hip b/flashweave.jl_amd/csrc/fw_devhiton.hip
--- a/flashweave.jl_amd/csrc/fw_devhiton.hip
+++ b/flashweave.jl_amd/csrc/fw_devhiton.hip
@@ -64,6 +64,11 @@
     const double *nb_stat, *nb_p;
     const float *tmat;
     fw_rejection *rej;
+};
+
+struct DhLoc {
+    const int32_t *cand0;
+    int32_t *tpc, *acc;
 };
 
 struct DhParams {
@@ -198,10 +203,29 @@
     return bytes;
 }
 
-__device__ bool dh_advance(DhTgt &x, const DhArrays &A, int lane, int d1, bool keep_elim_stats = false)
-{
+
+template <bool LOC>
+__device__ __forceinline__ bool dh_has_loc(const DhTgt &x, const DhLoc &L)
+{
+    return LOC && L.acc != nullptr && x.tm_off >= 0;
+}
+__device__ __forceinline__ int32_t dh_cand_loc(const DhTgt &x, const DhLoc &L, int q)
+{
+    return (x.phase == 0 ? L.cand0 : L.tpc)[x.co + q];
+}
+__device__ __forceinline__ void dh_acc_put(const DhArrays &A, const DhLoc &L, long long at, int32_t v, bool loc, int32_t vl)
+{
+    A.acc[at] = v;
+    if (loc) L.acc[at] = vl;
+}
+
+template <bool LOC>
+__device__ __forceinline__ bool dh_advance_impl(DhTgt &x, const DhArrays &A, int lane, int d1, bool keep_elim_stats, const DhLoc &L)
+{
+    const bool loc = dh_has_loc<LOC>(x, L);
     for (;;) {
-        int32_t *acc = A.acc + DH_ACC_OFF(x, x.cur, d1);
+        const long long ao = DH_ACC_OFF(x, x.cur, d1);
+        int32_t *acc = A.acc + ao;
         if (x.phase == 2) return false;
         const int32_t *cands = x.phase == 0 ? A.cand0 + x.cand_off : A.tpc_key + x.co;
         int32_t *dkey = (x.phase == 0 ? A.tpc_key : A.pc_key) + x.co;
@@ -210,10 +234,12 @@
         int32_t &dn = x.phase == 0 ? x.ntpc : x.npc;
         while (x.pos < x.nc) {
             const int32_t cand = cands[x.pos];
+            const int32_t candl = loc ? dh_cand_loc(x, L, x.pos) : 0;
             if (x.wl_n > 0 && dh_in_wl(x, A, cand)) {
                 if (lane == 0) {
-                    acc[x.na] = cand;
+                    dh_acc_put(A, L, ao + x.na, cand, loc, candl);
                     dkey[dn] = cand;
+                    if (loc && x.phase == 0) L.tpc[x.co + dn] = candl;
                     dstat[dn] = NAN;
                     dp[dn] = NAN;
                 }
@@ -229,9 +255,10 @@
                 for (int base = 0; base < x.na; base += 64) {
                     const int q = base + lane;
                     const int32_t v = q < x.na ? acc[q] : cand;
+                    const int32_t vl = (loc && q < x.na) ? L.acc[ao + q] : 0;
                     const bool keep = q < x.na && v != cand;
                     const unsigned long long m = __ballot(keep);
-                    if (keep) acc[w + __popcll(m & ((1ull << lane) - 1ull))] = v;
+                    if (keep) dh_acc_put(A, L, ao + w + __popcll(m & ((1ull << lane) - 1ull)), v, loc, vl);
                     w += __popcll(m);
                 }
                 x.na = w;
@@ -260,8 +287,9 @@
                         }
                 }
                 if (lane == 0) {
-                    acc[x.na] = cand;
+                    dh_acc_put(A, L, ao + x.na, cand, loc, candl);
                     dkey[dn] = cand;
+                    if (loc && x.phase == 0) L.tpc[x.co + dn] = candl;
                     dstat[dn] = s;
                     dp[dn] = p;
                 }
@@ -276,7 +304,7 @@
         if (x.phase == 0) {
             x.phase = 1;
             x.nc = x.ntpc;
-            for (int q = lane; q < x.ntpc; q += 64) acc[q] = A.tpc_key[x.co + q];
+            for (int q = lane; q < x.ntpc; q += 64) dh_acc_put(A, L, ao + q, A.tpc_key[x.co + q], loc, loc ? L.tpc[x.co + q] : 0);
             x.na = x.ntpc;
             x.pos = 0;
         } else {
@@ -296,6 +324,11 @@
         }
         __builtin_amdgcn_fence(__ATOMIC_SEQ_CST, "workgroup");
     }
+}
+
+__device__ bool dh_advance(DhTgt &x, const DhArrays &A, int lane, int d1, bool keep_elim_stats = false)
+{
+    return dh_advance_impl<false>(x, A, lane, d1, keep_elim_stats, DhLoc{});
 }
 
 __device__ __forceinline__ unsigned int dh_ceil_div(unsigned long long w, unsigned long long seglen, double inv)
@@ -387,24 +420,28 @@
     return M;
 }
 
-template <bool TR = false>
+template <bool TR = false, bool LOC = false>
 __device__ __forceinline__ bool dh_commit(DhTgt &x, const DhArrays &A, int lane, int d1, double r_stat, double r_p, int r_pow,
-                                          double alpha, bool exact = false, int max_k_rej = 0, unsigned long long r_nt = 0ull, int r_df = 0)
+                                          double alpha, bool exact = false, int max_k_rej = 0, unsigned long long r_nt = 0ull, int r_df = 0,
+                                          const DhLoc &L = DhLoc{})
 {
     const int32_t *cands = x.phase == 0 ? A.cand0 + x.cand_off : A.tpc_key + x.co;
     const int32_t cand = cands[x.pos];
+    const bool loc = dh_has_loc<LOC>(x, L);
+    const int32_t candl = loc ? dh_cand_loc(x, L, x.pos) : 0;
     ++x.pos;
     if (!(r_p < alpha && r_pow)) {
         if constexpr (TR) {
             if (lane == 0) dh_rej_write(x, A, max_k_rej, cand, A.acc + DH_ACC_OFF(x, x.cur, d1), x.na, r_nt, r_stat, r_p, r_df, r_pow);
         }
         if (!(exact && x.phase == 1)) return false;
-        if (lane == 0) A.acc[DH_ACC_OFF(x, x.cur, d1) + x.na] = cand;
+        if (lane == 0) dh_acc_put(A, L, DH_ACC_OFF(x, x.cur, d1) + x.na, cand, loc, candl);
         ++x.na;
         return true;
     }
     if (lane == 0) {
-        A.acc[DH_ACC_OFF(x, x.cur, d1) + x.na] = cand;
+        dh_acc_put(A, L, DH_ACC_OFF(x, x.cur, d1) + x.na, cand, loc, candl);
+        if (loc && x.phase == 0) L.tpc[x.co + x.ntpc] = candl;
         if (x.phase == 0) {
             A.tpc_key[x.co + x.ntpc] = cand;
             A.tpc_stat[x.co + x.ntpc] = r_stat;
@@ -1721,7 +1758,7 @@
                                             const FwSegOut *__restrict__ so, const long long *__restrict__ seg0,
                                             unsigned long long *__restrict__ win, unsigned int *__restrict__ sp,
                                             unsigned long long *__restrict__ win2, const int32_t *__restrict__ act, const DhParams &P,
-                                            const int ci )
+                                            const int ci , const DhLoc &L)
 {
     const int lane = threadIdx.x & 63;
     const int d1 = P.spec_depth + 1;
@@ -1784,8 +1821,8 @@
                 x.c_eval_short += x.na <= FW_HK_A ? x.jevaluated : 0ull;
                 x.na_max = x.na > x.na_max ? x.na : x.na_max;
                 x.c_alg += dh_alg_bytes(x.na, x.jevaluated, P.max_k, P.disc_bytes_per_col);
-                if constexpr (TR) kept = dh_commit<true>(x, A, lane, d1, r_stat, r_p, r_pow, P.alpha, P.elim_mode != 0, P.max_k, r_nt, r_df);
-                else kept = dh_commit(x, A, lane, d1, r_stat, r_p, r_pow, P.alpha, P.elim_mode != 0);
+                if constexpr (TR) kept = dh_commit<true, true>(x, A, lane, d1, r_stat, r_p, r_pow, P.alpha, P.elim_mode != 0, P.max_k, r_nt, r_df, L);
+                else kept = dh_commit<false, true>(x, A, lane, d1, r_stat, r_p, r_pow, P.alpha, P.elim_mode != 0, 0, 0ull, 0, L);
             }
         }
         if (nsp_done > 0) {
@@ -1823,12 +1860,12 @@
                 x.c_eval_short += n <= FW_HK_A ? M.ev : 0ull;
                 x.c_alg += dh_alg_bytes(n, M.ev, P.max_k, P.disc_bytes_per_col);
                 bool k;
-                if constexpr (TR) k = dh_commit<true>(x, A, lane, d1, r_stat, r_p, M.stop ? M.pow : 1, P.alpha, P.elim_mode != 0, P.max_k, M.nt, M.df);
-                else k = dh_commit(x, A, lane, d1, r_stat, r_p, M.stop ? M.pow : 1, P.alpha, P.elim_mode != 0);
+                if constexpr (TR) k = dh_commit<true, true>(x, A, lane, d1, r_stat, r_p, M.stop ? M.pow : 1, P.alpha, P.elim_mode != 0, P.max_k, M.nt, M.df, L);
+                else k = dh_commit<false, true>(x, A, lane, d1, r_stat, r_p, M.stop ? M.pow : 1, P.alpha, P.elim_mode != 0, 0, 0ull, 0, L);
                 valid = ph1 ? k : !k;
             }
         }
-        if (!x.jactive && x.phase != 2 && dh_advance(x, A, lane, d1, P.elim_mode == 2)) {
+        if (!x.jactive && x.phase != 2 && dh_advance_impl<true>(x, A, lane, d1, P.elim_mode == 2, L)) {
             const unsigned long long N = dh_enum_size(x.na, P.max_k, P.max_tests);
             x.jN = N;
             x.jnext = 0ull;
@@ -1869,7 +1906,9 @@
                         }
                     }
                 }
-                const int32_t *src = A.acc + DH_ACC_OFF(x, x.cur, d1);
+                const bool loc = dh_has_loc<true>(x, L);
+                const long long src_o = DH_ACC_OFF(x, x.cur, d1);
+                const int32_t *src = A.acc + src_o;
                 int w[DH_MAX_SPEC];
 #pragma unroll
                 for (int j = 0; j < DH_MAX_SPEC; ++j) w[j] = 0;
@@ -1877,14 +1916,14 @@
                 for (int base = 0; base < n; base += 64) {
                     const int i = base + lane;
                     const int32_t v = i < n ? src[i] : -1;
+                    const int32_t vl = (loc && i < n) ? L.acc[src_o + i] : 0;
                     bool alive = i < n;
 #pragma unroll
                     for (int j = 0; j < DH_MAX_SPEC; ++j) {
                         if (j < Q) {
                             alive = alive && v != cn[j];
                             const unsigned long long m = __ballot(alive);
-                            int32_t *dst = A.acc + DH_ACC_OFF(x, (x.cur + 1 + j) % d1, d1);
-                            if (alive) dst[w[j] + __popcll(m & ((1ull << lane) - 1ull))] = v;
+                            if (alive) dh_acc_put(A, L, DH_ACC_OFF(x, (x.cur + 1 + j) % d1, d1) + w[j] + __popcll(m & ((1ull << lane) - 1ull)), v, loc, vl);
                             w[j] += __popcll(m);
                         }
                     }
@@ -1893,13 +1932,12 @@
 #pragma unroll
                 for (int j = 0; j < DH_MAX_SPEC; ++j) {
                     if (j == q && j < Q && w[j] == n - (j + 1)) {
-                        int32_t *dst = A.acc + DH_ACC_OFF(x, (x.cur + 1 + j) % d1, d1);
                         if (lane <= j) {
                             int32_t tail = c0;
 #pragma unroll
                             for (int u = 0; u < DH_MAX_SPEC; ++u)
                                 if (lane == u + 1) tail = cn[u];
-                            dst[w[j] + lane] = tail;
+                            dh_acc_put(A, L, DH_ACC_OFF(x, (x.cur + 1 + j) % d1, d1) + w[j] + lane, tail, loc, loc ? L.tpc[x.co + x.pos + lane] : 0);
                         }
                         q = j + 1;
                     }
@@ -1923,7 +1961,10 @@
                 ++q;
             }
             if (q > 0) {
-                if (lane == 0) A.acc[DH_ACC_OFF(x, x.cur, d1) + x.na] = cands[x.pos];
+                if (lane == 0) {
+                    const bool loc = dh_has_loc<true>(x, L);
+                    dh_acc_put(A, L, DH_ACC_OFF(x, x.cur, d1) + x.na, cands[x.pos], loc, loc ? dh_cand_loc(x, L, x.pos) : 0);
+                }
                 const unsigned long long N2 = dh_enum_size(x.na + 1, P.max_k, P.max_tests);
                 const unsigned long long w0 = x.na + 1 >= 64 ? P.w0_big : P.w0_small;
                 x.nsp = q;
@@ -1943,12 +1984,14 @@
 }
 
 template <bool TR>
-__global__ __launch_bounds__(256) void dh_step_kernel(DhTgt *__restrict__ tg, int ntg, DhGlobal *__restrict__ g, DhArrays A,
+__global__ __launch_bounds__(256, 4) void dh_step_kernel(DhTgt *__restrict__ tg, int ntg, DhGlobal *__restrict__ g, DhArrays A,
                                                       const FwSegOut *__restrict__ so, const long long *__restrict__ seg0,
                                                       unsigned long long *__restrict__ win, unsigned int *__restrict__ sp,
-                                                      unsigned long long *__restrict__ win2, const int32_t *__restrict__ act, DhParams P)
-{
-    dh_step_dev<TR>(tg, ntg, g, A, so, seg0, win, sp, win2, act, P, (int)(blockIdx.x * 4 + (threadIdx.x >> 6)));
+                                                      unsigned long long *__restrict__ win2, const int32_t *__restrict__ act, DhParams P,
+                                                      const int32_t *loc_cand0, int32_t *loc_tpc, int32_t *loc_acc)
+{
+    const DhLoc L{loc_cand0, loc_tpc, loc_acc};
+    dh_step_dev<TR>(tg, ntg, g, A, so, seg0, win, sp, win2, act, P, (int)(blockIdx.x * 4 + (threadIdx.x >> 6)), L);
 }
 
 #define DH_PER 16
@@ -2080,7 +2123,8 @@
 }
 
 __global__ __launch_bounds__(256) void dh_tmat_build_kernel(const DhTgt *__restrict__ tg, int ntg, const int32_t *__restrict__ nb_idx,
-                                                            const float *__restrict__ cor, int p, float *__restrict__ tmat)
+                                                            const float *__restrict__ cor, int p, float *__restrict__ tmat,
+                                                            const int32_t *__restrict__ cand0, int32_t *__restrict__ cand0_loc)
 {
     __shared__ int32_t s_id[4096];
     const DhTgt &x = tg[blockIdx.x];
@@ -2089,6 +2133,22 @@
     const int32_t *ids = nb_idx + x.nb_off;
     for (int b = threadIdx.x; b < m; b += 256) s_id[b] = b == 0 ? x.T : ids[b - 1];
     __syncthreads();
+    if (blockIdx.y == 0 && x.phase == 0) {
+        const int32_t *cands = cand0 + x.cand_off;
+        for (int q = threadIdx.x; q < x.nc; q += 256) {
+            const int32_t v = cands[q];
+            int lo = 1, hi = m - 1;
+            while (lo < hi) {
+                const int mid = (lo + hi) >> 1;
+                if (s_id[mid] < v)
+                    lo = mid + 1;
+                else
+                    hi = mid;
+            }
+            if (m < 2 || s_id[lo] != v) __builtin_trap();
+            cand0_loc[x.co + q] = lo;
+        }
+    }
     float *M = tmat + x.tm_off;
     for (int a0 = (int)blockIdx.y * 4; a0 < m; a0 += (int)gridDim.y * 4)
         for (int b = threadIdx.x; b < m; b += 256) {
@@ -2104,7 +2164,7 @@
 
 __device__ __forceinline__ void dh_fill_one(const unsigned int s, const DhTgt *__restrict__ tg, int ntg, DhGlobal *__restrict__ g,
                                             const long long *__restrict__ seg0, const DhArrays &A, FwSeg *__restrict__ segs, int d1,
-                                            const int32_t *__restrict__ act)
+                                            const int32_t *__restrict__ act, int max_k, const DhLoc &L)
 {
     int lo = 0, hi = (int)g->n_act;
     while (lo < hi) {
@@ -2144,16 +2204,26 @@
     sg.tm = has_tm ? (uint64_t)(A.tmat + x.tm_off) : 0ull;
     sg.tm_ids = has_tm ? (uint64_t)(A.nb_idx + x.nb_off) : 0ull;
     sg.tm_m = has_tm ? x.nb_n + 1 : 0;
-    sg.pad1 = 0;
+    const bool use_tm = fw_seg_uses_tmat(has_tm, sg.acc_len, max_k);
+    sg.tm_y = use_tm ? (x.phase == 0 ? L.cand0 : L.tpc)[x.co + x.pos + (int)slot] : 0;
+    if (use_tm) {
+        sg.acc_off += L.acc - A.acc;
+#if defined(FW_FZ_FASTDBG) && FW_FZ_FASTDBG >= 6
+        const long long dist = L.acc - A.acc;
+        sg.pad = dist <= 0x7fffffffll ? (int32_t)dist : 0;
+#endif
+    }
     segs[s] = sg;
 }
 __global__ __launch_bounds__(256) void dh_fill_kernel(const DhTgt *__restrict__ tg, int ntg, DhGlobal *__restrict__ g,
                                                       const long long *__restrict__ seg0, const DhArrays A,
-                                                      FwSeg *__restrict__ segs, int d1, const int32_t *__restrict__ act)
-{
+                                                      FwSeg *__restrict__ segs, int d1, const int32_t *__restrict__ act, int max_k,
+                                                      const int32_t *loc_cand0, int32_t *loc_tpc, int32_t *loc_acc)
+{
+    const DhLoc L{loc_cand0, loc_tpc, loc_acc};
     const unsigned int s = blockIdx.x * 256 + threadIdx.x;
     if (s >= g->ns) return;
-    dh_fill_one(s, tg, ntg, g, seg0, A, segs, d1, act);
+    dh_fill_one(s, tg, ntg, g, seg0, A, segs, d1, act, max_k, L);
 }
 
 
@@ -2562,13 +2632,19 @@
 struct DhLists {
     int32_t *tpc_key, *pc_key, *acc, *wl;
     double *tpc_stat, *tpc_p, *pc_stat, *pc_p;
+    int32_t *cand0_loc, *tpc_loc, *acc_loc;
 };
-static DhLists dh_lists_layout(DhArena &a, size_t n, size_t acc_d1, size_t n_wl)
+static DhLists dh_lists_layout(DhArena &a, size_t n, size_t acc_d1, size_t n_wl, bool loc)
 {
     DhLists b{};
     b.tpc_key = a.take<int32_t>(n, 4);
     b.pc_key = a.take<int32_t>(n, 4);
-    b.acc = a.take<int32_t>(2 * n * acc_d1, 4);
+    b.acc = a.take<int32_t>((loc ? 4 : 2) * n * acc_d1, 4);
+    if (loc) {
+        b.acc_loc = b.acc ? b.acc + 2 * n * acc_d1 : nullptr;
+        b.cand0_loc = a.take<int32_t>(n, 4);
+        b.tpc_loc = a.take<int32_t>(n, 4);
+    }
     b.tpc_stat = a.take<double>(n, 8);
     b.tpc_p = a.take<double>(n, 8);
     b.pc_stat = a.take<double>(n, 8);
@@ -2632,7 +2708,7 @@
 
 struct DhRunSizes {
     size_t ntg, tot, d1, n_wl, max_ns, tm_floats, nz_arena, p, nnz;
-    bool log, per_target, nzk, own_nb;
+    bool log, per_target, nzk, own_nb, loc;
 };
 struct DhRunBufs {
     DhTgt *tg;
@@ -2655,7 +2731,7 @@
     b.tg = a.take<DhTgt>(z.ntg);
     b.s = dh_scratch_layout(a, z.ntg, z.max_ns, z.tm_floats);
     b.cand0 = a.take<int32_t>(z.tot, 4);
-    b.lists = dh_lists_layout(a, z.tot, z.d1, z.n_wl);
+    b.lists = dh_lists_layout(a, z.tot, z.d1, z.n_wl, z.loc);
     if (z.log) b.log = a.take<ulonglong2>(DH_LOG_CAP);
     if (z.per_target) {
         b.mq = a.take<MiQueue>(1);
@@ -2693,6 +2769,7 @@
     DhRunBufs D{};
     DhGlobal *hg = nullptr;
     DhArrays A{};
+    DhLoc L{};
     DhParams P{};
     double timed_s = 0.0;
     long timed_n = 0, launches_n = 0;
@@ -2761,7 +2838,7 @@
     const size_t tot = R.tot, nnz = (size_t)c->nb_off[p];
     const bool nb_on_dev = c->d_nb_idx != nullptr;
     const DhRunSizes z{(size_t)ntg, tot, (size_t)R.y.spec_depth + 1, R.wl.size(), R.max_ns, R.tm_floats, R.nz_arena, (size_t)p, nnz,
-                       R.y.log_path != nullptr, R.y.per_target, R.y.nzk, !nb_on_dev};
+                       R.y.log_path != nullptr, R.y.per_target, R.y.nzk, !nb_on_dev, R.tm_floats > 0};
     int rc;
     if ((rc = dh_arena_reserve(c, c->d_dh[R.chain], dh_run_layout, z, &R.D))) return rc;
     if ((rc = fw_pin_reserve(c, c->h_dh[R.chain], 4096))) return rc;
@@ -2789,8 +2866,10 @@
     }
     DhArrays &A = R.A = dh_arrays(c, R.use_devc ? c->d_cand : D.cand0, D.lists, D.nb);
     A.tmat = D.s.tmat;
+    R.L = D.s.tmat ? DhLoc{D.lists.cand0_loc, D.lists.tpc_loc, D.lists.acc_loc} : DhLoc{};
     if (D.s.tmat) {
-        hipLaunchKernelGGL(dh_tmat_build_kernel, dim3((unsigned)ntg, 8u), dim3(256), 0, st, (const DhTgt *)D.tg, ntg, A.nb_idx, (const float *)c->d_cor, p, D.s.tmat);
+        hipLaunchKernelGGL(dh_tmat_build_kernel, dim3((unsigned)ntg, 8u), dim3(256), 0, st, (const DhTgt *)D.tg, ntg, A.nb_idx, (const float *)c->d_cor, p, D.s.tmat,
+                           A.cand0, D.lists.cand0_loc);
         FW_HIP(c, hipGetLastError());
         if (R.trace_host) fprintf(stderr, "[fw] chain %d: local correlation matrices: %.1f MB\n", R.chain, 4e-6 * (double)R.tm_floats);
     }
@@ -2882,10 +2961,10 @@
         }
         if (A.rej)
             hipLaunchKernelGGL(dh_step_kernel<true>, dim3((n_act_bound + 3u) / 4u), dim3(256), 0, hs, D.tg, ntg, S.g, A,
-                               (const FwSegOut *)S.so, (const long long *)S.seg0, S.win, S.sp, S.win2, (const int32_t *)S.act, R.P);
+                               (const FwSegOut *)S.so, (const long long *)S.seg0, S.win, S.sp, S.win2, (const int32_t *)S.act, R.P, R.L.cand0, R.L.tpc, R.L.acc);
         else
             hipLaunchKernelGGL(dh_step_kernel<false>, dim3((n_act_bound + 3u) / 4u), dim3(256), 0, hs, D.tg, ntg, S.g, A,
-                               (const FwSegOut *)S.so, (const long long *)S.seg0, S.win, S.sp, S.win2, (const int32_t *)S.act, R.P);
+                               (const FwSegOut *)S.so, (const long long *)S.seg0, S.win, S.sp, S.win2, (const int32_t *)S.act, R.P, R.L.cand0, R.L.tpc, R.L.acc);
         if (compact)
             hipLaunchKernelGGL(dh_compact_kernel, dim3(1), dim3(1024), 0, hs, (const DhTgt *)D.tg, ntg, S.g, S.act);
         if (y.plan_small)
@@ -2895,7 +2974,7 @@
             hipLaunchKernelGGL(dh_plan_kernel, dim3(1), dim3(1024), 0, hs, ntg, S.g, (const unsigned long long *)S.win,
                                (const unsigned int *)S.sp, (const unsigned long long *)S.win2, (const int32_t *)S.act, S.seg0, PA);
         hipLaunchKernelGGL(dh_fill_kernel, dim3(g_fill), dim3(256), 0, hs, (const DhTgt *)D.tg, ntg, S.g,
-                           (const long long *)S.seg0, A, S.segs, y.spec_depth + 1, (const int32_t *)S.act);
+                           (const long long *)S.seg0, A, S.segs, y.spec_depth + 1, (const int32_t *)S.act, c->P.max_k, R.L.cand0, R.L.tpc, R.L.acc);
         if (y.use_hp) {
             FW_HIP(c, hipEventRecord(c->dh_hp_ev[R.chain][1], hs));
             FW_HIP(c, hipStreamWaitEvent(st, c->dh_hp_ev[R.chain][1], 0));
@@ -3144,13 +3223,13 @@
     double *os, *op;
     unsigned long long *tot;
 };
-static DhSchedState dh_sched_state_layout(DhArena &a, size_t nt, size_t p, size_t nnz, size_t acc_d1)
+static DhSchedState dh_sched_state_layout(DhArena &a, size_t nt, size_t p, size_t nnz, size_t acc_d1, bool loc)
 {
     DhSchedState b{};
     b.tg = a.take<DhTgt>(nt);
     b.round_of = a.take<int32_t>(p);
     b.wl_cnt = a.take<unsigned int>(p);
-    b.lists = dh_lists_layout(a, nnz, acc_d1, nnz);
+    b.lists = dh_lists_layout(a, nnz, acc_d1, nnz, loc);
     b.ot = a.take<int32_t>(nnz, 4);
     b.ou = a.take<int32_t>(nnz, 4);
     b.os = a.take<double>(nnz, 8);
@@ -3228,7 +3307,7 @@
 static DhSchedBufs dh_sched_layout(DhArena &a, const DhSchedSizes &z)
 {
     DhSchedBufs b{};
-    b.S = dh_sched_state_layout(a, z.nt, z.p, z.nnz, 1);
+    b.S = dh_sched_state_layout(a, z.nt, z.p, z.nnz, 1, false);
     b.sched = a.take<int32_t>(z.nt);
     b.order = a.take<int32_t>(z.nt);
     b.mq = a.take<MiQueue>(z.nrounds);
@@ -3306,6 +3385,7 @@
     size_t nt, p, nnz, d1, nslots;
     int K;
     DhFzChainSizes ch[FW_DH_MAX_CHAINS];
+    bool loc;
 };
 struct DhFzBufs {
     DhSchedState S;
@@ -3317,7 +3397,7 @@
 static DhFzBufs dh_fz_layout(DhArena &a, const DhFzSizes &z)
 {
     DhFzBufs b{};
-    b.S = dh_sched_state_layout(a, z.nt, z.p, z.nnz, z.d1);
+    b.S = dh_sched_state_layout(a, z.nt, z.p, z.nnz, z.d1, z.loc);
     b.slot_T = a.take<int32_t>(z.nt);
     b.slot_tm = a.take<long long>(z.nt);
     b.wl_max = a.take<unsigned int>(z.nslots);
@@ -3397,6 +3477,7 @@
                 z.ch[q].ntg = std::max(z.ch[q].ntg, (size_t)s[q].ntg);
                 z.ch[q].max_ns = std::max(z.ch[q].max_ns, (size_t)s[q].max_ns);
                 z.ch[q].tm_floats = std::max(z.ch[q].tm_floats, s[q].tm_floats);
+                z.loc = z.loc || s[q].tm_floats > 0;
             }
         }
     }
@@ -3443,6 +3524,7 @@
         const DhRoundScratch &cb = Rn.D.s;
         Rn.A = A;
         Rn.A.tmat = cb.tmat;
+        Rn.L = cb.tmat ? DhLoc{D.S.lists.cand0_loc, D.S.lists.tpc_loc, D.S.lists.acc_loc} : DhLoc{};
         Rn.hg = (DhGlobal *)c->h_dh[q].ptr;
         memset(Rn.hg, 0, 2 * sizeof(DhGlobal));
         unsigned int *h_wl_max = (unsigned int *)((char *)c->h_dh[q].ptr + 3072);
@@ -3456,7 +3538,7 @@
         }
         if (cb.tmat) {
             hipLaunchKernelGGL(dh_tmat_build_kernel, dim3((unsigned)s.ntg, 8u), dim3(256), 0, sq, (const DhTgt *)Rn.D.tg, s.ntg, A.nb_idx,
-                               (const float *)c->d_cor, p, cb.tmat);
+                               (const float *)c->d_cor, p, cb.tmat, A.cand0, D.S.lists.cand0_loc);
             FW_HIP(c, hipGetLastError());
         }
         Rn.P = dh_make_params(c, s.ntg, Rn.y.spec_depth, Rn.y.spec0_depth);
diff --git a/flashweave.jl_amd/csrc/fw_fz.hip b/flashweave.jl_amd/csrc/fw_fz.hip
--- a/flashweave.jl_amd/csrc/fw_fz.hip
+++ b/flashweave.jl_amd/csrc/fw_fz.hip
@@ -796,7 +796,10 @@
 #ifdef FW_FZ_FASTDBG
 extern "C" void fwi_fz_fastdbg_print()
 {
-    unsigned long long c[24] = {0};
+    unsigned long long c[26] = {0};
+    if (hipMemcpyFromSymbol(c, HIP_SYMBOL(fz_fast_cnt), sizeof(c)) == hipSuccess && c[24])
+        fprintf(stderr, "[fw] local indices (validation build): %llu entries of accepted lists and candidates checked against the search in the sorted ids, MISMATCHES %llu\n",
+                c[24], c[15]);
     if (hipMemcpyFromSymbol(c, HIP_SYMBOL(fz_fast_cnt), sizeof(c)) == hipSuccess && c[19])
         fprintf(stderr, "[fw] cheap-screen potential: of %llu fast-loop wave-iterations, every lane clearly (relative margin on |stat|^2: 2e-4 / 2e-3 / 2e-2) above the wavefront's minimum so far and inside the sure range in %llu / %llu / %llu\n",
                 c[19], c[16], c[17], c[18]);
diff --git a/flashweave.jl_amd/csrc/fw_fz_core.h b/flashweave.jl_amd/csrc/fw_fz_core.h
--- a/flashweave.jl_amd/csrc/fw_fz_core.h
+++ b/flashweave.jl_amd/csrc/fw_fz_core.h
@@ -505,8 +505,9 @@
 }
 
 #define FZ_L1_A 512
+static_assert(FZ_L1_A == FW_TAB_A, "fw_seg_uses_tmat: one list bound for the table variants that read a local matrix");
 #ifdef FW_FZ_FASTDBG
-static __device__ unsigned long long fz_fast_cnt[24];
+static __device__ unsigned long long fz_fast_cnt[26];
 #endif
 static __device__ int fz_dbg_flags;
 template <int K>
@@ -573,9 +574,6 @@
     constexpr bool L1T = HIGHK && !TAB && !LOCAL;
 #ifndef FW_FZ_L1T_ROW32
 #define FW_FZ_L1T_ROW32 1
-#endif
-#ifndef FW_FZ_TMAT_HIGHK
-#define FW_FZ_TMAT_HIGHK 1
 #endif
 #ifndef FW_L3_SCREEN
 #define FW_L3_SCREEN 0
@@ -662,32 +660,35 @@
     }
     int Xl = -1, Yl = -1;
     bool tloc = false;
-    if (!LOCAL && seg.tm != 0ull && (TAB3 || (FW_FZ_TMAT_HIGHK && ((HK && FW_FZ_TMAT_HIGHK != 2) || L1T) && in_lds))) {
-        int32_t *s_ids = TAB3 ? (int32_t *)s_tab : (HK ? (int32_t *)s_hk : (int32_t *)s3_blk);
+    if (!LOCAL && (TAB3 || (FW_FZ_TMAT_HIGHK && (HK || L1T))) && seg.tm_y != 0) {
         if (!TAB3) tloc = true;
-        const int32_t *ids = (const int32_t *)seg.tm_ids;
-        const int nid = seg.tm_m - 1;
-        for (int i = tid; i < nid; i += 256) s_ids[i] = ids[i];
-        __syncthreads();
-        auto local_of = [&](int v) -> int {
-            if (v == seg.X) return 0;
-            int lo = 0, hi = nid - 1;
-            while (lo < hi) {
-                const int mid = (lo + hi) >> 1;
-                if (s_ids[mid] < v)
-                    lo = mid + 1;
-                else
-                    hi = mid;
-            }
-            if (nid <= 0 || s_ids[lo] != v) __builtin_trap();
-            return lo + 1;
-        };
-        for (int i = tid; i < a; i += 256) s_acc[i] = local_of(s_acc[i]);
         Xl = 0;
-        Yl = local_of(seg.Y);
+        Yl = seg.tm_y;
         cor = cor_g + (((long long)seg.tm - (long long)(unsigned long long)cor_g) >> 2);
         p = seg.tm_m;
-        __syncthreads();
+#if defined(FW_FZ_FASTDBG) && FW_FZ_FASTDBG >= 6
+        if (seg.pad != 0) {
+            const int32_t *ids = (const int32_t *)seg.tm_ids;
+            const int nid = seg.tm_m - 1;
+            auto local_of = [&](int v) -> int {
+                if (v == seg.X) return 0;
+                int lo = 0, hi = nid - 1;
+                while (lo < hi) {
+                    const int mid = (lo + hi) >> 1;
+                    if (ids[mid] < v)
+                        lo = mid + 1;
+                    else
+                        hi = mid;
+                }
+                return (nid <= 0 || ids[lo] != v) ? -1 : lo + 1;
+            };
+            unsigned int bad = 0u;
+            for (int i = tid; i < a; i += 256) bad += local_of(gacc[(long long)i - (long long)seg.pad]) != gacc[i] ? 1u : 0u;
+            if (tid == 0) bad += local_of(seg.Y) != seg.tm_y ? 1u : 0u;
+            if (bad) atomicAdd(&fz_fast_cnt[15], (unsigned long long)bad);
+            if (tid == 0) atomicAdd(&fz_fast_cnt[24], (unsigned long long)a + 1ull);
+        }
+#endif
     }
     if (tid == 0) {
         s_best_x = FZ_X_NONE;
diff --git a/flashweave.jl_amd/csrc/fw_internal.h b/flashweave.jl_amd/csrc/fw_internal.h
--- a/flashweave.jl_amd/csrc/fw_internal.h
+++ b/flashweave.jl_amd/csrc/fw_internal.h
@@ -109,7 +109,7 @@
     uint64_t start;
     uint64_t end;
     uint64_t tm, tm_ids;
-    int32_t tm_m, pad1;
+    int32_t tm_m, tm_y;
 };
 
 #define FW_RANK_NONE (~0ull)
@@ -117,6 +117,15 @@
 #ifndef FW_HK_A
 #define FW_HK_A 88
 #endif
+#ifndef FW_FZ_TMAT_HIGHK
+#define FW_FZ_TMAT_HIGHK 1
+#endif
+static inline __host__ __device__ bool fw_seg_uses_tmat(bool has_tm, int acc_len, int max_k)
+{
+    if (!has_tm || acc_len > FW_TAB_A) return false;
+    if (max_k <= 3) return true;
+    return FW_FZ_TMAT_HIGHK == 1 || (FW_FZ_TMAT_HIGHK == 2 && acc_len > FW_HK_A);
+}
 
 struct FwNzJob {
     int32_t X, Y;
```

New measurement: 83.76 billion. No clear change (-0.0%).
